# julius-sk/spgemm-prunning

Measured on AMD Instinct MI355X. Metric: SpGEMM+SSpMM GTEPS (edges/s) & HBM-BW% on Reddit h=256 k=16; vs CPU SpMM, higher is better.
Workload: dtype f32

## Files before the change

include/maxk_hip.h:

```cpp
#ifndef MAXK_HIP_H_
#define MAXK_HIP_H_

#include <stddef.h>
#include <stdint.h>

#ifdef __cplusplus
extern "C" {
#endif

#define MAXK_OK 0
#define MAXK_ERR_INVALID (-1)
#define MAXK_ERR_HIP (-2)
#define MAXK_ERR_NODEVICE (-3)
#define MAXK_ERR_LIBRARY (-4)

int maxk_version(void);

const char *maxk_last_error(void);

int maxk_device_count(void);

const char *maxk_source_digest(void);

const char *maxk_build_config(void);
// ... 3 lines not shown
int maxk_spgemm_forward(const int32_t *row_ptr, const int32_t *col_idx, const float *edge_val,
                        const float *cbsr_val, const uint8_t *cbsr_idx, const float *row_div,
                        float *out, int64_t num_rows, int64_t num_cols, int64_t num_e,
                        int32_t dim_origin, int32_t dim_k, int32_t chunk_edges,
                        void *workspace, size_t workspace_bytes, void *stream);
int maxk_spgemm_forward_sel(const int32_t *row_ptr, const int32_t *col_idx, const float *edge_val,
                            const float *cbsr_val, const uint8_t *cbsr_idx, const float *row_div,
                            float *out, int64_t num_rows, int64_t num_cols, int64_t num_e,
                            int32_t dim_origin, int32_t dim_k, int32_t chunk_edges,
                            void *workspace, size_t workspace_bytes, void *stream,
                            uint8_t *edge_sel);
int maxk_spgemm_forward_accumulate(const int32_t *row_ptr, const int32_t *col_idx,
                                   const float *edge_val, const float *cbsr_val,
                                   const uint8_t *cbsr_idx, const float *row_div, float *out,
                                   int64_t num_rows, int64_t num_cols, int64_t num_e,
                                   int32_t dim_origin, int32_t dim_k, int32_t chunk_edges,
                                   void *workspace, size_t workspace_bytes, void *stream);
int maxk_spgemm_forward_accumulate_sel(const int32_t *row_ptr, const int32_t *col_idx,
                                       const float *edge_val, const float *cbsr_val,
                                       const uint8_t *cbsr_idx, const float *row_div, float *out,
                                       int64_t num_rows, int64_t num_cols, int64_t num_e,
                                       int32_t dim_origin, int32_t dim_k, int32_t chunk_edges,
                                       void *workspace, size_t workspace_bytes, void *stream,
                                       uint8_t *edge_sel);
int maxk_records_ok(int64_t num_rows, int64_t num_cols, int64_t num_e, int32_t dim_origin,
                    int32_t dim_k);
int maxk_cbsr_records(const float *cbsr_val, const uint8_t *cbsr_idx, uint8_t *rec,
                      int64_t num_rows, int32_t dim_origin, int32_t dim_k, void *stream);
int maxk_spgemm_forward_records(const int32_t *row_ptr, const int32_t *col_idx,
                                const float *edge_val, const uint8_t *rec, const float *row_div,
                                float *out, int64_t num_rows, int64_t num_cols, int64_t num_e,
                                int32_t dim_origin, int32_t dim_k, int32_t chunk_edges,
                                void *workspace, size_t workspace_bytes, void *stream,
                                int32_t accumulate);

size_t maxk_edge_weight_grad_workspace_size(int64_t num_rows, int64_t num_cols, int64_t num_e,
                                            int32_t dim_origin, int32_t dim_k,
                                            int32_t chunk_edges);
int maxk_edge_weight_grad(const int32_t *row_ptr, const int32_t *col_idx, const float *cbsr_val,
                          const uint8_t *cbsr_idx, const float *grad_out, const float *row_div,
                          float *grad_edge, int64_t num_rows, int64_t num_cols, int64_t num_e,
                          int32_t dim_origin, int32_t dim_k, int32_t chunk_edges,
                          void *workspace, size_t workspace_bytes, void *stream);

#define MAXK_MAX_HEADS 8

size_t maxk_spgemm_forward_heads_workspace_size(int64_t num_rows, int64_t num_cols,
                                                int64_t num_e, int32_t dim_origin, int32_t dim_k,
                                                int32_t num_heads, int32_t chunk_edges);
int maxk_spgemm_forward_heads(const int32_t *row_ptr, const int32_t *col_idx,
                              const float *edge_val, const float *cbsr_val,
                              const uint8_t *cbsr_idx, const float *row_div, float *out,
                              int64_t num_rows, int64_t num_cols, int64_t num_e,
                              int32_t dim_origin, int32_t dim_k, int32_t num_heads,
                              int32_t chunk_edges, void *workspace, size_t workspace_bytes,
                              void *stream);

size_t maxk_edge_weight_grad_heads_workspace_size(int64_t num_rows, int64_t num_cols,
                                                  int64_t num_e, int32_t dim_origin,
                                                  int32_t dim_k, int32_t num_heads,
                                                  int32_t chunk_edges);
int maxk_edge_weight_grad_heads(const int32_t *row_ptr, const int32_t *col_idx,
                                const float *cbsr_val, const uint8_t *cbsr_idx,
                                const float *grad_out, const float *row_div, float *grad_edge,
                                int64_t num_rows, int64_t num_cols, int64_t num_e,
                                int32_t dim_origin, int32_t dim_k, int32_t num_heads,
                                int32_t chunk_edges, void *workspace, size_t workspace_bytes,
                                void *stream);

size_t maxk_edge_softmax_workspace_size(int64_t num_rows, int64_t num_cols, int64_t num_e,
                                        int32_t chunk_edges);
int maxk_edge_softmax(const int32_t *row_ptr, const float *logits, float *w, int64_t num_rows,
                      int64_t num_cols, int64_t num_e, int32_t chunk_edges, void *workspace,
                      size_t workspace_bytes, void *stream);
size_t maxk_edge_softmax_backward_workspace_size(int64_t num_rows, int64_t num_cols,
                                                 int64_t num_e, int32_t chunk_edges);
int maxk_edge_softmax_backward(const int32_t *row_ptr, const float *w, const float *grad_w,
                               float *grad_logits, int64_t num_rows, int64_t num_cols,
                               int64_t num_e, int32_t chunk_edges, void *workspace,
                               size_t workspace_bytes, void *stream);
size_t maxk_gat_edge_softmax_workspace_size(int64_t num_rows, int64_t num_cols, int64_t num_e,
                                            int32_t chunk_edges);
int maxk_gat_edge_softmax(const int32_t *row_ptr, const int32_t *col_idx, const float *s_dst,
                          const float *s_src, float negative_slope, float *w, int64_t num_rows,
                          int64_t num_cols, int64_t num_e, int32_t chunk_edges, void *workspace,
                          size_t workspace_bytes, void *stream);
size_t maxk_gat_edge_softmax_backward_workspace_size(int64_t num_rows, int64_t num_cols,
                                                     int64_t num_e, int32_t chunk_edges);
int maxk_gat_edge_softmax_backward(const int32_t *row_ptr, const int32_t *col_idx,
                                   const int32_t *col_ptr, const int32_t *csc_eid,
                                   const float *s_dst, const float *s_src, float negative_slope,
                                   const float *w, const float *grad_w, float *grad_s_dst,
                                   float *grad_s_src, int64_t num_rows, int64_t num_cols,
                                   int64_t num_e, int32_t chunk_edges, void *workspace,
                                   size_t workspace_bytes, void *stream);

size_t maxk_gat_edge_softmax_heads_workspace_size(int32_t num_heads, int64_t num_rows,
                                                  int64_t num_cols, int64_t num_e,
                                                  int32_t chunk_edges);
int maxk_gat_edge_softmax_heads(const int32_t *row_ptr, const int32_t *col_idx,
                                const float *s_dst, const float *s_src, float negative_slope,
                                float *w, int32_t num_heads, int64_t num_rows, int64_t num_cols,
                                int64_t num_e, int32_t chunk_edges, void *workspace,
                                size_t workspace_bytes, void *stream);
size_t maxk_gat_edge_softmax_heads_backward_workspace_size(int32_t num_heads, int64_t num_rows,
                                                           int64_t num_cols, int64_t num_e,
                                                           int32_t chunk_edges);
int maxk_gat_edge_softmax_heads_backward(const int32_t *row_ptr, const int32_t *col_idx,
                                         const int32_t *col_ptr, const int32_t *csc_eid,
                                         const float *s_dst, const float *s_src,
                                         float negative_slope, const float *w,
                                         const float *grad_w, float *grad_s_dst,
                                         float *grad_s_src, int32_t num_heads, int64_t num_rows,
                                         int64_t num_cols, int64_t num_e, int32_t chunk_edges,
                                         void *workspace, size_t workspace_bytes, void *stream);

size_t maxk_gat_attention_heads_workspace_size(int64_t num_rows, int64_t num_cols, int64_t num_e,
                                               int32_t dim_origin, int32_t dim_k,
                                               int32_t num_heads, int32_t chunk_edges);
int maxk_gat_attention_heads(const int32_t *row_ptr, const int32_t *col_idx, const float *s_dst,
                             const float *s_src, float negative_slope, const float *cbsr_val,
                             const uint8_t *cbsr_idx, float *out, float *row_max, float *row_sum,
                             int64_t num_rows, int64_t num_cols, int64_t num_e,
                             int32_t dim_origin, int32_t dim_k, int32_t num_heads,
                             int32_t chunk_edges, void *workspace, size_t workspace_bytes,
                             void *stream);
size_t maxk_gat_edge_alpha_heads_workspace_size(int32_t num_heads, int64_t num_rows,
                                                int64_t num_cols, int64_t num_e);
int maxk_gat_edge_alpha_heads(const int32_t *row_ptr, const int32_t *col_idx, const float *s_dst,
                              const float *s_src, float negative_slope, const float *row_max,
                              const float *row_sum, float *w, int32_t num_heads,
                              int64_t num_rows, int64_t num_cols, int64_t num_e, void *workspace,
                              size_t workspace_bytes, void *stream);

size_t maxk_gat_attention_heads_backward_workspace_size(int64_t num_rows, int64_t num_cols,
                                                        int64_t num_e, int32_t dim_origin,
                                                        int32_t dim_k, int32_t num_heads,
                                                        int32_t chunk_edges);
int maxk_gat_attention_heads_backward(
    const int32_t *row_ptr, const int32_t *col_idx, const int32_t *col_ptr,
    const int32_t *csc_eid, const float *s_dst, const float *s_src, float negative_slope,
    const float *cbsr_val, const uint8_t *cbsr_idx, const float *out, const float *row_max,
    const float *row_sum, const float *grad_out, float *grad_s_dst, float *grad_s_src,
    float *grad_cbsr, int64_t num_rows, int64_t num_cols, int64_t num_e, int32_t dim_origin,
    int32_t dim_k, int32_t num_heads, int32_t chunk_edges, void *workspace,
    size_t workspace_bytes, void *stream);

int maxk_edge_dropout_heads(const float *w, float *out, int32_t num_heads, int64_t num_e, float p,
                            uint64_t seed, void *stream);
size_t maxk_gat_attention_heads_dropout_workspace_size(int64_t num_rows, int64_t num_cols,
                                                       int64_t num_e, int32_t dim_origin,
                                                       int32_t dim_k, int32_t num_heads,
                                                       int32_t chunk_edges);
int maxk_gat_attention_heads_dropout(
    const int32_t *row_ptr, const int32_t *col_idx, const float *s_dst, const float *s_src,
    float negative_slope, const float *cbsr_val, const uint8_t *cbsr_idx, float *out,
    float *row_max, float *row_sum, int64_t num_rows, int64_t num_cols, int64_t num_e,
    int32_t dim_origin, int32_t dim_k, int32_t num_heads, int32_t chunk_edges, float p,
    uint64_t seed, void *workspace, size_t workspace_bytes, void *stream);
size_t maxk_gat_attention_heads_dropout_backward_workspace_size(
    int64_t num_rows, int64_t num_cols, int64_t num_e, int32_t dim_origin, int32_t dim_k,
    int32_t num_heads, int32_t chunk_edges);
int maxk_gat_attention_heads_dropout_backward(
    const int32_t *row_ptr, const int32_t *col_idx, const int32_t *col_ptr,
    const int32_t *csc_eid, const float *s_dst, const float *s_src, float negative_slope,
    const float *cbsr_val, const uint8_t *cbsr_idx, const float *out, const float *row_max,
    const float *row_sum, const float *grad_out, float *grad_s_dst, float *grad_s_src,
    float *grad_cbsr, int64_t num_rows, int64_t num_cols, int64_t num_e, int32_t dim_origin,
    int32_t dim_k, int32_t num_heads, int32_t chunk_edges, float p, uint64_t seed,
    void *workspace, size_t workspace_bytes, void *stream);

size_t maxk_dot_attention_heads_workspace_size(int64_t num_rows, int64_t num_cols, int64_t num_e,
                                               int32_t dim_origin, int32_t dim_k,
                                               int32_t num_heads, int32_t chunk_edges);
int maxk_dot_attention_heads(const int32_t *row_ptr, const int32_t *col_idx, const float *q,
                             float scale, const float *cbsr_val, const uint8_t *cbsr_idx,
                             float *out, float *row_max, float *row_sum, int64_t num_rows,
                             int64_t num_cols, int64_t num_e, int32_t dim_origin, int32_t dim_k,
                             int32_t num_heads, int32_t chunk_edges, void *workspace,
                             size_t workspace_bytes, void *stream);
size_t maxk_dot_edge_alpha_heads_workspace_size(int64_t num_rows, int64_t num_cols, int64_t num_e,
                                                int32_t dim_origin, int32_t dim_k,
                                                int32_t num_heads, int32_t chunk_edges);
int maxk_dot_edge_alpha_heads(const int32_t *row_ptr, const int32_t *col_idx, const float *q,
                              float scale, const float *cbsr_val, const uint8_t *cbsr_idx,
                              const float *row_max, const float *row_sum, float *w,
                              int64_t num_rows, int64_t num_cols, int64_t num_e,
                              int32_t dim_origin, int32_t dim_k, int32_t num_heads,
                              int32_t chunk_edges, void *workspace, size_t workspace_bytes,
                              void *stream);

size_t maxk_dot_attention_heads_backward_workspace_size(int64_t num_rows, int64_t num_cols,
                                                        int64_t num_e, int32_t dim_origin,
                                                        int32_t dim_k, int32_t num_heads,
                                                        int32_t chunk_edges);
int maxk_dot_attention_heads_backward(
    const int32_t *row_ptr, const int32_t *col_idx, const int32_t *col_ptr, const int32_t *csc_eid,
    const float *q, float scale, const float *cbsr_val, const uint8_t *cbsr_idx, const float *out,
    const float *row_max, const float *row_sum, const float *grad_out, float *grad_q,
    float *grad_cbsr, int64_t num_rows, int64_t num_cols, int64_t num_e, int32_t dim_origin,
    int32_t dim_k, int32_t num_heads, int32_t chunk_edges, void *workspace,
    size_t workspace_bytes, void *stream);

size_t maxk_sspmm_backward_workspace_size(int64_t num_rows, int64_t num_cols, int64_t num_e,
                                          int32_t dim_origin, int32_t dim_k, int32_t chunk_edges);
int maxk_sspmm_backward(const int32_t *row_ptr, const int32_t *col_idx, const float *edge_val,
                        const float *grad_out, const float *row_div, const uint8_t *cbsr_idx,
                        float *grad_cbsr, int64_t num_rows, int64_t num_cols, int64_t num_e,
                        int32_t dim_origin, int32_t dim_k, int32_t chunk_edges,
                        void *workspace, size_t workspace_bytes, void *stream);

size_t maxk_sspmm_backward_csc_workspace_size(int64_t num_rows, int64_t num_cols, int64_t num_e,
                                              int32_t dim_origin, int32_t dim_k,
                                              int32_t chunk_edges);
int maxk_sspmm_backward_csc(const int32_t *row_ptr, const int32_t *col_idx, const float *edge_val,
                            const float *grad_out, const float *row_div, const uint8_t *cbsr_idx,
                            const int32_t *col_ptr, const int32_t *csc_eid, float *grad_cbsr,
                            int64_t num_rows, int64_t num_cols, int64_t num_e, int32_t dim_origin,
                            int32_t dim_k, int32_t chunk_edges, void *workspace,
                            size_t workspace_bytes, void *stream);

int maxk_sspmm_backward_csc_sel(const int32_t *row_ptr, const int32_t *col_idx,
                                const float *edge_val, const float *grad_out, const float *row_div,
                                const uint8_t *edge_sel, const int32_t *col_ptr,
                                const int32_t *csc_eid, float *grad_cbsr, int64_t num_rows,
                                int64_t num_cols, int64_t num_e, int32_t dim_origin, int32_t dim_k,
                                int32_t chunk_edges, void *workspace, size_t workspace_bytes,
                                void *stream);
int maxk_edge_selectors(const int32_t *col_idx, const uint8_t *cbsr_idx, int64_t num_e,
                        int32_t dim_k, uint8_t *edge_sel, void *stream);
int64_t maxk_edge_selectors_blocks(int64_t n_words);

size_t maxk_sspmm_backward_heads_workspace_size(int64_t num_rows, int64_t num_cols,
                                                int64_t num_e, int32_t dim_origin, int32_t dim_k,
                                                int32_t num_heads, int32_t chunk_edges);
int maxk_sspmm_backward_heads(const int32_t *row_ptr, const int32_t *col_idx,
                              const float *edge_val, const float *grad_out, const float *row_div,
                              const uint8_t *cbsr_idx, const int32_t *col_ptr,
                              const int32_t *csc_eid, float *grad_cbsr, int64_t num_rows,
                              int64_t num_cols, int64_t num_e, int32_t dim_origin, int32_t dim_k,
                              int32_t num_heads, int32_t chunk_edges, void *workspace,
                              size_t workspace_bytes, void *stream);

size_t maxk_transpose_plan_workspace_size(int64_t num_cols, int64_t num_e);
int maxk_transpose_plan(const int32_t *col_idx, int64_t num_cols, int64_t num_e,
                        int32_t *col_ptr, int32_t *csc_eid, void *workspace,
                        size_t workspace_bytes, void *stream);

int maxk_bucket_shift(int32_t dim_k);
int64_t maxk_bucket_count(int64_t num_cols, int32_t bucket_shift);

int32_t maxk_bsort_window(int32_t dim_k);
size_t maxk_bsort_plan_workspace_size(int64_t num_cols, int64_t num_e);
int maxk_bsort_plan(const int32_t *row_ptr, const int32_t *col_idx, int64_t num_rows,
                    int64_t num_cols, int64_t num_e, int32_t dim_k, int32_t bucket_shift,
                    int32_t *bucket_ptr, int32_t *bucket_pos, uint16_t *bucket_dst,
                    uint16_t *win_src, int32_t *edge_row, void *workspace,
                    size_t workspace_bytes, void *stream);
size_t maxk_sspmm_backward_bsort_workspace_size(int64_t num_rows, int64_t num_cols,
                                                int64_t num_e, int32_t dim_origin,
                                                int32_t dim_k);
int maxk_sspmm_backward_bsort(const int32_t *row_ptr, const int32_t *col_idx,
                              const float *edge_val, const float *grad_out, const float *row_div,
                              const uint8_t *cbsr_idx, const uint8_t *edge_sel,
                              const int32_t *bucket_ptr, const int32_t *bucket_pos,
                              const uint16_t *bucket_dst, const uint16_t *win_src,
                              const int32_t *edge_row, int32_t bucket_shift, float *grad_cbsr,
                              int64_t num_rows,
                              int64_t num_cols, int64_t num_e, int32_t dim_origin, int32_t dim_k,
                              void *workspace, size_t workspace_bytes, void *stream);

size_t maxk_sspmm_backward_pull_workspace_size(int64_t num_rows, int64_t num_cols,
                                               int32_t dim_origin, int32_t dim_k, int32_t slices);
int maxk_sspmm_backward_pull(const float *grad_out, const float *row_div,
                             const uint8_t *cbsr_idx, const int32_t *tile_ptr,
                             const uint32_t *ent, int32_t bucket_shift, int32_t slices,
                             float *grad_cbsr, int64_t num_rows, int64_t num_cols, int64_t num_e,
                             int32_t dim_origin, int32_t dim_k, void *workspace,
                             size_t workspace_bytes, void *stream);

#define MAXK_PULL_NO_REDUCE 2
#define MAXK_PULL_REDUCE_ONLY 4
size_t maxk_sspmm_backward_pull_tiles_workspace_size(int64_t num_rows, int64_t num_cols,
                                                     int32_t dim_origin, int32_t dim_k,
                                                     int32_t n_tiles);
int maxk_sspmm_backward_pull_tiles(const float *grad_out, const float *row_div,
                                   const uint8_t *cbsr_idx, const int32_t *tile_list,
                                   const int32_t *tile_ent, int32_t n_tiles,
                                   const int32_t *bucket_ptr, const int32_t *bucket_tiles,
                                   const uint32_t *ent, int32_t bucket_shift, int32_t slices,
                                   int32_t accumulate, float *grad_cbsr, int64_t num_rows,
                                   int64_t num_cols, int64_t num_e, int32_t dim_origin,
                                   int32_t dim_k, void *workspace, size_t workspace_bytes,
                                   void *stream);

int maxk_pull_shift(int32_t dim_k);
int maxk_pull_slices(int64_t num_rows, int64_t num_cols, int32_t dim_origin, int32_t dim_k);
size_t maxk_pull_plan_workspace_size(int64_t num_rows, int64_t num_cols, int64_t num_e,
                                     int32_t bucket_shift, int32_t slices);
int maxk_pull_plan(const int32_t *row_ptr, const int32_t *col_idx, const float *edge_val,
                   int64_t num_rows, int64_t num_cols, int64_t num_e, int32_t bucket_shift,
                   int32_t slices, int32_t *tile_ptr, uint32_t *ent, void *workspace,
                   size_t workspace_bytes, void *stream);

int maxk_dense_route(int32_t dim_origin, int32_t dim_k);
int maxk_dense_plan(const int32_t *row_ptr, const float *edge_val, const int32_t *csc_eid,
                    int64_t num_rows, int64_t num_e, int32_t *t_src, float *t_w, void *stream);
size_t maxk_sspmm_backward_dense_workspace_size(int64_t num_rows, int64_t num_cols,
                                                int64_t num_e, int32_t dim_origin, int32_t dim_k,
                                                int32_t chunk_edges);
int maxk_sspmm_backward_dense(const int32_t *col_ptr, const int32_t *t_src, const float *t_w,
                              const float *grad_out, const float *row_div,
                              const uint8_t *cbsr_idx, float *grad_cbsr, int64_t num_rows,
                              int64_t num_cols, int64_t num_e, int32_t dim_origin, int32_t dim_k,
                              int32_t chunk_edges, void *workspace, size_t workspace_bytes,
                              void *stream);

#define MAXK_BWD_PULL 0
#define MAXK_BWD_CSC 1
#define MAXK_BWD_HYBRID 3
#define MAXK_BWD_ATOMIC 4
#define MAXK_BWD_BSORT 5
#define MAXK_BWD_DENSE 6
#define MAXK_BSORT_KMAX 8
#define MAXK_HYBRID_LOCALITY 1.5
#define MAXK_HYBRID_DENSITY 0.5f
#define MAXK_HYBRID_PRESCALED 1
int maxk_backward_mode_auto(int64_t num_rows, int64_t num_cols, int64_t num_e, int32_t dim_origin,
                            int32_t dim_k, double pull_locality);
int maxk_pull_locality(const int32_t *row_ptr, const int32_t *col_idx, int64_t num_rows,
                       int64_t num_e, int32_t bucket_shift, double *locality, void *workspace,
                       size_t workspace_bytes, void *stream);
size_t maxk_hybrid_plan_workspace_size(int64_t num_rows, int64_t num_cols, int64_t num_e,
                                       int32_t bucket_shift, int32_t slices);
int maxk_hybrid_plan(const int32_t *row_ptr, const int32_t *col_idx, const float *edge_val,
                     const int32_t *tile_ptr, const uint32_t *ent, int64_t num_rows,
                     int64_t num_cols, int64_t num_e, int32_t bucket_shift, int32_t slices,
                     float density, int32_t *tile_list, int32_t *tile_ent, int32_t *bucket_ptr,
                     int32_t *bucket_tiles, uint32_t *ent_pull, int32_t *off_row_ptr,
                     int32_t *off_col, float *off_val, int64_t *counts, void *workspace,
                     size_t workspace_bytes, void *stream);
int maxk_pull_entries_scale(const uint32_t *ent, const int32_t *tile_ids, const int32_t *tile_ent,
                            int64_t n_runs, int64_t num_rows, int64_t num_cols,
                            int32_t bucket_shift, int32_t slices, const float *row_div,
                            uint32_t *ent_out, void *stream);
size_t maxk_sspmm_backward_hybrid_workspace_size(int64_t num_rows, int64_t num_cols,
                                                 int64_t n_off_e, int32_t dim_origin,
                                                 int32_t dim_k, int64_t n_tiles);
int maxk_sspmm_backward_hybrid(
    const float *grad_out, const float *row_div, const uint8_t *cbsr_idx,
    const int32_t *tile_list, const int32_t *tile_ent, int32_t n_tiles, const int32_t *bucket_ptr,
    const int32_t *bucket_tiles, const uint32_t *ent_pull, int64_t n_pull_e, int32_t bucket_shift,
    int32_t slices, const int32_t *off_row_ptr, const int32_t *off_col, const float *off_val,
    int64_t n_off_e, const int32_t *off_col_ptr, const int32_t *off_csc_eid, int32_t flags,
    float *grad_cbsr, int64_t num_rows, int64_t num_cols, int32_t dim_origin, int32_t dim_k,
    void *workspace, size_t workspace_bytes, void *stream, void *side_stream, void *ev_fork,
    void *ev_join);

int maxk_topk_cbsr(const float *x, int64_t ld_x, float *cbsr_val, uint8_t *cbsr_idx,
                   int32_t *idx32, int64_t num_rows, int32_t dim_origin, int32_t dim_k,
                   void *stream);
int maxk_topk_cbsr_u8(const uint8_t *x, int64_t ld_x, uint8_t *cbsr_val, uint8_t *cbsr_idx,
                      int32_t *idx32, int64_t num_rows, int32_t dim_origin, int32_t dim_k,
                      void *stream);
int maxk_topk_u8_reference(const uint8_t *x, uint8_t *val, uint8_t *idx, int64_t num_rows,
                           int32_t dim_origin, int32_t dim_k, void *stream);
int maxk_topk_error_rows(int64_t *rows, int32_t reset, void *stream);

int maxk_cbsr_scatter_dense(const float *cbsr_val, const uint8_t *cbsr_idx, float *dense,
                            int64_t num_rows, int32_t dim_origin, int32_t dim_k, void *stream);

int maxk_topk_cbsr_dense(const float *x, int64_t ld_x, float *cbsr_val, uint8_t *cbsr_idx,
                         float *dense, int64_t num_rows, int32_t dim_origin, int32_t dim_k,
                         void *stream);

int maxk_topk_backward(const float *grad_val, const float *grad_dense, const uint8_t *cbsr_idx,
                       float *grad_x, int64_t num_rows, int32_t dim_origin, int32_t dim_k,
                       void *stream);

int maxk_warp4_count(const int32_t *row_ptr, int64_t num_rows, int32_t warp_max_nz,
                     int64_t *num_entries, void *stream);
size_t maxk_warp4_build_workspace_size(int64_t num_rows);
int maxk_warp4_build(const int32_t *row_ptr, int64_t num_rows, int32_t warp_max_nz,
                     int32_t *warp4, int64_t num_entries, void *workspace,
                     size_t workspace_bytes, void *stream);
int maxk_warp4_to_row_ptr(const int32_t *warp4, int64_t num_entries, int64_t num_rows,
                          int32_t *row_ptr, void *stream);

typedef struct maxk_dense_spmm_plan maxk_dense_spmm_plan;
int maxk_dense_spmm_plan_create(maxk_dense_spmm_plan **plan, const int32_t *row_ptr,
                                const int32_t *col_idx, const float *edge_val, const float *x,
                                float *y, int64_t num_rows, int64_t num_cols, int64_t num_e,
                                int32_t dim, int32_t alg, void *stream);
int maxk_dense_spmm_run(maxk_dense_spmm_plan *plan, void *stream);
int maxk_dense_spmm_bind(maxk_dense_spmm_plan *plan, const float *x, float *y);
int maxk_dense_spmm_plan_destroy(maxk_dense_spmm_plan *plan);

#ifdef __cplusplus
}
#endif

#endif
```

spgemm-prunning_amd/csrc/sspmm_pull.hip:

```cpp
#include <algorithm>

#include "sspmm_bwd.h"

namespace maxk {
namespace {

__global__ __launch_bounds__(kBlock) void gprime_kernel(const float *__restrict__ G,
                                                        const float *__restrict__ row_div,
                                                        float *__restrict__ Gp, int64_t n4,
                                                        int D4) {
    const int64_t i = blockIdx.x * (int64_t)kBlock + threadIdx.x;
    if (i >= n4) return;
    const float dv = row_div[i / D4];
    float4 v = reinterpret_cast<const float4 *>(G)[i];
    v.x /= dv;
    v.y /= dv;
    v.z /= dv;
    v.w /= dv;
    reinterpret_cast<float4 *>(Gp)[i] = v;
}

template <int LR, int U, bool SEL_LDS, int VPL>
__global__ __launch_bounds__(1024) void pull_tile_kernel(
    const float *__restrict__ Gp, const uint8_t *__restrict__ cbsr_idx,
    const int32_t *__restrict__ tile_ptr, const uint2 *__restrict__ ent,
    float *__restrict__ tile_out, int64_t num_cols, int n_buckets, int rows_per_slice, int D,
    int k, int shift) {
    extern __shared__ double acc[];
    constexpr int EPI = kWave / LR;
    constexpr int STEP = EPI * U;
    const int tid = threadIdx.x;
    const int lane = lane_id(), w = tid / kWave;
    const int g = lane / LR, q = lane % LR;
    const bool qok = q < k / VPL;
    const int ks = k + 1;
    const int t = blockIdx.x;
    const int j = t % n_buckets;
    const float *__restrict__ Gs = Gp + (size_t)(t / n_buckets) * rows_per_slice * D;
    const int s0 = tile_ptr[t], s1 = tile_ptr[t + 1];
    const int64_t c0 = (int64_t)j << shift;
    const uint8_t *__restrict__ selg = cbsr_idx + c0 * k;
    uint8_t *sel_lds = reinterpret_cast<uint8_t *>(acc + (ks << shift));
    for (int i = tid; i < (ks << shift); i += 1024) acc[i] = 0.0;
    if (SEL_LDS) {
        const int rows = num_cols - c0 < (1 << shift) ? (int)(num_cols - c0) : (1 << shift);
        const int nb = rows * k;
        for (int i = tid; i < nb / 16; i += 1024)
            reinterpret_cast<uint4 *>(sel_lds)[i] = reinterpret_cast<const uint4 *>(selg)[i];
        for (int i = (nb & ~15) + tid; i < nb; i += 1024) sel_lds[i] = selg[i];
    }
    __syncthreads();
    int base = s0 + w * STEP;
    uint2 en[U];
    constexpr bool kShfl = MAXK_PULL_SHFL && LR <= 8;
    constexpr int NL = (STEP + kWave - 1) / kWave;
    uint2 my[NL];
    auto load_ids = [&](int b) {
        if constexpr (kShfl) {
#pragma unroll
            for (int m = 0; m < NL; ++m) {
                const int e = b + m * kWave + lane;
                my[m] = ent[e < s1 ? e : s1 - 1];
                if (e >= s1 || m * kWave + lane >= STEP) my[m].x = 0xffff0000u;
            }
        } else {
#pragma unroll
            for (int u = 0; u < U; ++u) {
                const int e = b + u * EPI + g;
                en[u] = ent[e < s1 ? e : s1 - 1];
                if (e >= s1) en[u].x = 0xffff0000u;
            }
        }
    };
    if (base < s1) load_ids(base);
    for (; base < s1; base += 16 * STEP) {
        if constexpr (kShfl) {
#pragma unroll
            for (int u = 0; u < U; ++u) {
                const int m = (u * EPI) / kWave;
                const int src = (u * EPI + g - m * kWave) * 4;
                en[u].x = (uint32_t)__builtin_amdgcn_ds_bpermute(src, (int)my[m].x);
                en[u].y = (uint32_t)__builtin_amdgcn_ds_bpermute(src, (int)my[m].y);
            }
        }
        uint32_t sv[U];
        int dc[U];
        float wc[U];
#pragma unroll
        for (int u = 0; u < U; ++u) {
            const uint32_t key = en[u].x;
            dc[u] = (key >> 16) == 0xffffu ? -1 : (int)(key >> 16);
            const int bo = (dc[u] < 0 ? 0 : dc[u]) * k + (qok ? q : 0) * VPL;
            const uint8_t *sb8 = SEL_LDS ? sel_lds : selg;
            sv[u] = VPL == 4 ? *reinterpret_cast<const uint32_t *>(sb8 + bo) : (uint32_t)sb8[bo];
        }
        float v[U][VPL];
#pragma unroll
        for (int u = 0; u < U; ++u) {
            const float *gr = Gs + (en[u].x & 0xffffu) * (uint32_t)D;
#pragma unroll
            for (int i = 0; i < VPL; ++i) {
                const uint32_t c = (sv[u] >> (8 * i)) & 255u;
                const bool in = c < (uint32_t)D;
                const float x = gr[in ? c : 0u];
                v[u][i] = in ? x : 0.0f;
            }
            wc[u] = __uint_as_float(en[u].y);
        }
        if (base + 16 * STEP < s1) load_ids(base + 16 * STEP);
#pragma unroll
        for (int u = 0; u < U; ++u) {
            if (dc[u] >= 0 && qok) {
                double *a = &acc[dc[u] * ks + VPL * q];
#pragma unroll
                for (int i = 0; i < VPL; ++i) atomicAdd(a + i, (double)(wc[u] * v[u][i]));
            }
        }
    }
    __syncthreads();
    float *o = tile_out + (size_t)t * ((size_t)k << shift);
    if (MAXK_PULL_F4_FLUSH && k % 4 == 0) {
        for (int i4 = tid; i4 < (k << shift) / 4; i4 += 1024) {
            const double *a = &acc[i4 * 4 + (i4 * 4) / k];
            reinterpret_cast<float4 *>(o)[i4] =
                make_float4((float)a[0], (float)a[1], (float)a[2], (float)a[3]);
        }
    } else {
        for (int i = tid; i < (k << shift); i += 1024) o[i] = (float)acc[i + i / k];
    }
}

__global__ __launch_bounds__(kBlock) void pull_sel_kernel(const uint8_t *__restrict__ sel,
                                                          uint8_t *__restrict__ sel_q,
                                                          uint8_t *__restrict__ lmap,
                                                          int64_t num_cols, int k, int kp,
                                                          int vpl) {
    __shared__ uint32_t bm[kBlock / 4 * 8];
    __shared__ uint8_t s_out[kBlock], l_out[kBlock];
    const int nd = kBlock / k;
    const int tid = threadIdx.x;
    const int d = tid / k, l = tid % k;
    const int64_t c0 = (int64_t)blockIdx.x * nd;
    const int64_t c = c0 + d;
    const bool act = d < nd && c < num_cols;
    for (int i = tid; i < nd * 8; i += kBlock) bm[i] = 0u;
    __syncthreads();
    const uint32_t s = act ? sel[c * k + l] : 0u;
    if (act) atomicOr(&bm[d * 8 + (s >> 5)], 1u << (s & 31));
    __syncthreads();
    if (act) {
        int distinct = 0, rank = 0;
        for (int wd = 0; wd < 8; ++wd) {
            const uint32_t b = bm[d * 8 + wd];
            distinct += __popc(b);
            if (wd < (int)(s >> 5)) rank += __popc(b);
        }
        rank += __popc(bm[d * 8 + (s >> 5)] & ((1u << (s & 31)) - 1u));
        if (distinct < k) {
            rank = 0;
            for (int m = 0; m < k; ++m) {
                const uint32_t sm = sel[c * k + m];
                rank += (sm < s) || (sm == s && m < l);
            }
        }
        const int ql = kp / vpl, h = rank / kp, r = rank % kp;
        const int slot = h * kp + vpl * (r % ql) + r / ql;
        s_out[d * k + slot] = (uint8_t)s;
        l_out[d * k + slot] = (uint8_t)l;
    }
    __syncthreads();
    const int64_t nb = (num_cols - c0 < nd ? num_cols - c0 : nd) * (int64_t)k;
    if (tid < nb) {
        sel_q[c0 * k + tid] = s_out[tid];
        lmap[c0 * k + tid] = l_out[tid];
    }
}

__global__ __launch_bounds__(kBlock) void pull_sel4_kernel(const uint8_t *__restrict__ sel,
                                                           uint8_t *__restrict__ sel_q,
                                                           uint8_t *__restrict__ lmap,
                                                           int64_t num_cols, int k, int kp,
                                                           int vpl) {
    __shared__ uint32_t bm[kBlock * 8];
    __shared__ uint32_t s_out[kBlock], l_out[kBlock];
    const int tpd = k / 4;
    const int nd = kBlock / tpd;
    const int tid = threadIdx.x;
    const int d = tid / tpd, l0 = (tid % tpd) * 4;
    const int64_t c0 = (int64_t)blockIdx.x * nd;
    const int64_t c = c0 + d;
    const bool act = d < nd && c < num_cols;
    for (int i = tid; i < nd * 8; i += kBlock) bm[i] = 0u;
    __syncthreads();
    const uint32_t w4 = act ? *reinterpret_cast<const uint32_t *>(sel + c * k + l0) : 0u;
    if (act) {
#pragma unroll
        for (int j = 0; j < 4; ++j) {
            const uint32_t sj = (w4 >> (8 * j)) & 255u;
            atomicOr(&bm[d * 8 + (sj >> 5)], 1u << (sj & 31));
        }
    }
    __syncthreads();
    if (act) {
        uint32_t wds[8];
        int distinct = 0;
#pragma unroll
        for (int wd = 0; wd < 8; ++wd) {
            wds[wd] = bm[d * 8 + wd];
            distinct += __popc(wds[wd]);
        }
        uint8_t *so = reinterpret_cast<uint8_t *>(s_out), *lo = reinterpret_cast<uint8_t *>(l_out);
        const int ql = kp / vpl;
#pragma unroll
        for (int j = 0; j < 4; ++j) {
            const uint32_t sj = (w4 >> (8 * j)) & 255u;
            const int l = l0 + j;
            int rank = 0;
            if (distinct == k) {
                const int hi = (int)(sj >> 5);
#pragma unroll
                for (int wd = 0; wd < 8; ++wd) {
                    rank += wd < hi ? __popc(wds[wd]) : 0;
                    rank += wd == hi ? __popc(wds[wd] & ((1u << (sj & 31)) - 1u)) : 0;
                }
            } else {
                for (int m = 0; m < k; ++m) {
                    const uint32_t sm = sel[c * k + m];
                    rank += (sm < sj) || (sm == sj && m < l);
                }
            }
            const int h = rank / kp, r = rank % kp;
            const int slot = h * kp + vpl * (r % ql) + r / ql;
            so[d * k + slot] = (uint8_t)sj;
            lo[d * k + slot] = (uint8_t)l;
        }
    }
    __syncthreads();
    const int64_t nbytes = (num_cols - c0 < nd ? num_cols - c0 : nd) * (int64_t)k;
    if ((int64_t)tid * 4 < nbytes) {
        reinterpret_cast<uint32_t *>(sel_q + c0 * k)[tid] = s_out[tid];
        reinterpret_cast<uint32_t *>(lmap + c0 * k)[tid] = l_out[tid];
    }
}

template <int LR, int U, bool FULLD, int VPL>
__device__ __forceinline__ void pull_q_entries(double *acc, const uint8_t *sel_lds,
                                               __amdgpu_buffer_rsrc_t grs,
                                               __amdgpu_buffer_rsrc_t ers, int n_e, int D,
                                               int kp, int shift) {
    constexpr int EPI = kWave / LR;
    constexpr int STEP = EPI * U;
    constexpr int NL = (STEP + kWave - 1) / kWave;
    const int tid = threadIdx.x;
    const int lane = lane_id(), w = tid / kWave;
    constexpr int EPQ = LR < 16 ? 16 / LR : 1;
    const int lc = (lane % 16) % 4, lm = (lane % 16) / 4;
    constexpr bool TR = MAXK_PULL_TRANSPOSE && LR <= 16;
    const int g = !TR ? lane / LR
                  : LR >= 4 ? (lane / 16) * EPQ + lc / (LR / 4 > 0 ? LR / 4 : 1)
                            : (lane / 16) * EPQ + lc * (4 / LR) + lm / LR;
    const int q = !TR ? lane % LR
                  : LR >= 4 ? (lc % (LR / 4 > 0 ? LR / 4 : 1)) * 4 + lm
                            : lm % LR;
    const bool qok = q < kp / VPL;
    const int ks = pull_ks(kp, shift);
    const uint32_t Db = (uint32_t)D * 4u;
    const int stride = 16 * STEP;
    const int base = w * STEP;
    const int nsteps = base < n_e ? (n_e - base + stride - 1) / stride : 0;
    const int idle = (w * kWave + lane) & ((1 << shift) - 1);

    typedef unsigned int u32x2 __attribute__((ext_vector_type(2)));
    u32x2 myA[NL], myB[NL];
    float vA[U][VPL], vB[U][VPL];
    int dA[U], dB[U];
    float wA[U], wB[U];
    auto load_ent = [&](u32x2(&my)[NL], int n) {
#pragma unroll
        for (int m = 0; m < NL; ++m)
            my[m] = __builtin_amdgcn_raw_buffer_load_b64(
                ers, (int)((uint32_t)(base + n * stride + m * kWave + lane) * 8u), 0, 0);
    };
    auto issue = [&](u32x2(&my)[NL], float(&v)[U][VPL], int(&dc)[U], float(&wc)[U], int n) {
        uint32_t ex[U], ey[U];
#pragma unroll
        for (int u = 0; u < U; ++u) {
            const int m = (u * EPI) / kWave;
            const int src = (u * EPI + g - m * kWave) * 4;
            ex[u] = (uint32_t)__builtin_amdgcn_ds_bpermute(src, (int)my[m][0]);
            ey[u] = (uint32_t)__builtin_amdgcn_ds_bpermute(src, (int)my[m][1]);
        }
        load_ent(my, n + 2);
        uint64_t sv[U];
        bool ok[U];
        const int eb = base + n * stride + g;
#pragma unroll
        for (int u = 0; u < U; ++u) {
            ok[u] = eb + u * EPI < n_e && qok;
            const int d = ok[u] ? (int)(ex[u] >> 16) : idle;
            dc[u] = d * ks + VPL * q * ok[u];
            const uint8_t *sp = sel_lds + d * kp + (ok[u] ? q * VPL : 0);
            if constexpr (VPL == 8)
                sv[u] = *reinterpret_cast<const uint64_t *>(sp);
            else if constexpr (VPL == 4)
                sv[u] = *reinterpret_cast<const uint32_t *>(sp);
            else
                sv[u] = *reinterpret_cast<const uint16_t *>(sp);
            wc[u] = ok[u] ? __uint_as_float(ey[u]) : 0.0f;
        }
#pragma unroll
        for (int u = 0; u < U; ++u) {
            const uint32_t ro = ok[u] ? (ex[u] & 0xffffu) * Db : 0x80000000u;
#pragma unroll
            for (int i = 0; i < VPL; ++i) {
                const uint32_t c = VPL == 8 ? (uint32_t)(sv[u] >> (8 * i)) & 255u
                                            : ((uint32_t)sv[u] >> (8 * i)) & 255u;
                uint32_t off = ro + c * 4u;
                if (!FULLD) off = c < (uint32_t)D ? off : 0x80000000u;
                v[u][i] = __builtin_bit_cast(
                    float, __builtin_amdgcn_raw_buffer_load_b32(grs, (int)off, 0, 0));
            }
        }
    };
    auto consume = [&](float(&v)[U][VPL], int(&dc)[U], float(&wc)[U]) {
#pragma unroll
        for (int u = 0; u < U; ++u) {
            double *a = &acc[dc[u]];
#pragma unroll
            for (int i = 0; i < VPL; ++i) atomicAdd(a + i, (double)(wc[u] * v[u][i]));
        }
    };
    if (nsteps > 0) {
        load_ent(myA, 0);
        load_ent(myB, 1);
        __builtin_amdgcn_sched_barrier(0);
        issue(myA, vA, dA, wA, 0);
        for (int n = 0; n < nsteps; n += 2) {
            issue(myB, vB, dB, wB, n + 1);
            __builtin_amdgcn_sched_barrier(0);
            consume(vA, dA, wA);
            __builtin_amdgcn_sched_barrier(0);
            issue(myA, vA, dA, wA, n + 2);
            __builtin_amdgcn_sched_barrier(0);
            consume(vB, dB, wB);
            __builtin_amdgcn_sched_barrier(0);
        }
    }
}

struct PullTile {
    int64_t r0, nrows, c0;
    int s0, s1;
};
__device__ __forceinline__ PullTile pull_tile_of(int t, int i, const int32_t *__restrict__ tile_ptr,
                                                 int n_buckets, int rows_per_slice,
                                                 int64_t num_rows, int shift) {
    PullTile p;
    p.r0 = (int64_t)(t / n_buckets) * rows_per_slice;
    p.nrows = num_rows - p.r0 < rows_per_slice ? num_rows - p.r0 : rows_per_slice;
    p.c0 = (int64_t)(t % n_buckets) << shift;
    p.s0 = tile_ptr[i];
    p.s1 = tile_ptr[i + 1];
    return p;
}

constexpr int kSelRegs = 2;
struct PullSel {
    uint4 v[kSelRegs];
};
__device__ __forceinline__ PullSel pull_sel_load(const uint8_t *__restrict__ sel_q, int64_t c0,
                                                 int64_t num_cols, int k, int kp, int h,
                                                 int shift) {
    PullSel r;
    const int tid = threadIdx.x;
    const int rows = num_cols - c0 < (1 << shift) ? (int)(num_cols - c0) : (1 << shift);
    const uint8_t *__restrict__ selg = sel_q + c0 * k + h * kp;
#pragma unroll
    for (int m = 0; m < kSelRegs; ++m) {
        const int i = tid + m * 1024;
        uint4 x = make_uint4(0u, 0u, 0u, 0u);
        if (kp % 16 == 0) {
            const int ppr = kp / 16;
            if (i < rows * ppr)
                x = *reinterpret_cast<const uint4 *>(selg + (int64_t)(i / ppr) * k + (i % ppr) * 16);
        } else {
            uint32_t wd[4];
            const int wpr = kp / 4;
#pragma unroll
            for (int b = 0; b < 4; ++b) {
                const int wi = i * 4 + b;
                wd[b] = wi < rows * wpr
                            ? *reinterpret_cast<const uint32_t *>(selg + (int64_t)(wi / wpr) * k +
                                                                  (wi % wpr) * 4)
                            : 0u;
            }
            x = make_uint4(wd[0], wd[1], wd[2], wd[3]);
        }
        r.v[m] = x;
    }
    return r;
}
__device__ __forceinline__ void pull_sel_store(uint8_t *sel_lds, const PullSel &r, int kp,
                                               int shift) {
    const int n16 = (kp << shift) / 16;
#pragma unroll
    for (int m = 0; m < kSelRegs; ++m) {
        const int i = threadIdx.x + m * 1024;
        if (i < n16) reinterpret_cast<uint4 *>(sel_lds)[i] = r.v[m];
    }
}

__device__ __forceinline__ void pull_flush(const double *acc, float *__restrict__ tile_out, int t,
                                           int h, int k, int kp, int shift) {
    const int ks = pull_ks(kp, shift);
    float *o = tile_out + (size_t)t * ((size_t)k << shift) + h * kp;
    const int w4 = kp / 4;
    for (int i4 = threadIdx.x; i4 < (kp << shift) / 4; i4 += 1024) {
        const int c = i4 / w4, s4 = i4 % w4;
        const double *a = &acc[c * ks + 4 * s4];
        *reinterpret_cast<float4 *>(o + (size_t)c * k + 4 * s4) =
            make_float4((float)a[0], (float)a[1], (float)a[2], (float)a[3]);
    }
}

template <int LR, int U, bool FULLD, int VPL>
__global__ __launch_bounds__(1024) void pull_q_kernel(
    const float *__restrict__ Gp, const uint8_t *__restrict__ sel_q,
    const int32_t *__restrict__ tile_ptr, const uint2 *__restrict__ ent,
    float *__restrict__ tile_out, int64_t num_cols, int n_buckets, int n_tiles,
    int rows_per_slice, int64_t num_rows, int D, int k, int kp, int shift,
    const int32_t *__restrict__ tile_list) {
    extern __shared__ double acc[];
    const int tid = threadIdx.x;
    const int ks = pull_ks(kp, shift);
    const int H = k / kp;
    const int tp = MAXK_PULL_XCD ? xcd_contiguous_block(blockIdx.x, gridDim.x) : blockIdx.x;
    if (tp >= n_tiles * H) return;
    const int ti = tp / H, h = tp % H;
    const int t = tile_list ? tile_list[ti] : ti;
    const PullTile p = pull_tile_of(t, ti, tile_ptr, n_buckets, rows_per_slice, num_rows, shift);
    uint8_t *sel_lds = reinterpret_cast<uint8_t *>(acc + (ks << shift));
    for (int i = tid; i < (ks << shift); i += 1024) acc[i] = 0.0;
    pull_sel_store(sel_lds, pull_sel_load(sel_q, p.c0, num_cols, k, kp, h, shift), kp, shift);
    __syncthreads();
    const auto grs =
        wave_buffer(Gp + p.r0 * D, (uint32_t)(p.nrows > 0 ? p.nrows : 0) * (uint32_t)D * 4u);
    const auto ers = wave_buffer(ent + p.s0, (uint32_t)(p.s1 - p.s0) * 8u);
    pull_q_entries<LR, U, FULLD, VPL>(acc, sel_lds, grs, ers, p.s1 - p.s0, D, kp, shift);
    __syncthreads();
    pull_flush(acc, tile_out, ti, h, k, kp, shift);
}

__global__ __launch_bounds__(kBlock) void pull_reduce_kernel(const float *__restrict__ tile_out,
                                                             const uint8_t *__restrict__ lmap,
                                                             float *__restrict__ grad_cbsr,
                                                             int64_t num_cols, int n_buckets,
                                                             int slices, int k, int shift,
                                                             const int32_t *__restrict__ bucket_ptr,
                                                             const int32_t *__restrict__ bucket_tiles,
                                                             int accumulate) {
    const int j = blockIdx.x;
    const int64_t c0 = (int64_t)j << shift;
    const int rows = num_cols - c0 < (1 << shift) ? (int)(num_cols - c0) : (1 << shift);
    const int i = blockIdx.y * kBlock + threadIdx.x;
    const int nf = rows * k;
    if (i * 4 >= nf) return;
    const size_t n4 = ((size_t)k << shift) / 4;
    const float4 *to = reinterpret_cast<const float4 *>(tile_out);
    if (i * 4 + 4 > nf) {
        const int f0 = i * 4;
        for (int f = f0; f < nf; ++f) {
            float a = tile_out[(size_t)j * n4 * 4 + f];
            for (int s = 1; s < slices; ++s) a += tile_out[((size_t)s * n_buckets + j) * n4 * 4 + f];
            grad_cbsr[c0 * k + f] = a;
        }
        return;
    }
    float4 a;
    if (bucket_ptr) {
        a = make_float4(0.f, 0.f, 0.f, 0.f);
        for (int q = bucket_ptr[j]; q < bucket_ptr[j + 1]; ++q) {
            const float4 b = to[(size_t)bucket_tiles[q] * n4 + i];
            a.x += b.x;
            a.y += b.y;
            a.z += b.z;
            a.w += b.w;
        }
    } else {
        a = to[(size_t)j * n4 + i];
        for (int s = 1; s < slices; ++s) {
            const float4 b = to[((size_t)s * n_buckets + j) * n4 + i];
            a.x += b.x;
            a.y += b.y;
            a.z += b.z;
            a.w += b.w;
        }
    }
    if (lmap) {
        const size_t f0 = (size_t)c0 * k + (size_t)i * 4;
        const uint32_t m = *reinterpret_cast<const uint32_t *>(lmap + f0);
        float *row = grad_cbsr + (f0 / k) * k;
        if (accumulate) {
            a.x += row[m & 255u];
            a.y += row[(m >> 8) & 255u];
            a.z += row[(m >> 16) & 255u];
            a.w += row[m >> 24];
        }
        row[m & 255u] = a.x;
        row[(m >> 8) & 255u] = a.y;
        row[(m >> 16) & 255u] = a.z;
        row[m >> 24] = a.w;
        return;
    }
    reinterpret_cast<float4 *>(grad_cbsr + c0 * k)[i] = a;
}

int pull_parts(int k, int shift) {
    for (int H = 1; H <= k / 4; H *= 2) {
        if (k % (4 * H)) break;
        if (pull_fits(k / H, k / H, shift)) return H;
    }
    return 0;
}

struct PullLayout {
    size_t tile_off, sel_off, lmap_off, total;
};

PullLayout pull_layout(int64_t num_rows, int64_t num_cols, int D, int k, int64_t tiles,
                       int shift) {
    PullLayout L{};
    L.tile_off = al256((size_t)num_rows * D * sizeof(float));
    L.sel_off = L.tile_off + (size_t)tiles * ((size_t)k << shift) * sizeof(float);
    const size_t nsel = k % 4 == 0 ? al256((size_t)num_cols * k) : 0;
    L.lmap_off = L.sel_off + nsel;
    L.total = L.lmap_off + nsel;
    return L;
}

int pull_impl(const float *grad_out, const float *row_div, const uint8_t *cbsr_idx,
              const int32_t *tile_ptr, const uint32_t *ent, int32_t bucket_shift, int32_t slices,
              bool listed, const int32_t *tile_list, int32_t n_list, const int32_t *bucket_ptr,
              const int32_t *bucket_tiles, int32_t accumulate, float *grad_cbsr, int64_t num_rows,
              int64_t num_cols, int64_t num_e, int32_t dim_origin, int32_t dim_k, void *workspace,
              size_t workspace_bytes, void *stream) {
    if (int rc = check_common(num_rows, num_cols, num_e, dim_origin, dim_k, 0)) return rc;
    MAXK_REQUIRE(dim_k % 4 == 0 || dim_k <= 64,
                 "pull backward needs dim_k %% 4 == 0 or dim_k <= 64, got %d", dim_k);
    MAXK_REQUIRE(dim_origin % 4 == 0, "pull backward needs dim_origin %% 4 == 0, got %d",
                 dim_origin);
    const bool v4 = dim_k % 4 == 0;
    const int parts = MAXK_PULL_Q && v4 && bucket_shift >= 4 && bucket_shift <= 15
                          ? pull_parts(dim_k, bucket_shift)
                          : 0;
    const int max_shift = std::max(maxk_bucket_shift(dim_k), maxk_pull_shift(dim_k));
    MAXK_REQUIRE(bucket_shift >= 4 && bucket_shift <= 15 && bucket_shift <= max_shift &&
                     (parts > 0 || bucket_shift <= maxk_bucket_shift(dim_k)),
                 "bucket_shift %d out of range [4, min(15, %d)] for dim_k %d", bucket_shift,
                 max_shift, dim_k);
    const int64_t nb = maxk_bucket_count(num_cols, bucket_shift);
    MAXK_REQUIRE(slices >= 1 && slices * nb < (1LL << 31), "slices %d out of range", slices);
    const int64_t rps = (num_rows + slices - 1) / slices;
    MAXK_REQUIRE(rps <= 65536, "%d slices leave %lld rows per slice (max 65536)", slices,
                 (long long)rps);
    hipStream_t s = as_stream(stream);
    if (num_cols == 0) return MAXK_OK;
    MAXK_REQUIRE(grad_cbsr && tile_ptr, "grad_cbsr/tile_ptr must not be NULL");
    MAXK_REQUIRE(num_e == 0 || (grad_out && cbsr_idx && ent),
                 "grad/selector/plan pointers must not be NULL");
    MAXK_REQUIRE(!listed || (parts > 0 && bucket_ptr && n_list >= 0 &&
                             (n_list == 0 || (tile_list && bucket_tiles))),
                 "listed tiles need dim_k %% 4 == 0 and tile_list/bucket_ptr/bucket_tiles");
    const int64_t tiles = listed ? (int64_t)n_list : (int64_t)slices * nb;
    const PullLayout L = pull_layout(num_rows, num_cols, dim_origin, dim_k, tiles, bucket_shift);
    MAXK_REQUIRE(workspace && workspace_bytes >= L.total,
                 "workspace too small: need %zu bytes, got %zu", L.total, workspace_bytes);
    char *ws = reinterpret_cast<char *>(workspace);
    const bool front = !(accumulate & MAXK_PULL_REDUCE_ONLY);
    const bool back = !(accumulate & MAXK_PULL_NO_REDUCE);
    MAXK_REQUIRE(listed || (front && back), "reduce-only / no-reduce need listed tiles");
    MAXK_REQUIRE(front || back, "no-reduce and reduce-only together run nothing");
    const int k = dim_k;
    const float *Gp = grad_out;
    if (front && row_div && num_rows > 0 && num_e > 0) {
        const int64_t n4 = num_rows * dim_origin / 4;
        hipLaunchKernelGGL(gprime_kernel, dim3((unsigned)ceil_div(n4, kBlock)), dim3(kBlock), 0,
                           s, grad_out, row_div, reinterpret_cast<float *>(workspace), n4,
                           dim_origin / 4);
        MAXK_LAUNCHED("gprime_kernel");
        Gp = reinterpret_cast<const float *>(workspace);
    }
    float *tile_out = reinterpret_cast<float *>(ws + L.tile_off);
    const size_t acc_b = ((size_t)(k + 1) << bucket_shift) * sizeof(double);
    const size_t sel_b = ((size_t)k << bucket_shift);
    const bool sel_lds = acc_b + sel_b <= kPullLdsBytes;
    const size_t lds = acc_b + (sel_lds ? sel_b : 0);
    const uint2 *ent2 = reinterpret_cast<const uint2 *>(ent);
    const uint8_t *lmap = nullptr;
    if (parts > 0) {
        const int kp = k / parts;
        const size_t lds_q = pull_lds_bytes(pull_ks(kp, bucket_shift), kp, bucket_shift);
        uint8_t *sel_q = reinterpret_cast<uint8_t *>(ws + L.sel_off);
        uint8_t *lm = reinterpret_cast<uint8_t *>(ws + L.lmap_off);
        const int nd = kBlock / k;
        const int vpl = kp != 8 ? 4 : MAXK_PULL_VPL8 ? MAXK_PULL_VPL8 : parts == 1 ? 8 : 4;
        lmap = lm;
        if (!front) goto reduce;
        if (MAXK_PULL_SEL4 && (reinterpret_cast<uintptr_t>(cbsr_idx) & 3) == 0) {
            const int nd4 = kBlock / (k / 4);
            hipLaunchKernelGGL(pull_sel4_kernel, dim3((unsigned)ceil_div(num_cols, nd4)),
                               dim3(kBlock), 0, s, cbsr_idx, sel_q, lm, num_cols, k, kp, vpl);
            MAXK_LAUNCHED("pull_sel4_kernel");
        } else {
            hipLaunchKernelGGL(pull_sel_kernel, dim3((unsigned)ceil_div(num_cols, nd)),
                               dim3(kBlock), 0, s, cbsr_idx, sel_q, lm, num_cols, k, kp, vpl);
            MAXK_LAUNCHED("pull_sel_kernel");
        }
        const int64_t work = tiles * parts;
        const bool fulld = dim_origin == kMaxDim;
        const unsigned grid = (unsigned)(MAXK_PULL_XCD ? xcd_grid(work) : work);
        if (work == 0) goto reduce;
        const int lr = vpl == 4 ? lanes_per_edge(kp / 4) : kp / vpl;
        const bool ok = with_lanes(lr, [&](auto lr_c) {
            with_const<2, 4, 8>(vpl, [&](auto vpl_c) {
                with_const<0, 1>(fulld, [&](auto fd_c) {
                    constexpr int LR = decltype(lr_c)::value, VPL = decltype(vpl_c)::value;
                    if constexpr (VPL == 4 || LR * VPL == 8)
                        hipLaunchKernelGGL(
                            (pull_q_kernel<LR, MAXK_PULL_QU, decltype(fd_c)::value, VPL>),
                            dim3(grid), dim3(1024), lds_q, s, Gp, sel_q, tile_ptr, ent2, tile_out,
                            num_cols, (int)nb, (int)tiles, (int)rps, num_rows, dim_origin, k, kp,
                            bucket_shift, tile_list);
                });
            });
        });
        if (!ok) return bad_lanes(lr);
        MAXK_LAUNCHED("pull_q_kernel");
    } else {
        const int lr = lanes_per_edge(v4 ? k / 4 : k);
        const bool ok = with_lanes(lr, [&](auto lr_c) {
            with_const<0, 1>(sel_lds, [&](auto sl_c) {
                with_const<1, 4>(v4 ? 4 : 1, [&](auto vpl_c) {
                    hipLaunchKernelGGL(
                        (pull_tile_kernel<decltype(lr_c)::value, MAXK_PULL_U,
                                          decltype(sl_c)::value, decltype(vpl_c)::value>),
                        dim3((unsigned)tiles), dim3(1024), lds, s, Gp, cbsr_idx, tile_ptr, ent2,
                        tile_out, num_cols, (int)nb, (int)rps, dim_origin, k, bucket_shift);
                });
            });
        });
        if (!ok) return bad_lanes(lr);
        MAXK_LAUNCHED("pull_tile_kernel");
    }
reduce:
    if (!back) return MAXK_OK;
    hipLaunchKernelGGL(pull_reduce_kernel,
                       dim3((unsigned)nb, (unsigned)ceil_div(ceil_div((int64_t)k << bucket_shift, 4), kBlock)),
                       dim3(kBlock), 0, s, tile_out, lmap, grad_cbsr, num_cols, (int)nb, slices,
                       k, bucket_shift, listed ? bucket_ptr : nullptr,
                       listed ? bucket_tiles : nullptr, accumulate & 1);
    MAXK_LAUNCHED("pull_reduce_kernel");
    return MAXK_OK;
}
}
}

using namespace maxk;

extern "C" size_t maxk_sspmm_backward_pull_workspace_size(int64_t num_rows, int64_t num_cols,
                                                          int32_t dim_origin, int32_t dim_k,
                                                          int32_t slices) {
    if (num_rows < 0 || num_cols < 0 || dim_origin <= 0 || dim_k <= 0 || slices <= 0) return 0;
    const int shift = std::max(maxk_bucket_shift(dim_k), maxk_pull_shift(dim_k));
    return pull_layout(num_rows, num_cols, dim_origin, dim_k,
                       (int64_t)slices * maxk_bucket_count(num_cols, shift), shift).total;
}

extern "C" int maxk_sspmm_backward_pull(const float *grad_out, const float *row_div,
                                        const uint8_t *cbsr_idx, const int32_t *tile_ptr,
                                        const uint32_t *ent, int32_t bucket_shift,
                                        int32_t slices, float *grad_cbsr, int64_t num_rows,
                                        int64_t num_cols, int64_t num_e, int32_t dim_origin,
                                        int32_t dim_k, void *workspace, size_t workspace_bytes,
                                        void *stream) {
    clear_error();
    return pull_impl(grad_out, row_div, cbsr_idx, tile_ptr, ent, bucket_shift, slices, false,
                     nullptr, 0, nullptr, nullptr, 0, grad_cbsr, num_rows, num_cols, num_e, dim_origin, dim_k,
                     workspace, workspace_bytes, stream);
}

extern "C" size_t maxk_sspmm_backward_pull_tiles_workspace_size(int64_t num_rows,
                                                                int64_t num_cols,
                                                                int32_t dim_origin,
                                                                int32_t dim_k, int32_t n_tiles) {
    if (num_rows < 0 || num_cols < 0 || dim_origin <= 0 || dim_k <= 0 || n_tiles < 0) return 0;
    return pull_layout(num_rows, num_cols, dim_origin, dim_k, n_tiles,
                       std::max(maxk_bucket_shift(dim_k), maxk_pull_shift(dim_k))).total;
}

extern "C" int maxk_sspmm_backward_pull_tiles(
    const float *grad_out, const float *row_div, const uint8_t *cbsr_idx,
    const int32_t *tile_list, const int32_t *tile_ent, int32_t n_tiles,
    const int32_t *bucket_ptr, const int32_t *bucket_tiles, const uint32_t *ent,
    int32_t bucket_shift, int32_t slices, int32_t accumulate, float *grad_cbsr,
    int64_t num_rows, int64_t num_cols, int64_t num_e, int32_t dim_origin, int32_t dim_k,
    void *workspace, size_t workspace_bytes, void *stream) {
    clear_error();
    MAXK_REQUIRE(tile_ent, "tile_ent must not be NULL");
    return pull_impl(grad_out, row_div, cbsr_idx, tile_ent, ent, bucket_shift, slices, true,
                     tile_list, n_tiles, bucket_ptr, bucket_tiles, accumulate, grad_cbsr, num_rows, num_cols,
                     num_e, dim_origin, dim_k, workspace, workspace_bytes, stream);
}
```

spgemm-prunning_amd/csrc/transpose.hip:

```cpp
#include <hipcub/hipcub.hpp>

#include <algorithm>

#include "common.h"

namespace maxk {
namespace {

__global__ void iota_kernel(int32_t *__restrict__ a, int64_t n) {
    const int64_t i = (int64_t)blockIdx.x * blockDim.x + threadIdx.x;
    if (i < n) a[i] = (int32_t)i;
}

__global__ void col_ptr_kernel(const int32_t *__restrict__ sorted_cols, int64_t num_e,
                               int num_cols, int32_t *__restrict__ col_ptr) {
    const int64_t t = (int64_t)blockIdx.x * blockDim.x + threadIdx.x;
    if (t > num_e) return;
    int cur = t < num_e ? sorted_cols[t] : num_cols;
    int prev = t == 0 ? -1 : sorted_cols[t - 1];
    cur = cur > num_cols ? num_cols : cur;
    prev = prev > num_cols ? num_cols : prev;
    for (int c = prev + 1; c <= cur; ++c) col_ptr[c] = (int32_t)t;
}

// ... 117 lines not shown
    size_t tmp_bytes = workspace_bytes - 2 * a;
    hipLaunchKernelGGL(iota_kernel, dim3((unsigned)ceil_div(num_e, kBlock)), dim3(kBlock), 0, s,
                       ids, num_e);
    MAXK_LAUNCHED("iota_kernel");
    const int kb = key_bits(num_cols);
    if (bucket_shift < kb) {
        MAXK_HIP(hipcub::DeviceRadixSort::SortPairs(tmp, tmp_bytes, col_idx, keys_out, ids,
                                                    bucket_eid, (int)num_e, bucket_shift, kb, s));
    } else {
        MAXK_HIP(hipMemcpyAsync(keys_out, col_idx, (size_t)num_e * 4, hipMemcpyDeviceToDevice, s));
        MAXK_HIP(hipMemcpyAsync(bucket_eid, ids, (size_t)num_e * 4, hipMemcpyDeviceToDevice, s));
    }
    hipLaunchKernelGGL(bucket_ptr_kernel, dim3((unsigned)ceil_div(num_e + 1, kBlock)),
                       dim3(kBlock), 0, s, keys_out, num_e, (int)bucket_shift, (int)nb, bucket_ptr,
                       bucket_dst);
    MAXK_LAUNCHED("bucket_ptr_kernel");
    return MAXK_OK;
}

namespace maxk {
namespace {

__global__ void bsort_key_kernel(const int32_t *__restrict__ col_idx, int64_t num_e, int W,
                                 int nb, int shift, int32_t *__restrict__ keys,
                                 int32_t *__restrict__ ids) {
    const int64_t e = (int64_t)blockIdx.x * blockDim.x + threadIdx.x;
    if (e >= num_e) return;
    int b = col_idx[e] >> shift;
    b = b < 0 ? 0 : (b >= nb ? nb - 1 : b);
    keys[e] = (int32_t)((e / W) * nb + b);
    ids[e] = (int32_t)e;
}

__global__ void bsort_pos_kernel(const int32_t *__restrict__ perm, int64_t num_e, int W,
                                 uint16_t *__restrict__ win_src, int32_t *__restrict__ pos) {
    const int64_t p = (int64_t)blockIdx.x * blockDim.x + threadIdx.x;
    if (p >= num_e) return;
    const int e = perm[p];
    win_src[p] = (uint16_t)(e - p / W * W);
    pos[e] = (int32_t)p;
}

__global__ void bsort_map_kernel(const int32_t *__restrict__ pos, int64_t num_e,
                                 int32_t *__restrict__ bucket_pos) {
    const int64_t i = (int64_t)blockIdx.x * blockDim.x + threadIdx.x;
    if (i < num_e) bucket_pos[i] = pos[bucket_pos[i]];
}

__global__ void bsort_rows_kernel(const int32_t *__restrict__ row_ptr, int num_rows,
                                  int64_t num_e, int32_t *__restrict__ edge_row) {
    const int64_t e = (int64_t)blockIdx.x * blockDim.x + threadIdx.x;
    if (e >= num_e) return;
    int lo = 0, hi = num_rows - 1;
    while (lo < hi) {
        const int mid = (int)(((int64_t)lo + hi + 1) >> 1);
        if (row_ptr[mid] <= e) lo = mid; else hi = mid - 1;
    }
    edge_row[e] = lo;
}

size_t bsort_sort_bytes(int64_t num_e) {
    size_t bytes = 0;
    (void)hipcub::DeviceRadixSort::SortPairs(nullptr, bytes, (const int32_t *)nullptr,
                                             (int32_t *)nullptr, (const int32_t *)nullptr,
                                             (int32_t *)nullptr, (int)num_e, 0, 31);
    return bytes;
}

}
}

extern "C" size_t maxk_bsort_plan_workspace_size(int64_t num_cols, int64_t num_e) {
    if (num_cols < 0 || num_e <= 0) return 0;
    const size_t a = al256((size_t)num_e * 4);
    const size_t bucket = bucket_plan_workspace_size(num_cols, num_e);
    const size_t own = 4 * a + al256(bsort_sort_bytes(num_e));
    return own > bucket ? own : bucket;
}

extern "C" int maxk_bsort_plan(const int32_t *row_ptr, const int32_t *col_idx, int64_t num_rows,
                               int64_t num_cols, int64_t num_e, int32_t dim_k,
                               int32_t bucket_shift, int32_t *bucket_ptr, int32_t *bucket_pos,
                               uint16_t *bucket_dst, uint16_t *win_src, int32_t *edge_row,
                               void *workspace, size_t workspace_bytes, void *stream) {
    clear_error();
    const int W = maxk_bsort_window(dim_k);
    MAXK_REQUIRE(W > 0, "window-sorted plan needs dim_k %% 4 == 0 in [4, 256], got %d", dim_k);
    MAXK_REQUIRE(num_rows >= 0 && num_rows < (1LL << 31), "num_rows out of range");
    MAXK_REQUIRE(num_cols >= 0 && num_cols < (1LL << 31), "num_cols out of range");
    MAXK_REQUIRE(num_e >= 0 && num_e < (1LL << 31), "num_e out of range");
    MAXK_REQUIRE(bucket_shift >= 0 && bucket_shift <= 16, "bucket_shift must be in [0,16]");
    const int64_t nb = maxk_bucket_count(num_cols, bucket_shift);
    const int64_t nwin = ceil_div(num_e, W);
    MAXK_REQUIRE(nwin * (nb > 0 ? nb : 1) < (1LL << 31),
                 "%lld windows x %lld buckets exceed the 31-bit sort key", (long long)nwin,
                 (long long)nb);
    const size_t need = maxk_bsort_plan_workspace_size(num_cols, num_e);
    if (num_e > 0) {
        MAXK_REQUIRE(row_ptr && win_src && edge_row, "row_ptr/win_src/edge_row must not be NULL");
        MAXK_REQUIRE(num_rows > 0, "edges present but num_rows == 0");
        MAXK_REQUIRE(workspace && workspace_bytes >= need, "workspace too small: need %zu", need);
    }
    if (int rc = bucket_plan(col_idx, num_cols, num_e, bucket_shift, bucket_ptr, bucket_pos,
                                  bucket_dst, workspace, workspace_bytes, stream))
        return rc;
    if (num_e == 0) return MAXK_OK;
    hipStream_t s = as_stream(stream);
    char *ws = reinterpret_cast<char *>(workspace);
    const size_t a = al256((size_t)num_e * 4);
    int32_t *keys = reinterpret_cast<int32_t *>(ws);
    int32_t *ids = reinterpret_cast<int32_t *>(ws + a);
    int32_t *keys_out = reinterpret_cast<int32_t *>(ws + 2 * a);
    int32_t *perm = reinterpret_cast<int32_t *>(ws + 3 * a);
    void *tmp = ws + 4 * a;
    size_t tmp_bytes = workspace_bytes - 4 * a;
    const dim3 g((unsigned)ceil_div(num_e, kBlock));
    const int nbi = (int)(nb > 0 ? nb : 1);
    hipLaunchKernelGGL(bsort_key_kernel, g, dim3(kBlock), 0, s, col_idx, num_e, W, nbi,
                       (int)bucket_shift, keys, ids);
    MAXK_LAUNCHED("bsort_key_kernel");
    MAXK_HIP(hipcub::DeviceRadixSort::SortPairs(tmp, tmp_bytes, keys, keys_out, ids, perm,
                                                (int)num_e, 0, key_bits(nwin * nbi), s));
    int32_t *pos = keys;
    hipLaunchKernelGGL(bsort_pos_kernel, g, dim3(kBlock), 0, s, perm, num_e, W, win_src, pos);
    MAXK_LAUNCHED("bsort_pos_kernel");
    hipLaunchKernelGGL(bsort_map_kernel, g, dim3(kBlock), 0, s, pos, num_e, bucket_pos);
    MAXK_LAUNCHED("bsort_map_kernel");
    hipLaunchKernelGGL(bsort_rows_kernel, g, dim3(kBlock), 0, s, row_ptr, (int)num_rows, num_e,
                       edge_row);
    MAXK_LAUNCHED("bsort_rows_kernel");
    return MAXK_OK;
}

namespace maxk {
namespace {

constexpr int64_t kPullSliceBytes = 7LL << 19;

__global__ void pull_key_kernel(const int32_t *__restrict__ row_ptr,
                                const int32_t *__restrict__ col_idx, int num_rows,
                                int rows_per_slice, int n_buckets, int shift,
                                int32_t *__restrict__ keys, int32_t *__restrict__ row_of) {
    const int r = (int)(((int64_t)blockIdx.x * blockDim.x + threadIdx.x) / kWave);
    if (r >= num_rows) return;
    const int lane = lane_id();
    const int b = row_ptr[r], e = row_ptr[r + 1];
    const int base = (r / rows_per_slice) * n_buckets;
    for (int i = b + lane; i < e; i += kWave) {
        keys[i] = base + (col_idx[i] >> shift);
        row_of[i] = r;
    }
}

__global__ void pull_gather_kernel(const int32_t *__restrict__ eid,
                                   const int32_t *__restrict__ row_of,
                                   const int32_t *__restrict__ col_idx,
                                   const float *__restrict__ edge_val, int64_t num_e, int shift,
                                   int rows_per_slice, uint2 *__restrict__ ent) {
    const int64_t i = (int64_t)blockIdx.x * blockDim.x + threadIdx.x;
    if (i >= num_e) return;
    const int e = eid[i];
    const int r = row_of[e];
    const uint32_t in_slice = (uint32_t)(r % rows_per_slice);
    const uint32_t dst = (uint32_t)(col_idx[e] & ((1 << shift) - 1));
    ent[i] = make_uint2(in_slice | (dst << 16), __float_as_uint(edge_val[e]));
}

__global__ void tile_ptr_kernel(const int32_t *__restrict__ sorted_keys, int64_t num_e,
                                int n_tiles, int32_t *__restrict__ tile_ptr) {
    const int64_t t = (int64_t)blockIdx.x * blockDim.x + threadIdx.x;
    if (t > num_e) return;
    int cur = t < num_e ? sorted_keys[t] : n_tiles;
    int prev = t == 0 ? -1 : sorted_keys[t - 1];
    cur = cur > n_tiles ? n_tiles : cur;
    prev = prev > n_tiles ? n_tiles : prev;
    for (int x = prev + 1; x <= cur; ++x) tile_ptr[x] = (int32_t)t;
}

size_t pull_sort_temp_bytes(int64_t num_e, int64_t n_tiles) {
    size_t bytes = 0;
    (void)hipcub::DeviceRadixSort::SortPairs(nullptr, bytes, (const int32_t *)nullptr,
                                             (int32_t *)nullptr, (const int32_t *)nullptr,
                                             (int32_t *)nullptr, (int)num_e, 0,
                                             key_bits(n_tiles));
    return bytes;
}

}
}

extern "C" int maxk_pull_shift(int32_t dim_k) {
    if (dim_k <= 0) return -1;
    int s = maxk_bucket_shift(dim_k);
    const int kp_min = dim_k >= 32 ? MAXK_PULL_MIN_KP_WIDE : MAXK_PULL_MIN_KP;
    for (int H = 2; MAXK_PULL_Q && H <= MAXK_PULL_H && dim_k % (4 * H) == 0 &&
                    dim_k / H >= kp_min;
         H *= 2) {
        const int kp = dim_k / H;
        int sh = 0;
        while (sh < 15 && maxk::pull_fits(kp, kp, sh + 1)) ++sh;
        s = std::max(s, sh);
    }
    const int p = s - MAXK_PULL_SHIFT_DELTA;
    return p < 4 ? 4 : (p > 15 ? 15 : p);
}

static int pull_parts_of(int32_t dim_k) {
    int H = 1;
    const int kp_min = dim_k >= 32 ? MAXK_PULL_MIN_KP_WIDE : MAXK_PULL_MIN_KP;
    while (MAXK_PULL_Q && 2 * H <= MAXK_PULL_H && dim_k % (8 * H) == 0 && dim_k / (2 * H) >= kp_min)
        H *= 2;
    return H;
}


extern "C" int maxk_pull_slices(int64_t num_rows, int64_t num_cols, int32_t dim_origin,
                                int32_t dim_k) {
    if (num_rows <= 0 || dim_origin <= 0) return 1;
    if (num_cols <= 0) num_cols = num_rows;
    const int parts = dim_k % 4 == 0 ? pull_parts_of(dim_k) : 1;
    const int64_t part_bytes = dim_k <= 8    ? maxk::kPullSliceBytes * 3 / 2
                               : dim_k <= 16 ? maxk::kPullSliceBytes * 33 / 28
                                             : maxk::kPullSliceBytes;
    const int64_t per = part_bytes * (parts < 3 ? parts : 3);
    int64_t s = (num_rows * dim_origin * 4 + per - 1) / per;
    const int64_t lo = (num_rows + 65535) / 65536;
    s = s < lo ? lo : s;
    if (dim_k % 4 == 0 && MAXK_PULL_Q) {
        const int shift = maxk_pull_shift(dim_k);
        const int64_t wg = maxk_bucket_count(num_cols, shift) * parts;
        const int64_t cus = device_cus();
        auto rounds = [&](int64_t n) { return (n * wg + cus - 1) / cus; };
        if (shift > 0 && wg > 0 && rounds(s) <= 5) {
            int64_t best = s;
            for (int64_t c = s - 1; c >= (s + 1) / 2 && c >= lo; --c)
                if (rounds(c) < rounds(best)) best = c;
            s = best;
        }
    }
    return (int)(s < 1 ? 1 : (s > 256 ? 256 : s));
}

extern "C" size_t maxk_pull_plan_workspace_size(int64_t num_rows, int64_t num_cols,
                                                int64_t num_e, int32_t bucket_shift,
                                                int32_t slices) {
    if (num_rows < 0 || num_cols < 0 || num_e <= 0 || slices <= 0) return 0;
    const int64_t nt = slices * maxk_bucket_count(num_cols, bucket_shift);
    return 5 * al256((size_t)num_e * 4) + al256(pull_sort_temp_bytes(num_e, nt));
}

extern "C" int maxk_pull_plan(const int32_t *row_ptr, const int32_t *col_idx,
                              const float *edge_val, int64_t num_rows, int64_t num_cols,
                              int64_t num_e, int32_t bucket_shift, int32_t slices,
                              int32_t *tile_ptr, uint32_t *ent, void *workspace,
                              size_t workspace_bytes, void *stream) {
    clear_error();
    MAXK_REQUIRE(num_rows >= 0 && num_rows < (1LL << 31), "num_rows out of range");
    MAXK_REQUIRE(num_cols >= 0 && num_cols < (1LL << 31), "num_cols out of range");
    MAXK_REQUIRE(num_e >= 0 && num_e < (1LL << 31), "num_e out of range");
    MAXK_REQUIRE(bucket_shift >= 4 && bucket_shift <= 15, "bucket_shift must be in [4,15]");
    const int64_t nb = maxk_bucket_count(num_cols, bucket_shift);
    MAXK_REQUIRE(slices >= 1 && slices * nb < (1LL << 31), "slices %d out of range", slices);
    const int64_t rps64 = (num_rows + slices - 1) / slices;
    MAXK_REQUIRE(rps64 <= 65536, "%d slices leave %lld rows per slice (max 65536)", slices,
                 (long long)rps64);
    MAXK_REQUIRE(tile_ptr != nullptr, "tile_ptr must not be NULL");
    hipStream_t s = as_stream(stream);
    const int64_t nt = slices * nb;
    if (num_e == 0 || num_rows == 0) {
        MAXK_HIP(hipMemsetAsync(tile_ptr, 0, (size_t)(nt + 1) * 4, s));
        return MAXK_OK;
    }
    MAXK_REQUIRE(row_ptr && col_idx && edge_val && ent, "CSR/plan pointers must not be NULL");
    const size_t need = maxk_pull_plan_workspace_size(num_rows, num_cols, num_e, bucket_shift, slices);
    MAXK_REQUIRE(workspace && workspace_bytes >= need, "workspace too small: need %zu", need);
    char *ws = reinterpret_cast<char *>(workspace);
    const size_t a = al256((size_t)num_e * 4);
    int32_t *keys = reinterpret_cast<int32_t *>(ws);
    int32_t *keys_out = reinterpret_cast<int32_t *>(ws + a);
    int32_t *ids = reinterpret_cast<int32_t *>(ws + 2 * a);
    int32_t *eid = reinterpret_cast<int32_t *>(ws + 3 * a);
    int32_t *row_of = reinterpret_cast<int32_t *>(ws + 4 * a);
    void *tmp = ws + 5 * a;
    size_t tmp_bytes = workspace_bytes - 5 * a;
    const int rps = (int)rps64;
    hipLaunchKernelGGL(pull_key_kernel, dim3((unsigned)ceil_div(num_rows * kWave, kBlock)),
                       dim3(kBlock), 0, s, row_ptr, col_idx, (int)num_rows, rps, (int)nb,
                       (int)bucket_shift, keys, row_of);
    MAXK_LAUNCHED("pull_key_kernel");
    hipLaunchKernelGGL(iota_kernel, dim3((unsigned)ceil_div(num_e, kBlock)), dim3(kBlock), 0, s,
                       ids, num_e);
    MAXK_LAUNCHED("iota_kernel");
    MAXK_HIP(hipcub::DeviceRadixSort::SortPairs(tmp, tmp_bytes, keys, keys_out, ids, eid,
                                                (int)num_e, 0, key_bits(nt), s));
    hipLaunchKernelGGL(pull_gather_kernel, dim3((unsigned)ceil_div(num_e, kBlock)), dim3(kBlock),
                       0, s, eid, row_of, col_idx, edge_val, num_e, (int)bucket_shift, rps,
                       reinterpret_cast<uint2 *>(ent));
    MAXK_LAUNCHED("pull_gather_kernel");
    hipLaunchKernelGGL(tile_ptr_kernel, dim3((unsigned)ceil_div(num_e + 1, kBlock)), dim3(kBlock),
                       0, s, keys_out, num_e, (int)nt, tile_ptr);
    MAXK_LAUNCHED("tile_ptr_kernel");
    return MAXK_OK;
}
```

spgemm-prunning_amd/maxk_cuda_kernels/__init__.py:

```python
from __future__ import annotations

import contextlib
import ctypes
import os
import warnings
from typing import List, Optional, Tuple

import torch

from . import _capi
from ._cache import TensorCache

_L = _capi.load()

__all__ = [
    "spmm_maxk_forward", "spmm_maxk_backward", "cuda_topk_maxk", "cuda_topk_maxk_float",
    "topk_u8_reference",
    "records_ok",
    "cbsr_records",
    "spgemm_forward_records",
    "prepare_cbsr_format_maxk", "cusparse_spmm", "load_warp4_metadata",
    "load_warp4_metadata_csc", "generate_sparse_selector", "benchmark_spmm_maxk",
    "validate_spmm_maxk", "validate_spmm_maxk_backward", "CudaTimer",
    "topk_cbsr", "cbsr_scatter_dense", "topk_cbsr_dense", "topk_backward", "topk_error_rows",
    "build_warp4_metadata", "warp4_to_indptr",
    "spgemm_forward", "sspmm_backward", "edge_weight_grad", "graph_only_mode", "DenseSpMMPlan",
    "edge_softmax", "edge_softmax_backward", "gat_edge_softmax", "gat_edge_softmax_backward",
    "spgemm_forward_heads", "edge_weight_grad_heads", "MAX_HEADS", "heads_forward_route",
    "sspmm_backward_heads", "heads_backward_route",
    "gat_edge_softmax_heads", "gat_edge_softmax_heads_backward", "heads_softmax_route",
    "gat_attention_heads", "gat_edge_alpha_heads", "heads_attention_route",
    "gat_attention_heads_backward", "heads_attention_backward_route", "edge_dropout_heads",
    "dot_attention_heads", "dot_edge_alpha_heads", "dot_attention_heads_backward",
    "dot_attention_backward_route",
    "version", "device_count",
    "transpose_plan", "bsort_plan", "pull_plan", "edge_selector_mode", "backward_plan", "BWD_MODES",
    "dense_plan", "hybrid_plan", "pull_locality", "edge_selectors_wanted",
]

FULL_DIM = 256


def _lib():
    return _L


def version() -> int:
    return _lib().maxk_version()


def device_count() -> int:
    return _lib().maxk_device_count()


def _validate_mode() -> str:
    v = os.environ.get("MAXK_VALIDATE", "")
    return "once" if v == "" else ("never" if v == "0" else "always")


def _validate_default() -> bool:
    return _validate_mode() == "always"


_CHECKED = TensorCache()


def _check_graph_once(row_ptr, col_idx, num_cols):
    def build():
        _validate_graph(row_ptr, col_idx, num_cols, col_idx.numel())
        return True
    _CHECKED.get((row_ptr, col_idx), (int(num_cols),), build)


def _validate_call(validate, row_ptr, col_idx, num_cols, sel, D):
    if validate is False:
        return
    if torch.cuda.is_current_stream_capturing():
        return
    if validate if validate is not None else _validate_default():
        _validate_graph(row_ptr, col_idx, num_cols, col_idx.numel())
        _validate_selector(sel, D)
    elif validate is None and _validate_mode() == "once":
        _check_graph_once(row_ptr, col_idx, num_cols)


def _ptr(t: Optional[torch.Tensor]):
    return t.data_ptr() if t is not None and t.numel() > 0 else None


def _need(t, name, dtype=None):
    if not isinstance(t, torch.Tensor):
        raise RuntimeError(f"{name} must be a tensor")
    if not t.is_cuda:
        raise RuntimeError(f"{name} must be CUDA tensor")
    if dtype is not None and t.dtype != dtype:
        raise RuntimeError(f"{name} must be {str(dtype).replace('torch.', '')}")
    if not t.is_contiguous():
        raise RuntimeError(f"{name} must be contiguous")


def _stream(dev):
    return torch._C._cuda_getCurrentRawStream(
        dev.index if dev.index is not None else torch.cuda.current_device())


_NO_SWITCH = contextlib.nullcontext()


def _on(dev):
    cur = torch._C._cuda_getDevice()
    return _NO_SWITCH if dev.index is None or dev.index == cur else torch.cuda.device(dev)


def _launch(dev, name, *args):
    with _on(dev):
        _capi.check(getattr(_L, name)(*args), name)


def _sized(dev, name, *args) -> int:
    with _on(dev):
        return int(getattr(_L, name)(*args))


def _workspace(dev, size_name, *size_args) -> torch.Tensor:
    return torch.empty(max(_sized(dev, size_name, *size_args), 1), dtype=torch.uint8, device=dev)


def _launch_ws(dev, name, size_name, size_args, args, tail=()):
    with _on(dev):
        n = max(getattr(_L, size_name)(*size_args), 1)
        ws = torch.empty(n, dtype=torch.uint8, device=dev)
        _capi.check(getattr(_L, name)(*args, ws.data_ptr(), n, _stream(dev), *tail), name)


def _validate_graph(row_ptr, col_idx, num_cols, num_e):
    if row_ptr.numel() == 0:
        raise RuntimeError("row_ptr must have num_rows+1 entries")
    if int(row_ptr[0]) != 0 or int(row_ptr[-1]) != num_e:
        raise RuntimeError(f"row_ptr must start at 0 and end at num_e={num_e}")
    if row_ptr.numel() > 1 and bool((row_ptr[1:] < row_ptr[:-1]).any()):
        raise RuntimeError("row_ptr must be non-decreasing")
    if num_e and (int(col_idx.min()) < 0 or int(col_idx.max()) >= num_cols):
        raise RuntimeError(f"col_idx out of range [0, {num_cols})")


def _validate_selector(sel, D):
    if sel.numel() and int(sel.max()) >= D:
        raise RuntimeError(f"sparse_selector entries must be < dim_origin={D}")


def warp4_to_indptr(warp4_metadata: torch.Tensor, num_v: int,
                    num_warps: Optional[int] = None) -> torch.Tensor:
    _need(warp4_metadata, "warp4_metadata", torch.int32)
    W = warp4_metadata.numel() // 4 if num_warps is None else min(int(num_warps),
                                                                   warp4_metadata.numel() // 4)
    row_ptr = torch.empty(num_v + 1, dtype=torch.int32, device=warp4_metadata.device)
    _launch(warp4_metadata.device, "maxk_warp4_to_row_ptr", _ptr(warp4_metadata), W, num_v,
            _ptr(row_ptr), _stream(warp4_metadata.device))
    return row_ptr


def build_warp4_metadata(indptr: torch.Tensor, warp_max_nz: int = 64) -> torch.Tensor:
    _need(indptr, "indptr", torch.int32)
    dev = indptr.device
    V = indptr.numel() - 1
    n = ctypes.c_int64(0)
    _launch(dev, "maxk_warp4_count", _ptr(indptr), V, warp_max_nz, ctypes.byref(n), _stream(dev))
    out = torch.empty(4 * n.value, dtype=torch.int32, device=dev)
    _launch_ws(dev, "maxk_warp4_build", "maxk_warp4_build_workspace_size", (V,),
               (_ptr(indptr), V, warp_max_nz, _ptr(out), n.value))
    return out


def _read_warp4_file(path: str, device="cuda") -> torch.Tensor:
    if not os.path.exists(path):
        raise RuntimeError(f"Cannot open warp4 file: {path}")
    import numpy as np
    data = np.fromfile(path, dtype=np.int32)
    return torch.from_numpy(data).to(device)


def load_warp4_metadata(graph_name: str, num_warps: int = 12, warp_max_nz: int = 64) -> torch.Tensor:
    path = f"kernels/w{num_warps}_nz{warp_max_nz}_warp_4/{graph_name}.warp4"
    return _read_warp4_file(path)


def load_warp4_metadata_csc(graph_name: str, num_warps: int = 12,
                            warp_max_nz: int = 64) -> torch.Tensor:
    path = f"kernels/w{num_warps}_nz{warp_max_nz}_warp_4_csc/{graph_name}.warp4_csc"
    return _read_warp4_file(path)


def _forward_common(indptr, indices, values, num_cols, k, sel, D, row_div, chunk, out, accumulate,
                    validate, dev):
    if values.numel() != indices.numel():
        raise RuntimeError("values and indices must have the same length")
    num_rows = indptr.numel() - 1
    if row_div is not None:
        _need(row_div, "row_div", torch.float32)
        if row_div.numel() != num_rows:
            raise RuntimeError("row_div must have num_rows entries")
    _validate_call(validate, indptr, indices, num_cols, sel, D)
    if out is None:
        if accumulate:
            raise RuntimeError("accumulate=True needs out=")
        out = torch.empty(num_rows, D, dtype=torch.float32, device=dev)
    else:
        _need(out, "out", torch.float32)
        if tuple(out.shape) != (num_rows, D):
            raise RuntimeError("out must be [num_rows, dim_origin]")
    return out, (num_rows, num_cols, indices.numel(), D, k, chunk)


def spgemm_forward(indptr: torch.Tensor, indices: torch.Tensor, values: torch.Tensor,
                   cbsr_val: torch.Tensor, cbsr_idx: torch.Tensor, dim_origin: int,
                   row_div: Optional[torch.Tensor] = None, chunk: int = 0,
                   out: Optional[torch.Tensor] = None, validate: Optional[bool] = None,
                   accumulate: bool = False, edge_sel_out: Optional[torch.Tensor] = None
                   ) -> torch.Tensor:
    for t, n, dt in ((indptr, "indptr", torch.int32), (indices, "indices", torch.int32),
                     (values, "values", torch.float32), (cbsr_val, "input_data", torch.float32),
                     (cbsr_idx, "sparse_selector", torch.uint8)):
        _need(t, n, dt)
    num_cols, k = (cbsr_val.shape[0], cbsr_val.shape[1]) if cbsr_val.dim() == 2 else (0, 0)
    if cbsr_idx.shape != cbsr_val.shape:
        raise RuntimeError("input_data and sparse_selector must have the same [V, k] shape")
    out, shape = _forward_common(indptr, indices, values, num_cols, k, cbsr_idx, int(dim_origin),
                                 row_div, chunk, out, accumulate, validate, cbsr_val.device)
    tail = ()
    if edge_sel_out is not None:
        _need(edge_sel_out, "edge_sel_out", torch.uint8)
        if tuple(edge_sel_out.shape) != (shape[2], k):
            raise RuntimeError("edge_sel_out must be [num_e, k]")
        tail = (_ptr(edge_sel_out),)
    _launch_ws(cbsr_val.device, "maxk_spgemm_forward" + ("_accumulate" if accumulate else "")
               + ("_sel" if tail else ""), "maxk_spgemm_forward_workspace_size", shape,
               (_ptr(indptr), _ptr(indices), _ptr(values), _ptr(cbsr_val), _ptr(cbsr_idx),
                _ptr(row_div), _ptr(out), *shape), tail)
    return out


def edge_weight_grad(indptr: torch.Tensor, indices: torch.Tensor, cbsr_val: torch.Tensor,
                     cbsr_idx: torch.Tensor, grad_output: torch.Tensor,
                     row_div: Optional[torch.Tensor] = None, chunk: int = 0,
                     out: Optional[torch.Tensor] = None,
                     validate: Optional[bool] = None) -> torch.Tensor:
    for t, n, dt in ((indptr, "indptr", torch.int32), (indices, "indices", torch.int32),
                     (cbsr_val, "input_data", torch.float32),
                     (cbsr_idx, "sparse_selector", torch.uint8),
                     (grad_output, "grad_output", torch.float32)):
        _need(t, n, dt)
    if cbsr_val.dim() != 2 or cbsr_idx.shape != cbsr_val.shape:
        raise RuntimeError("input_data and sparse_selector must have the same [V, k] shape")
    num_cols, k = cbsr_val.shape
    num_rows = indptr.numel() - 1
    if grad_output.dim() != 2 or grad_output.shape[0] != num_rows:
        raise RuntimeError("grad_output must be [num_rows, dim_origin]")
    D = grad_output.shape[1]
    if row_div is not None:
        _need(row_div, "row_div", torch.float32)
        if row_div.numel() != num_rows:
            raise RuntimeError("row_div must have num_rows entries")
    _validate_call(validate, indptr, indices, num_cols, cbsr_idx, D)
    E = indices.numel()
    dev = grad_output.device
    if out is None:
        out = torch.empty(E, dtype=torch.float32, device=dev)
    else:
        _need(out, "out", torch.float32)
        if tuple(out.shape) != (E,):
            raise RuntimeError("out must be [num_e]")
    shape = (num_rows, num_cols, E, D, k, chunk)
    _launch_ws(dev, "maxk_edge_weight_grad", "maxk_edge_weight_grad_workspace_size", shape,
               (_ptr(indptr), _ptr(indices), _ptr(cbsr_val), _ptr(cbsr_idx), _ptr(grad_output),
                _ptr(row_div), _ptr(out), *shape))
    return out


MAX_HEADS = 8


def _heads_operands(indptr, indices, cbsr_val, cbsr_idx, row_div, validate, D):
    for t, n, dt in ((indptr, "indptr", torch.int32), (indices, "indices", torch.int32),
                     (cbsr_val, "input_data", torch.float32),
                     (cbsr_idx, "sparse_selector", torch.uint8)):
        _need(t, n, dt)
    if cbsr_val.dim() != 2 or cbsr_idx.shape != cbsr_val.shape:
        raise RuntimeError("input_data and sparse_selector must have the same [V, k] shape")
    num_cols, k = cbsr_val.shape
    num_rows = indptr.numel() - 1
    if row_div is not None:
        _need(row_div, "row_div", torch.float32)
        if row_div.numel() != num_rows:
            raise RuntimeError("row_div must have num_rows entries")
    _validate_call(validate, indptr, indices, num_cols, cbsr_idx, D)
    return num_rows, num_cols, k


def _heads_out(out, shape, dev, what):
    if out is None:
        return torch.empty(*shape, dtype=torch.float32, device=dev)
    _need(out, "out", torch.float32)
    if tuple(out.shape) != tuple(shape):
        raise RuntimeError(f"out must be {what}")
    return out


def spgemm_forward_heads(indptr: torch.Tensor, indices: torch.Tensor, values: torch.Tensor,
                         cbsr_val: torch.Tensor, cbsr_idx: torch.Tensor, dim_origin: int,
                         row_div: Optional[torch.Tensor] = None, chunk: int = 0,
                         out: Optional[torch.Tensor] = None,
                         validate: Optional[bool] = None) -> torch.Tensor:
    D = int(dim_origin)
    _need(values, "values", torch.float32)
    num_rows, num_cols, k = _heads_operands(indptr, indices, cbsr_val, cbsr_idx, row_div,
                                            validate, D)
    E = indices.numel()
    if values.dim() != 2 or values.shape[1] != E or not 1 <= values.shape[0] <= MAX_HEADS:
        raise RuntimeError(f"values must be [H, num_e] with 1 <= H <= {MAX_HEADS}")
    H = values.shape[0]
    dev = cbsr_val.device
    out = _heads_out(out, (H, num_rows, D), dev, "[H, num_rows, dim_origin]")
    shape = (num_rows, num_cols, E, D, k, H, chunk)
    _launch_ws(dev, "maxk_spgemm_forward_heads", "maxk_spgemm_forward_heads_workspace_size", shape,
               (_ptr(indptr), _ptr(indices), _ptr(values), _ptr(cbsr_val), _ptr(cbsr_idx),
                _ptr(row_div), _ptr(out), *shape))
    return out


HEADS_SPARSE_DEGREE = 128


def heads_forward_route(num_rows: int, num_e: int) -> str:
    forced = os.environ.get("MAXK_HEADS_FWD", "")
    if forced in ("heads", "calls"):
        return forced
    return "heads" if num_e < HEADS_SPARSE_DEGREE * num_rows else "calls"


def edge_weight_grad_heads(indptr: torch.Tensor, indices: torch.Tensor, cbsr_val: torch.Tensor,
# ... 270 lines not shown
    _need(row_sum, "row_sum", torch.float32)
    if tuple(row_max.shape) != (H, num_rows) or tuple(row_sum.shape) != (H, num_rows):
        raise RuntimeError("row_max and row_sum must be [H, num_rows]")
    _validate_rows(validate, indptr, indices, num_cols, E)
    dev = s_src.device
    out = _heads_out(out, (H, E), dev, "[H, num_e]")
    shape = (H, num_rows, num_cols, E)
    _launch_ws(dev, "maxk_gat_edge_alpha_heads", "maxk_gat_edge_alpha_heads_workspace_size", shape,
               (_ptr(indptr), _ptr(indices), _ptr(s_dst), _ptr(s_src), float(negative_slope),
                _ptr(row_max), _ptr(row_sum), _ptr(out), *shape))
    return out


def _dot_operands(indptr, indices, q, cbsr_val, cbsr_idx, D, scale, validate):
    _need(q, "q", torch.float32)
    if q.dim() != 3 or not 1 <= q.shape[0] <= MAX_HEADS or q.shape[2] != D:
        raise RuntimeError(f"q must be [H, num_rows, dim_origin] with 1 <= H <= {MAX_HEADS}")
    num_rows, num_cols, k = _heads_operands(indptr, indices, cbsr_val, cbsr_idx, None, validate, D)
    if q.shape[1] != num_rows:
        raise RuntimeError("q must be [H, num_rows, dim_origin]")
    scale = float(scale)
    if not (0.0 < scale < float("inf")):
        raise RuntimeError(f"scale must be finite and > 0, got {scale}")
    return q.shape[0], num_rows, num_cols, k, scale


def dot_attention_heads(indptr: torch.Tensor, indices: torch.Tensor, q: torch.Tensor,
                        cbsr_val: torch.Tensor, cbsr_idx: torch.Tensor, dim_origin: int,
                        scale: float, chunk: int = 0, validate: Optional[bool] = None,
                        out: Optional[torch.Tensor] = None):
    D = int(dim_origin)
    H, num_rows, num_cols, k, scale = _dot_operands(indptr, indices, q, cbsr_val, cbsr_idx, D,
                                                    scale, validate)
    dev = cbsr_val.device
    out = _heads_out(out, (H, num_rows, D), dev, "[H, num_rows, dim_origin]")
    row_max = torch.empty(H, num_rows, dtype=torch.float32, device=dev)
    row_sum = torch.empty(H, num_rows, dtype=torch.float32, device=dev)
    shape = (num_rows, num_cols, indices.numel(), D, k, H, chunk)
    _launch_ws(dev, "maxk_dot_attention_heads", "maxk_dot_attention_heads_workspace_size", shape,
               (_ptr(indptr), _ptr(indices), _ptr(q), scale, _ptr(cbsr_val), _ptr(cbsr_idx),
                _ptr(out), _ptr(row_max), _ptr(row_sum), *shape))
    return out, row_max, row_sum


def dot_edge_alpha_heads(indptr: torch.Tensor, indices: torch.Tensor, q: torch.Tensor,
                         cbsr_val: torch.Tensor, cbsr_idx: torch.Tensor, dim_origin: int,
                         scale: float, row_max: torch.Tensor, row_sum: torch.Tensor,
                         chunk: int = 0, out: Optional[torch.Tensor] = None,
                         validate: Optional[bool] = None) -> torch.Tensor:
    D = int(dim_origin)
    H, num_rows, num_cols, k, scale = _dot_operands(indptr, indices, q, cbsr_val, cbsr_idx, D,
                                                    scale, validate)
    _need(row_max, "row_max", torch.float32)
    _need(row_sum, "row_sum", torch.float32)
    if tuple(row_max.shape) != (H, num_rows) or tuple(row_sum.shape) != (H, num_rows):
        raise RuntimeError("row_max and row_sum must be [H, num_rows]")
    dev = cbsr_val.device
    E = indices.numel()
    out = _heads_out(out, (H, E), dev, "[H, num_e]")
    shape = (num_rows, num_cols, E, D, k, H, chunk)
    _launch_ws(dev, "maxk_dot_edge_alpha_heads", "maxk_dot_edge_alpha_heads_workspace_size", shape,
               (_ptr(indptr), _ptr(indices), _ptr(q), scale, _ptr(cbsr_val), _ptr(cbsr_idx),
                _ptr(row_max), _ptr(row_sum), _ptr(out), *shape))
    return out


def dot_attention_heads_backward(indptr: torch.Tensor, indices: torch.Tensor, q: torch.Tensor,
                                 cbsr_val: torch.Tensor, cbsr_idx: torch.Tensor,
                                 out: torch.Tensor, row_max: torch.Tensor, row_sum: torch.Tensor,
                                 grad_output: torch.Tensor, scale: float, chunk: int = 0,
                                 validate: Optional[bool] = None, plan=None):
    _need(grad_output, "grad_output", torch.float32)
    _need(out, "out", torch.float32)
    _need(q, "q", torch.float32)
    if q.dim() != 3:
        raise RuntimeError(f"q must be [H, num_rows, dim_origin] with 1 <= H <= {MAX_HEADS}")
    D = q.shape[2]
    H, num_rows, num_cols, k, scale = _dot_operands(indptr, indices, q, cbsr_val, cbsr_idx, D,
                                                    scale, validate)
    if tuple(grad_output.shape) != (H, num_rows, D) or tuple(out.shape) != (H, num_rows, D):
        raise RuntimeError("out and grad_output must be [H, num_rows, dim_origin]")
    _need(row_max, "row_max", torch.float32)
    _need(row_sum, "row_sum", torch.float32)
    if tuple(row_max.shape) != (H, num_rows) or tuple(row_sum.shape) != (H, num_rows):
        raise RuntimeError("row_max and row_sum must be [H, num_rows]")
    dev = cbsr_val.device
    col_ptr, csc_eid = plan if plan is not None else transpose_plan(indices, num_cols)
    grad_q = torch.empty(H, num_rows, D, dtype=torch.float32, device=dev)
    grad_cbsr = torch.empty(num_cols, k, dtype=torch.float32, device=dev)
    shape = (num_rows, num_cols, indices.numel(), D, k, H, chunk)
    _launch_ws(dev, "maxk_dot_attention_heads_backward",
               "maxk_dot_attention_heads_backward_workspace_size", shape,
               (_ptr(indptr), _ptr(indices), _ptr(col_ptr), _ptr(csc_eid), _ptr(q), scale,
                _ptr(cbsr_val), _ptr(cbsr_idx), _ptr(out), _ptr(row_max), _ptr(row_sum),
                _ptr(grad_output), _ptr(grad_q), _ptr(grad_cbsr), *shape))
    return grad_q, grad_cbsr


def dot_attention_backward_route(num_heads: int, num_rows: int, num_e: int, k: int) -> str:
    forced = os.environ.get("MAXK_DOT_ATTN_BWD", "")
    if forced in ("fused", "rebuilt"):
        return forced
    return "fused"


def heads_attention_route(num_heads: int, num_rows: int, num_e: int) -> Tuple[str, str]:
    forced = os.environ.get("MAXK_HEADS_ATTN", "")
    if forced in ("fused", "stored"):
        return forced, forced
    dense = num_e >= HEADS_SPARSE_DEGREE * num_rows
    return ("fused" if dense and num_heads >= 2 else "stored"), "stored"


def gat_attention_heads_backward(indptr: torch.Tensor, indices: torch.Tensor,
                                 s_dst: torch.Tensor, s_src: torch.Tensor,
                                 cbsr_val: torch.Tensor, cbsr_idx: torch.Tensor,
                                 out: torch.Tensor, row_max: torch.Tensor, row_sum: torch.Tensor,
                                 grad_output: torch.Tensor, negative_slope: float = 0.2,
                                 chunk: int = 0, validate: Optional[bool] = None, plan=None,
                                 dropout: float = 0.0, seed: int = 0):
    _need(grad_output, "grad_output", torch.float32)
    _need(out, "out", torch.float32)
    if grad_output.dim() != 3 or not 1 <= grad_output.shape[0] <= MAX_HEADS:
        raise RuntimeError(f"grad_output must be [H, num_rows, dim_origin] with 1 <= H <= "
                           f"{MAX_HEADS}")
    D = grad_output.shape[2]
    H, num_rows, num_cols, E = _gat_heads_operands(indptr, indices, s_dst, s_src)
    _, cols2, k = _heads_operands(indptr, indices, cbsr_val, cbsr_idx, None, validate, D)
    if cols2 != num_cols:
        raise RuntimeError("s_src must be [H, num_cols] with num_cols = input_data.shape[0]")
    if tuple(grad_output.shape) != (H, num_rows, D) or tuple(out.shape) != (H, num_rows, D):
        raise RuntimeError("out and grad_output must be [H, num_rows, dim_origin]")
    _need(row_max, "row_max", torch.float32)
    _need(row_sum, "row_sum", torch.float32)
    if tuple(row_max.shape) != (H, num_rows) or tuple(row_sum.shape) != (H, num_rows):
        raise RuntimeError("row_max and row_sum must be [H, num_rows]")
    dev = cbsr_val.device
    col_ptr, csc_eid = plan if plan is not None else transpose_plan(indices, num_cols)
    g_dst = torch.empty(H, num_rows, dtype=torch.float32, device=dev)
    g_src = torch.empty(H, num_cols, dtype=torch.float32, device=dev)
    g_cbsr = torch.empty(num_cols, k, dtype=torch.float32, device=dev)
    shape = (num_rows, num_cols, E, D, k, H, chunk)
    args = (_ptr(indptr), _ptr(indices), _ptr(col_ptr), _ptr(csc_eid), _ptr(s_dst), _ptr(s_src),
            float(negative_slope), _ptr(cbsr_val), _ptr(cbsr_idx), _ptr(out), _ptr(row_max),
            _ptr(row_sum), _ptr(grad_output), _ptr(g_dst), _ptr(g_src), _ptr(g_cbsr), *shape)
    if dropout > 0:
        _launch_ws(dev, "maxk_gat_attention_heads_dropout_backward",
                   "maxk_gat_attention_heads_dropout_backward_workspace_size", shape,
                   args + _dropout_args(dropout, seed))
    else:
        _dropout_args(dropout, seed)
        _launch_ws(dev, "maxk_gat_attention_heads_backward",
                   "maxk_gat_attention_heads_backward_workspace_size", shape, args)
    return g_dst, g_src, g_cbsr


def heads_attention_backward_route(num_heads: int, num_rows: int, num_e: int) -> str:
    forced = os.environ.get("MAXK_HEADS_ATTN_BWD", "")
    if forced in ("fused", "rebuilt"):
        return forced
    return "fused"


def records_ok(num_rows: int, num_cols: int, num_e: int, dim_origin: int, k: int) -> bool:
    return bool(_lib().maxk_records_ok(int(num_rows), int(num_cols), int(num_e), int(dim_origin),
                                       int(k)))


def cbsr_records(cbsr_val: torch.Tensor, cbsr_idx: torch.Tensor, dim_origin: int,
                 out: Optional[torch.Tensor] = None) -> torch.Tensor:
    _need(cbsr_val, "cbsr_val", torch.float32)
    _need(cbsr_idx, "cbsr_idx", torch.uint8)
    if cbsr_val.dim() != 2 or cbsr_idx.shape != cbsr_val.shape:
        raise RuntimeError("cbsr_val / cbsr_idx must be the same [V, k] shape")
    V, k = cbsr_val.shape
    if out is None:
        out = torch.empty(V, 5 * k, dtype=torch.uint8, device=cbsr_val.device)
    elif out.dtype != torch.uint8 or tuple(out.shape) != (V, 5 * k) or not out.is_contiguous():
        raise RuntimeError("out must be a contiguous uint8 [V, 5k] tensor")
    _launch(cbsr_val.device, "maxk_cbsr_records", _ptr(cbsr_val), _ptr(cbsr_idx), _ptr(out), V,
            int(dim_origin), k, _stream(cbsr_val.device))
    return out


def spgemm_forward_records(indptr: torch.Tensor, indices: torch.Tensor, values: torch.Tensor,
                           rec: torch.Tensor, k: int, dim_origin: int,
                           row_div: Optional[torch.Tensor] = None, chunk: int = 0,
                           out: Optional[torch.Tensor] = None,
                           accumulate: bool = False,
                           validate: Optional[bool] = None) -> torch.Tensor:
    _need(indptr, "indptr", torch.int32)
    _need(indices, "indices", torch.int32)
    _need(values, "values", torch.float32)
    _need(rec, "rec", torch.uint8)
    k = int(k)
    if k <= 0 or rec.dim() != 2 or rec.shape[1] != 5 * k:
        raise RuntimeError("rec must be [num_cols, 5k]")
    out, shape = _forward_common(indptr, indices, values, rec.shape[0], k, rec[:, 4 * k:],
                                 int(dim_origin), row_div, chunk, out, accumulate, validate,
                                 rec.device)
    _launch_ws(rec.device, "maxk_spgemm_forward_records", "maxk_spgemm_forward_workspace_size",
               shape, (_ptr(indptr), _ptr(indices), _ptr(values), _ptr(rec), _ptr(row_div),
                       _ptr(out), *shape), (1 if accumulate else 0,))
    return out


_PLAN_CACHE = TensorCache()


def transpose_plan(indices: torch.Tensor, num_cols: int, cache: bool = True):
    _need(indices, "indices", torch.int32)

    def build():
        dev = indices.device
        E = indices.numel()
        col_ptr = torch.empty(num_cols + 1, dtype=torch.int32, device=dev)
        csc_eid = torch.empty(max(E, 1), dtype=torch.int32, device=dev)[:E]
        _launch_ws(dev, "maxk_transpose_plan", "maxk_transpose_plan_workspace_size",
                   (num_cols, E), (_ptr(indices), num_cols, E, _ptr(col_ptr), _ptr(csc_eid)))
        return col_ptr, csc_eid
    return _PLAN_CACHE.get((indices,), (int(num_cols),), build, cache)


_DENSE_CACHE = TensorCache()


def dense_plan(indptr: torch.Tensor, indices: torch.Tensor, values: torch.Tensor, num_cols: int,
               cache: bool = True):
    for t, n, dt in ((indptr, "indptr", torch.int32), (indices, "indices", torch.int32),
                     (values, "values", torch.float32)):
        _need(t, n, dt)

    def build():
        col_ptr, csc_eid = transpose_plan(indices, num_cols, cache=False)
        dev = indices.device
        E = indices.numel()
        t_src = torch.empty(max(E, 1), dtype=torch.int32, device=dev)[:E]
        t_w = torch.empty(max(E, 1), dtype=torch.float32, device=dev)[:E]
        _launch(dev, "maxk_dense_plan", _ptr(indptr), _ptr(values), _ptr(csc_eid),
                indptr.numel() - 1, E, _ptr(t_src), _ptr(t_w), _stream(dev))
        return col_ptr, t_src, t_w
    return _DENSE_CACHE.get((indptr, indices, values), (int(num_cols),), build, cache)


_BSORT_CACHE = TensorCache()


def bsort_plan(indptr: torch.Tensor, indices: torch.Tensor, num_cols: int, k: int,
               cache: bool = True):
    _need(indptr, "indptr", torch.int32)
    _need(indices, "indices", torch.int32)
    L = _lib()
    if int(L.maxk_bsort_window(int(k))) <= 0:
        raise RuntimeError(f"bsort_plan: k must be a multiple of 4 in [4, 256], got {k}")
    shift = int(L.maxk_bucket_shift(int(k)))

    def build():
        dev = indices.device
        E = indices.numel()
        nb = int(L.maxk_bucket_count(num_cols, shift))
        bptr = torch.empty(nb + 1, dtype=torch.int32, device=dev)
        bpos = torch.empty(max(E, 1), dtype=torch.int32, device=dev)[:E]
        bdst = torch.empty(max(E, 1), dtype=torch.uint16, device=dev)[:E]
        wsrc = torch.empty(max(E, 1), dtype=torch.uint16, device=dev)[:E]
        wrow = torch.empty(max(E, 1), dtype=torch.int32, device=dev)[:E]
        _launch_ws(dev, "maxk_bsort_plan", "maxk_bsort_plan_workspace_size", (num_cols, E),
                   (_ptr(indptr), _ptr(indices), indptr.numel() - 1, num_cols, E, int(k), shift,
                    _ptr(bptr), _ptr(bpos), _ptr(bdst), _ptr(wsrc), _ptr(wrow)))
        return bptr, bpos, bdst, wsrc, wrow, shift
    return _BSORT_CACHE.get((indptr, indices), (int(k), int(num_cols)), build, cache)


_PULL_CACHE = TensorCache()


def pull_plan(indptr: torch.Tensor, indices: torch.Tensor, values: torch.Tensor, num_cols: int,
              k: int, dim: int = 256, slices: Optional[int] = None, cache: bool = True,
              shift: Optional[int] = None):
    for t, n, dt in ((indptr, "indptr", torch.int32), (indices, "indices", torch.int32),
                     (values, "values", torch.float32)):
        _need(t, n, dt)
    L = _lib()
    num_rows = indptr.numel() - 1
    shift = int(L.maxk_pull_shift(int(k))) if shift is None else int(shift)
    if shift < 0:
        raise RuntimeError(f"pull_plan: invalid k {k}")
    S = int(slices) if slices else _sized(indices.device, "maxk_pull_slices", num_rows,
                                          int(num_cols), int(dim), int(k))

    def build():
        dev = indices.device
        E = indices.numel()
        nb = int(L.maxk_bucket_count(num_cols, shift))
        tptr = torch.empty(S * nb + 1, dtype=torch.int32, device=dev)
        ent = torch.empty(max(E, 1), 2, dtype=torch.int32, device=dev)[:E]
        _launch_ws(dev, "maxk_pull_plan", "maxk_pull_plan_workspace_size",
                   (num_rows, num_cols, E, shift, S),
                   (_ptr(indptr), _ptr(indices), _ptr(values), num_rows, num_cols, E, shift, S,
                    _ptr(tptr), _ptr(ent)))
        return tptr, ent, shift, S
    return _PULL_CACHE.get((indptr, indices, values), (shift, S, int(num_cols)), build, cache)


_HYBRID_CACHE = TensorCache()
MAXK_PULL_NO_REDUCE, MAXK_PULL_REDUCE_ONLY = 2, 4
MAXK_HYBRID_PRESCALED = 1
_MODE_OF_CODE = {0: "pull", 1: "csc", 3: "hybrid", 4: "atomic", 5: "bsort", 6: "dense"}
_SIDE: dict = {}


def _side_stream(dev: torch.device) -> "torch.cuda.Stream":
    i = dev.index if dev.index is not None else torch.cuda.current_device()
    if i not in _SIDE:
        _SIDE[i] = torch.cuda.Stream(device=i)
    return _SIDE[i]
HYBRID_DENSITY = 0.5
HYBRID_LOCALITY = 1.5


def hybrid_plan(indptr: torch.Tensor, indices: torch.Tensor, values: torch.Tensor,
                num_cols: int, k: int, dim: int = 256, density: Optional[float] = None,
                cache: bool = True):
    if density is None:
        density = float(os.environ.get("MAXK_HYBRID_DENSITY", HYBRID_DENSITY))
    if k % 4:
        raise RuntimeError(f"hybrid backward needs k % 4 == 0, got k={k}")

    def build():
        tptr, ent, shift, S = pull_plan(indptr, indices, values, num_cols, k, dim, cache=False)
        dev = indices.device
        num_rows = indptr.numel() - 1
        E = indices.numel()
        nb = int(_lib().maxk_bucket_count(num_cols, shift))
        nt = S * nb
        i32 = dict(dtype=torch.int32, device=dev)
        tile_list = torch.empty(max(nt, 1), **i32)
        tile_ent = torch.empty(nt + 1, **i32)
        bucket_ptr = torch.empty(nb + 1, **i32)
        bucket_tiles = torch.empty(max(nt, 1), **i32)
        ent_d = torch.empty(max(E, 1), 2, **i32)
        off_ip = torch.empty(num_rows + 1, **i32)
        off_ix = torch.empty(max(E, 1), **i32)
        off_val = torch.empty(max(E, 1), dtype=torch.float32, device=dev)
        counts = (ctypes.c_int64 * 3)()
        _launch_ws(dev, "maxk_hybrid_plan", "maxk_hybrid_plan_workspace_size",
                   (num_rows, num_cols, E, shift, S),
                   (_ptr(indptr), _ptr(indices), _ptr(values), _ptr(tptr), _ptr(ent), num_rows,
                    num_cols, E, shift, S, float(density), _ptr(tile_list), _ptr(tile_ent),
                    _ptr(bucket_ptr), _ptr(bucket_tiles), _ptr(ent_d), _ptr(off_ip), _ptr(off_ix),
                    _ptr(off_val), counts))
        n_t, n_p, n_o = (int(c) for c in counts)
        del tptr, ent
        tile_list, bucket_tiles = tile_list[:n_t].clone(), bucket_tiles[:n_t].clone()
        tile_ent = tile_ent[:n_t + 1].clone()
        ent_d = ent_d[:n_p].clone()
        off_ix, off_val = off_ix[:n_o].clone(), off_val[:n_o].clone()
        off = (off_ip, off_ix, off_val, transpose_plan(off_ix, num_cols, cache=False))
        return tile_list, tile_ent, bucket_ptr, bucket_tiles, ent_d, shift, S, off
    return _HYBRID_CACHE.get((indptr, indices, values),
                             (int(k), int(dim), float(density), int(num_cols)), build, cache)


BWD_MODES = ("auto", "pull", "csc", "atomic", "hybrid", "bsort", "dense")
BSORT_KMAX = 8
_BSORT_WARNED: set = set()


_LOCALITY = TensorCache()
_SCALED = TensorCache()


def _scaled_entries(ent: torch.Tensor, tiles: Optional[torch.Tensor], tile_ent: torch.Tensor,
                    num_rows: int, num_cols: int, shift: int, S: int,
                    row_div: torch.Tensor) -> Optional[torch.Tensor]:
    sc = _SCALED.lookup((ent, row_div), ())
    if sc is not None:
        return sc
    if ent.is_cuda and torch.cuda.is_current_stream_capturing():
        return None

    def build():
        sc = torch.empty_like(ent)
        _launch(ent.device, "maxk_pull_entries_scale", _ptr(ent), _ptr(tiles), _ptr(tile_ent),
                tile_ent.numel() - 1, num_rows, num_cols, shift, S, _ptr(row_div), _ptr(sc),
                _stream(ent.device))
        return sc
    return _SCALED.get((ent, row_div), (), build)


def _prescale() -> bool:
    return os.environ.get("MAXK_PULL_PRESCALE", "1") != "0"


def pull_locality(indptr: torch.Tensor, indices: torch.Tensor, shift: int) -> float:
    def build():
        _need(indptr, "indptr", torch.int32)
        _need(indices, "indices", torch.int32)
        dev = indices.device
        out = ctypes.c_double(0.0)
        ws = torch.empty(8, dtype=torch.uint8, device=dev)
        _launch(dev, "maxk_pull_locality", _ptr(indptr), _ptr(indices), indptr.numel() - 1,
                indices.numel(), int(shift), ctypes.byref(out), _ptr(ws), ws.numel(),
                _stream(dev))
        return float(out.value)
    return _LOCALITY.get((indptr, indices), (int(shift),), build)


def _bwd_mode(mode: Optional[str], k: int = 4, num_e: int = 0, num_cols: int = 0,
              num_rows: Optional[int] = None, dim: Optional[int] = None,
              graph: Optional[tuple] = None) -> str:
    mode = mode or os.environ.get("MAXK_BWD_MODE", "auto")
    if mode not in BWD_MODES:
        raise RuntimeError(f"backward mode must be one of {BWD_MODES}, got {mode!r}")
    if mode == "auto":
        L = _lib()
        rows = num_rows if num_rows else num_cols
        D = -1 if dim is None else int(dim)
        code = int(L.maxk_backward_mode_auto(rows, num_cols, num_e, D, int(k), -1.0))
        if (code in (1, 5) and graph is not None and k % 4 == 0 and num_e > 0
                and rows <= 256 * 65536):
            loc = pull_locality(graph[0], graph[1], int(L.maxk_pull_shift(int(k))))
            code = int(L.maxk_backward_mode_auto(rows, num_cols, num_e, D, int(k), loc))
        mode = _MODE_OF_CODE[code]
    for ok, message in _MODE_NEEDS.get(mode, ()):
        if not ok(k, dim):
            raise RuntimeError(message.format(k=k, dim=dim))
    return mode


def _k4_dim4(k, dim):
    return k % 4 == 0 and (dim is None or dim % 4 == 0)


_MODE_NEEDS = {
    "bsort": ((lambda k, dim: k % 4 == 0, "backward mode 'bsort' needs k % 4 == 0, got k={k}"),),
    "pull": ((lambda k, dim: k % 4 == 0 or k <= 64,
              "backward mode 'pull' needs k % 4 == 0 or k <= 64, got k={k}"),
             (lambda k, dim: dim is None or dim % 4 == 0,
              "backward mode 'pull' needs dim_origin % 4 == 0, got {dim}")),
    "dense": ((_k4_dim4, "backward mode 'dense' needs k % 4 == 0 and dim_origin % 4 == 0, "
                         "got k={k}, dim={dim}"),),
    "hybrid": ((_k4_dim4, "backward mode 'hybrid' needs k % 4 == 0 and dim_origin % 4 == 0, "
                          "got k={k}, dim={dim}"),),
}


def graph_only_mode(k: int, num_e: int, num_cols: int) -> Optional[str]:
    if os.environ.get("MAXK_BWD_MODE", "auto") != "auto":
        return None
    L = _lib()
    k = int(k)
    if (k > 0 and k % 4 == 0 and k <= BSORT_KMAX and num_e > 0 and
            int(L.maxk_bsort_window(k)) * (1 << int(L.maxk_bucket_shift(k))) >= 2 * num_cols):
        return "bsort"
    return "csc"


def backward_plan(indices: torch.Tensor, num_cols: int, k: int, mode: Optional[str] = None,
                  num_rows: Optional[int] = None, indptr: Optional[torch.Tensor] = None,
                  values: Optional[torch.Tensor] = None, dim: Optional[int] = None):
    mode = _bwd_mode(mode, k, indices.numel(), num_cols, num_rows, dim,
                     None if indptr is None else (indptr, indices))
    if mode in ("pull", "hybrid"):
        if indptr is None or values is None:
            raise RuntimeError(f"backward_plan: mode '{mode}' needs indptr= and values=")
        if mode == "hybrid":
            return hybrid_plan(indptr, indices, values, num_cols, k, dim or 256)
        return pull_plan(indptr, indices, values, num_cols, k, dim or 256)
    if mode == "dense":
        if indptr is None or values is None:
            raise RuntimeError("backward_plan: mode 'dense' needs indptr= and values=")
        return dense_plan(indptr, indices, values, num_cols)
    if mode == "bsort":
        if indptr is None:
            raise RuntimeError("backward_plan: mode 'bsort' needs indptr=")
        return bsort_plan(indptr, indices, num_cols, k)
    if mode == "csc":
        return transpose_plan(indices, num_cols)
    return None


def sspmm_backward(indptr: torch.Tensor, indices: torch.Tensor, values: torch.Tensor,
                   grad_output: torch.Tensor, cbsr_idx: torch.Tensor,
                   row_div: Optional[torch.Tensor] = None, chunk: int = 0,
                   out: Optional[torch.Tensor] = None, validate: Optional[bool] = None,
                   mode: Optional[str] = None, plan=None,
                   edge_sel: Optional[torch.Tensor] = None) -> torch.Tensor:
    for t, n, dt in ((indptr, "indptr", torch.int32), (indices, "indices", torch.int32),
                     (values, "values", torch.float32), (grad_output, "grad_output", torch.float32),
                     (cbsr_idx, "sparse_selector", torch.uint8)):
        _need(t, n, dt)
    num_rows = indptr.numel() - 1
    if grad_output.dim() != 2 or grad_output.shape[0] != num_rows:
        raise RuntimeError("grad_output must be [num_rows, dim_origin]")
    D = grad_output.shape[1]
    num_cols, k = cbsr_idx.shape
    if row_div is not None:
        _need(row_div, "row_div", torch.float32)
        if row_div.numel() != num_rows:
            raise RuntimeError("row_div must have num_rows entries")
    _validate_call(validate, indptr, indices, num_cols, cbsr_idx, D)
    dev = grad_output.device
    if out is None:
        out = torch.empty(num_cols, k, dtype=torch.float32, device=dev)
    else:
        _need(out, "out", torch.float32)
        if tuple(out.shape) != (num_cols, k):
            raise RuntimeError("out must be [num_cols, k]")
    E = indices.numel()
    asked = mode or os.environ.get("MAXK_BWD_MODE", "auto")
    mode = _bwd_mode(mode, k, E, num_cols, num_rows, D, (indptr, indices))
    if mode == "dense" and asked == "auto" and not (
            grad_output.data_ptr() % 16 == 0 and out.data_ptr() % 16 == 0
            and cbsr_idx.data_ptr() % 4 == 0):
        mode, plan = "pull", None
    if edge_sel is not None and mode in ("csc", "bsort"):
        _need(edge_sel, "edge_sel", torch.uint8)
        if tuple(edge_sel.shape) != (E, k):
            raise RuntimeError("edge_sel must be [num_e, k]")
    _BWD[mode](indptr, indices, values, grad_output, row_div, cbsr_idx, edge_sel, out,
               (num_rows, num_cols, E, D, k), chunk, plan)
    return out


def _bwd_dense(indptr, indices, values, G, row_div, sel, edge_sel, out, shape, chunk, plan):
    col_ptr, t_src, t_w = (plan if plan is not None
                           else dense_plan(indptr, indices, values, shape[1]))
    _launch_ws(G.device, "maxk_sspmm_backward_dense", "maxk_sspmm_backward_dense_workspace_size",
               (*shape, chunk),
               (_ptr(col_ptr), _ptr(t_src), _ptr(t_w), _ptr(G), _ptr(row_div), _ptr(sel),
                _ptr(out), *shape, chunk))


def _bwd_hybrid(indptr, indices, values, G, row_div, sel, edge_sel, out, shape, chunk, plan):
    num_rows, num_cols, _, D, k = shape
    tl, te, bp, bt, ent, shift, S, off = (plan if plan is not None else
                                         hybrid_plan(indptr, indices, values, num_cols, k, D))
    oip, oix, oval, (ocp, oeid) = off
    n_t, n_off = tl.numel(), oix.numel()
    flags = 0
    if row_div is not None and n_t > 0 and _prescale():
        sc = _scaled_entries(ent, tl, te, num_rows, num_cols, shift, S, row_div)
        if sc is not None:
            ent, flags = sc, MAXK_HYBRID_PRESCALED
    dev = G.device
    size = "maxk_sspmm_backward_hybrid_workspace_size", (num_rows, num_cols, n_off, D, k, n_t)
    if not (n_off > 0 and n_t > 0 and os.environ.get("MAXK_HYBRID_STREAMS", "1") != "0"):
        _launch_ws(dev, "maxk_sspmm_backward_hybrid", *size,
                   (_ptr(G), _ptr(row_div), _ptr(sel), _ptr(tl), _ptr(te), n_t, _ptr(bp), _ptr(bt),
                    _ptr(ent), ent.shape[0], shift, S, _ptr(oip), _ptr(oix), _ptr(oval), n_off,
                    _ptr(ocp), _ptr(oeid), flags, _ptr(out), num_rows, num_cols, D, k),
                   (None, None, None))
        return
    with _on(dev):
        ws = _workspace(dev, size[0], *size[1])
        a = _sized(dev, "maxk_sspmm_backward_csc_workspace_size", num_rows, num_cols, n_off, D,
                   k, 0)
        a = (a + 255) // 256 * 256
        ws_csc, ws_pull = ws[:a], ws[a:]
        tile_div = None if flags & MAXK_HYBRID_PRESCALED else row_div

        def tiles(acc, stream):
            _launch(dev, "maxk_sspmm_backward_pull_tiles", _ptr(G), _ptr(tile_div), _ptr(sel),
                    _ptr(tl), _ptr(te), n_t, _ptr(bp), _ptr(bt), _ptr(ent), shift, S, acc,
                    _ptr(out), num_rows, num_cols, ent.shape[0], D, k, _ptr(ws_pull),
                    ws_pull.numel(), stream)
        main = torch.cuda.current_stream(dev)
        side = _side_stream(dev)
        side.wait_stream(main)
        tiles(MAXK_PULL_NO_REDUCE, ctypes.c_void_p(side.cuda_stream))
        _launch(dev, "maxk_sspmm_backward_csc", _ptr(oip), _ptr(oix), _ptr(oval), _ptr(G),
                _ptr(row_div), _ptr(sel), _ptr(ocp), _ptr(oeid), _ptr(out), num_rows, num_cols,
                n_off, D, k, 0, _ptr(ws_csc), ws_csc.numel(), _stream(dev))
        main.wait_stream(side)
        tiles(MAXK_PULL_REDUCE_ONLY | 1, _stream(dev))


def _bwd_pull(indptr, indices, values, G, row_div, sel, edge_sel, out, shape, chunk, plan):
    num_rows, num_cols, E, D, k = shape
    tptr, ent, shift, S = (plan if plan is not None else
                           pull_plan(indptr, indices, values, num_cols, k, D))
    if row_div is not None and E > 0 and _prescale():
        sc = _scaled_entries(ent, None, tptr, num_rows, num_cols, shift, S, row_div)
        if sc is not None:
            ent, row_div = sc, None
    _launch_ws(G.device, "maxk_sspmm_backward_pull", "maxk_sspmm_backward_pull_workspace_size",
               (num_rows, num_cols, D, k, S),
               (_ptr(G), _ptr(row_div), _ptr(sel), _ptr(tptr), _ptr(ent), shift, S, _ptr(out),
                *shape))


def _bwd_bsort(indptr, indices, values, G, row_div, sel, edge_sel, out, shape, chunk, plan):
    k = shape[4]
    if k > BSORT_KMAX and (id(indptr), k) not in _BSORT_WARNED:
        _BSORT_WARNED.add((id(indptr), k))
        warnings.warn(f"backward mode 'bsort' at k={k} > {BSORT_KMAX} (MAXK_BSORT_KMAX): a "
                      f"window of {int(_lib().maxk_bsort_window(k))} edges holds few rows per "
                      "destination bucket; correct, but csc is faster", stacklevel=3)
    bptr, bpos, bdst, wsrc, wrow, shift = (plan if plan is not None
                                           else bsort_plan(indptr, indices, shape[1], k))
    _launch_ws(G.device, "maxk_sspmm_backward_bsort", "maxk_sspmm_backward_bsort_workspace_size",
               shape,
               (_ptr(indptr), _ptr(indices), _ptr(values), _ptr(G), _ptr(row_div), _ptr(sel),
                _ptr(edge_sel), _ptr(bptr), _ptr(bpos), _ptr(bdst), _ptr(wsrc), _ptr(wrow), shift,
                _ptr(out), *shape))


def _bwd_atomic(indptr, indices, values, G, row_div, sel, edge_sel, out, shape, chunk, plan):
    _launch_ws(G.device, "maxk_sspmm_backward", "maxk_sspmm_backward_workspace_size",
               (*shape, chunk),
               (_ptr(indptr), _ptr(indices), _ptr(values), _ptr(G), _ptr(row_div), _ptr(sel),
                _ptr(out), *shape, chunk))


def _bwd_csc(indptr, indices, values, G, row_div, sel, edge_sel, out, shape, chunk, plan):
    col_ptr, csc_eid = plan if plan is not None else transpose_plan(indices, shape[1])
    name = "maxk_sspmm_backward_csc"
    if edge_sel is not None:
        name, sel = name + "_sel", edge_sel
    _launch_ws(G.device, name, "maxk_sspmm_backward_csc_workspace_size", (*shape, chunk),
               (_ptr(indptr), _ptr(indices), _ptr(values), _ptr(G), _ptr(row_div), _ptr(sel),
                _ptr(col_ptr), _ptr(csc_eid), _ptr(out), *shape, chunk))


_BWD = {"dense": _bwd_dense, "hybrid": _bwd_hybrid, "pull": _bwd_pull, "bsort": _bwd_bsort,
        "atomic": _bwd_atomic, "csc": _bwd_csc}


def sspmm_backward_heads(indptr: torch.Tensor, indices: torch.Tensor, values: torch.Tensor,
                         grad_output: torch.Tensor, cbsr_idx: torch.Tensor,
                         row_div: Optional[torch.Tensor] = None, chunk: int = 0,
                         out: Optional[torch.Tensor] = None, validate: Optional[bool] = None,
                         plan=None) -> torch.Tensor:
    _need(values, "values", torch.float32)
    _need(grad_output, "grad_output", torch.float32)
    _need(indptr, "indptr", torch.int32)
    _need(indices, "indices", torch.int32)
    _need(cbsr_idx, "sparse_selector", torch.uint8)
    if grad_output.dim() != 3 or not 1 <= grad_output.shape[0] <= MAX_HEADS:
        raise RuntimeError(f"grad_output must be [H, num_rows, dim_origin] with 1 <= H <= "
                           f"{MAX_HEADS}")
    H, _, D = grad_output.shape
    if cbsr_idx.dim() != 2:
        raise RuntimeError("sparse_selector must be [V, k]")
    num_cols, k = cbsr_idx.shape
    num_rows = indptr.numel() - 1
    E = indices.numel()
    if grad_output.shape[1] != num_rows:
        raise RuntimeError("grad_output must be [H, num_rows, dim_origin]")
    if tuple(values.shape) != (H, E):
        raise RuntimeError("values must be [H, num_e], H that of grad_output")
    if row_div is not None:
        _need(row_div, "row_div", torch.float32)
        if row_div.numel() != num_rows:
            raise RuntimeError("row_div must have num_rows entries")
    _validate_call(validate, indptr, indices, num_cols, cbsr_idx, D)
    dev = grad_output.device
    out = _heads_out(out, (num_cols, k), dev, "[num_cols, k]")
    col_ptr, csc_eid = plan if plan is not None else transpose_plan(indices, num_cols)
    shape = (num_rows, num_cols, E, D, k, H, chunk)
    _launch_ws(dev, "maxk_sspmm_backward_heads", "maxk_sspmm_backward_heads_workspace_size", shape,
               (_ptr(indptr), _ptr(indices), _ptr(values), _ptr(grad_output), _ptr(row_div),
                _ptr(cbsr_idx), _ptr(col_ptr), _ptr(csc_eid), _ptr(out), *shape))
    return out


HEADS_MAX_COLS = 1 << 24


def heads_backward_route(k: int, num_e: int, num_cols: int, num_rows: int,
                         num_heads: Optional[int] = None) -> str:
    if num_cols >= HEADS_MAX_COLS:
        return "calls"
    forced = os.environ.get("MAXK_HEADS_BWD", "")
    if forced in ("heads", "calls"):
        return forced
    if graph_only_mode(k, num_e, num_cols) is None or num_heads == 1:
        return "calls"
    return "heads"


EDGE_SEL_KMAX = 16


def edge_selectors_wanted(k: int) -> bool:
    mode = os.environ.get("MAXK_EDGE_SEL", "auto")
    if k % 4 or mode == "0":
        return False
    return mode == "1" or k <= EDGE_SEL_KMAX


def edge_selector_mode(indptr: torch.Tensor, indices: torch.Tensor, k: int, num_cols: int,
                       dim: Optional[int] = None, mode: Optional[str] = None) -> Optional[str]:
    if indices.numel() == 0 or not edge_selectors_wanted(k):
        return None
    if mode is None:
        mode = _bwd_mode(None, k, indices.numel(), num_cols, indptr.numel() - 1, dim,
                         (indptr, indices))
    return mode if mode in ("csc", "bsort") else None


def use_edge_selectors(indptr: torch.Tensor, indices: torch.Tensor, k: int, num_cols: int,
                       dim: Optional[int] = None) -> bool:
    return edge_selector_mode(indptr, indices, k, num_cols, dim) is not None


def edge_selectors(indices: torch.Tensor, cbsr_idx: torch.Tensor,
                   out: Optional[torch.Tensor] = None) -> torch.Tensor:
    _need(indices, "indices", torch.int32)
    _need(cbsr_idx, "sparse_selector", torch.uint8)
    E, k = indices.numel(), cbsr_idx.shape[1]
    if out is None:
        out = torch.empty(E, k, dtype=torch.uint8, device=indices.device)
    _launch(indices.device, "maxk_edge_selectors", _ptr(indices), _ptr(cbsr_idx), E, k, _ptr(out),
            _stream(indices.device))
    return out


def spmm_maxk_forward(warp4_metadata: torch.Tensor, indices: torch.Tensor, values: torch.Tensor,
                      input_data: torch.Tensor, sparse_selector: torch.Tensor, num_warps: int,
                      dim_sparse: int, *, dim_origin: int = FULL_DIM,
                      indptr: Optional[torch.Tensor] = None,
                      row_div: Optional[torch.Tensor] = None) -> torch.Tensor:
    _need(input_data, "input_data", torch.float32)
    if input_data.dim() != 2 or input_data.shape[1] != dim_sparse:
        raise RuntimeError("input_data must be [V, dim_sparse]")
    if indptr is None:
        indptr = warp4_to_indptr(warp4_metadata, input_data.shape[0], num_warps)
    return spgemm_forward(indptr, indices, values, input_data, sparse_selector, dim_origin,
                          row_div=row_div)


def spmm_maxk_backward(warp4_metadata: torch.Tensor, indices: torch.Tensor, values: torch.Tensor,
                       grad_output: torch.Tensor, sparse_selector: torch.Tensor, num_warps: int,
                       dim_sparse: int, *, indptr: Optional[torch.Tensor] = None,
                       row_div: Optional[torch.Tensor] = None) -> torch.Tensor:
    _need(grad_output, "grad_output", torch.float32)
    _need(sparse_selector, "sparse_selector", torch.uint8)
    if sparse_selector.dim() != 2 or sparse_selector.shape[1] != dim_sparse:
        raise RuntimeError("sparse_selector must be [V, dim_sparse]")
    if indptr is None:
        indptr = warp4_to_indptr(warp4_metadata, grad_output.shape[0], num_warps)
    return sspmm_backward(indptr, indices, values, grad_output, sparse_selector, row_div=row_div)


def topk_cbsr(x: torch.Tensor, k: int, with_int32: bool = False):
    if x.dim() != 2:
        raise RuntimeError("Input must be 2D tensor")
    if not x.is_cuda:
        raise RuntimeError("Input must be on CUDA")
    if x.stride(1) != 1:
        x = x.contiguous()
    V, D = x.shape
    if not (0 < k <= D):
        raise RuntimeError("Invalid k value")
    dev = x.device
    val = torch.empty(V, k, dtype=x.dtype, device=dev)
    idx = torch.empty(V, k, dtype=torch.uint8, device=dev)
    idx32 = torch.empty(V, k, dtype=torch.int32, device=dev) if with_int32 else None
    if x.dtype == torch.float32:
        name = "maxk_topk_cbsr"
    elif x.dtype == torch.uint8:
        name = "maxk_topk_cbsr_u8"
    else:
        raise RuntimeError("Input must be float32 or uint8")
    check = _checks_topk_rows(dev)
    _launch(dev, name, _ptr(x), x.stride(0), _ptr(val), _ptr(idx), _ptr(idx32), V, D, k,
            _stream(dev))
    if check:
        _check_topk_rows(dev, name)
    return (val, idx, idx32) if with_int32 else (val, idx)


def topk_error_rows(device=None, reset: bool = True) -> int:
    dev = torch.device("cuda", torch.cuda.current_device()) if device is None else device
    n = ctypes.c_int64(0)
    _launch(dev, "maxk_topk_error_rows", ctypes.byref(n), 1 if reset else 0, _stream(dev))
    return int(n.value)


def _checks_topk_rows(dev) -> bool:
    if not _validate_default() or torch.cuda.is_current_stream_capturing():
        return False
    topk_error_rows(dev, reset=True)
    return True


def _check_topk_rows(dev, name):
    bad = topk_error_rows(dev)
    if bad:
        raise RuntimeError(f"{name}: {bad} rows took other than k winners (kernel bug)")


def topk_u8_reference(input: torch.Tensor, k: int) -> Tuple[torch.Tensor, torch.Tensor]:
    _need(input, "input", torch.uint8)
    if input.dim() != 2 or input.shape[1] != 256:
        raise RuntimeError("the reference's uint8 top-k takes [N, 256] rows")
    if not 0 < k <= 256:
        raise RuntimeError("Invalid k value")
    N = input.shape[0]
    val = torch.empty(N, k, dtype=torch.uint8, device=input.device)
    idx = torch.empty(N, k, dtype=torch.uint8, device=input.device)
    _launch(input.device, "maxk_topk_u8_reference", _ptr(input), _ptr(val), _ptr(idx), N, 256,
            int(k), _stream(input.device))
    return val, idx


def cuda_topk_maxk(input: torch.Tensor, k: int,
                   reference_compat: bool = False) -> Tuple[torch.Tensor, torch.Tensor]:
    if input.dtype != torch.uint8:
        raise RuntimeError("Input must be uint8 tensor")
    if reference_compat:
        return topk_u8_reference(input, k)
    return topk_cbsr(input, k)


def cuda_topk_maxk_float(input: torch.Tensor, k: int,
                         reference_compat: bool = False) -> Tuple[torch.Tensor, torch.Tensor]:
    if not reference_compat:
        val, _, idx32 = topk_cbsr(input, k, with_int32=True)
        return val, idx32
    if input.dtype == torch.float32:
        q = torch.clamp((input * 255.0).round(), 0, 255).to(torch.uint8)
        v8, i8 = topk_u8_reference(q.contiguous(), k)
        table = (torch.arange(256, dtype=torch.float32) / 255.0).to(input.device)
        return table[v8.long()], i8.to(torch.int32)
    if input.dtype == torch.uint8:
        v8, i8 = topk_u8_reference(input, k)
        return v8, i8.to(torch.int32)
    raise RuntimeError("Input must be float32 or uint8")


def prepare_cbsr_format_maxk(features: torch.Tensor, maxk: int):
    return cuda_topk_maxk_float(features, maxk)


def cbsr_scatter_dense(cbsr_val: torch.Tensor, cbsr_idx: torch.Tensor, dim_origin: int,
                       out: Optional[torch.Tensor] = None) -> torch.Tensor:
    _need(cbsr_val, "cbsr_val", torch.float32)
    _need(cbsr_idx, "cbsr_idx", torch.uint8)
    V, k = cbsr_val.shape
    dev = cbsr_val.device
    if out is None:
        out = torch.empty(V, dim_origin, dtype=torch.float32, device=dev)
    _launch(dev, "maxk_cbsr_scatter_dense", _ptr(cbsr_val), _ptr(cbsr_idx), _ptr(out), V,
            dim_origin, k, _stream(dev))
    return out


def topk_cbsr_dense(x: torch.Tensor, k: int):
    if not (isinstance(x, torch.Tensor) and x.is_cuda and x.dtype == torch.float32):
        raise RuntimeError("x must be a float32 CUDA tensor")
    if x.dim() != 2:
        raise RuntimeError("Input must be 2D tensor")
    if x.stride(1) != 1:
        x = x.contiguous()
    V, D = x.shape
    if not (0 < k <= D):
        raise RuntimeError("Invalid k value")
    dev = x.device
    val = torch.empty(V, k, dtype=torch.float32, device=dev)
    idx = torch.empty(V, k, dtype=torch.uint8, device=dev)
    dense = torch.empty(V, D, dtype=torch.float32, device=dev)
    check = _checks_topk_rows(dev)
    _launch(dev, "maxk_topk_cbsr_dense", _ptr(x), x.stride(0), _ptr(val), _ptr(idx), _ptr(dense),
            V, D, k, _stream(dev))
    if check:
        _check_topk_rows(dev, "maxk_topk_cbsr_dense")
    return dense, val, idx


def topk_backward(grad_val: Optional[torch.Tensor], grad_dense: Optional[torch.Tensor],
                  cbsr_idx: torch.Tensor, dim_origin: int,
                  out: Optional[torch.Tensor] = None) -> torch.Tensor:
    _need(cbsr_idx, "cbsr_idx", torch.uint8)
    V, k = cbsr_idx.shape
    dev = cbsr_idx.device
    if grad_val is not None:
        _need(grad_val, "grad_val", torch.float32)
        if tuple(grad_val.shape) != (V, k):
            raise RuntimeError("grad_val must be [V, k]")
    if grad_dense is not None:
        _need(grad_dense, "grad_dense", torch.float32)
        if tuple(grad_dense.shape) != (V, dim_origin):
# ... 124 lines not shown
```

spgemm-prunning_amd/maxk_cuda_kernels/_capi.py:

```python
from __future__ import annotations

import ctypes
import os

_HERE = os.path.dirname(os.path.abspath(__file__))
LIB_PATH = os.environ.get(
    "MAXK_HIP_LIB", os.path.join(os.path.dirname(_HERE), "lib", "libmaxk_hip.so"))

MAXK_OK = 0
ERRORS = {-1: "invalid argument", -2: "HIP error", -3: "no HIP device", -4: "rocSPARSE error"}

_p = ctypes.c_void_p
_i32 = ctypes.c_int32
_i64 = ctypes.c_int64
_sz = ctypes.c_size_t

SIGNATURES = {
    "maxk_version": (ctypes.c_int, []),
    "maxk_last_error": (ctypes.c_char_p, []),
    "maxk_device_count": (ctypes.c_int, []),
    "maxk_source_digest": (ctypes.c_char_p, []),
    "maxk_build_config": (ctypes.c_char_p, []),
    "maxk_spgemm_forward_workspace_size": (_sz, [_i64, _i64, _i64, _i32, _i32, _i32]),
    "maxk_spgemm_forward": (ctypes.c_int, [_p, _p, _p, _p, _p, _p, _p, _i64, _i64, _i64,
                                           _i32, _i32, _i32, _p, _sz, _p]),
    "maxk_spgemm_forward_sel": (ctypes.c_int, [_p, _p, _p, _p, _p, _p, _p, _i64, _i64, _i64,
                                           _i32, _i32, _i32, _p, _sz, _p, _p]),
    "maxk_spgemm_forward_accumulate": (ctypes.c_int, [_p, _p, _p, _p, _p, _p, _p, _i64, _i64, _i64,
                                           _i32, _i32, _i32, _p, _sz, _p]),
    "maxk_spgemm_forward_accumulate_sel": (ctypes.c_int, [_p, _p, _p, _p, _p, _p, _p, _i64, _i64,
                                                          _i64, _i32, _i32, _i32, _p, _sz, _p,
                                                          _p]),
    "maxk_records_ok": (ctypes.c_int, [_i64, _i64, _i64, _i32, _i32]),
    "maxk_cbsr_records": (ctypes.c_int, [_p, _p, _p, _i64, _i32, _i32, _p]),
    "maxk_spgemm_forward_records": (ctypes.c_int, [_p, _p, _p, _p, _p, _p, _i64, _i64, _i64, _i32,
                                                   _i32, _i32, _p, _sz, _p, _i32]),
    "maxk_edge_weight_grad_workspace_size": (_sz, [_i64, _i64, _i64, _i32, _i32, _i32]),
    "maxk_edge_weight_grad": (ctypes.c_int, [_p, _p, _p, _p, _p, _p, _p, _i64, _i64, _i64,
                                             _i32, _i32, _i32, _p, _sz, _p]),
    "maxk_spgemm_forward_heads_workspace_size": (_sz, [_i64, _i64, _i64, _i32, _i32, _i32, _i32]),
    "maxk_spgemm_forward_heads": (ctypes.c_int, [_p, _p, _p, _p, _p, _p, _p, _i64, _i64, _i64,
                                                 _i32, _i32, _i32, _i32, _p, _sz, _p]),
    "maxk_edge_weight_grad_heads_workspace_size": (_sz, [_i64, _i64, _i64, _i32, _i32, _i32,
                                                         _i32]),
    "maxk_edge_weight_grad_heads": (ctypes.c_int, [_p, _p, _p, _p, _p, _p, _p, _i64, _i64, _i64,
                                                   _i32, _i32, _i32, _i32, _p, _sz, _p]),
    "maxk_edge_softmax_workspace_size": (_sz, [_i64, _i64, _i64, _i32]),
    "maxk_edge_softmax": (ctypes.c_int, [_p, _p, _p, _i64, _i64, _i64, _i32, _p, _sz, _p]),
    "maxk_edge_softmax_backward_workspace_size": (_sz, [_i64, _i64, _i64, _i32]),
    "maxk_edge_softmax_backward": (ctypes.c_int, [_p, _p, _p, _p, _i64, _i64, _i64, _i32, _p, _sz,
                                                  _p]),
    "maxk_gat_edge_softmax_workspace_size": (_sz, [_i64, _i64, _i64, _i32]),
    "maxk_gat_edge_softmax": (ctypes.c_int, [_p, _p, _p, _p, ctypes.c_float, _p, _i64, _i64, _i64,
                                             _i32, _p, _sz, _p]),
    "maxk_gat_edge_softmax_backward_workspace_size": (_sz, [_i64, _i64, _i64, _i32]),
    "maxk_gat_edge_softmax_backward": (ctypes.c_int, [_p, _p, _p, _p, _p, _p, ctypes.c_float, _p,
                                                      _p, _p, _p, _i64, _i64, _i64, _i32, _p, _sz,
                                                      _p]),
    "maxk_gat_edge_softmax_heads_workspace_size": (_sz, [_i32, _i64, _i64, _i64, _i32]),
    "maxk_gat_edge_softmax_heads": (ctypes.c_int, [_p, _p, _p, _p, ctypes.c_float, _p, _i32, _i64,
                                                   _i64, _i64, _i32, _p, _sz, _p]),
    "maxk_gat_edge_softmax_heads_backward_workspace_size": (_sz, [_i32, _i64, _i64, _i64, _i32]),
    "maxk_gat_edge_softmax_heads_backward": (ctypes.c_int, [_p, _p, _p, _p, _p, _p,
                                                            ctypes.c_float, _p, _p, _p, _p, _i32,
                                                            _i64, _i64, _i64, _i32, _p, _sz, _p]),
    "maxk_gat_attention_heads_workspace_size": (_sz, [_i64, _i64, _i64, _i32, _i32, _i32, _i32]),
    "maxk_gat_attention_heads": (ctypes.c_int, [_p, _p, _p, _p, ctypes.c_float, _p, _p, _p, _p, _p,
                                                _i64, _i64, _i64, _i32, _i32, _i32, _i32, _p, _sz,
                                                _p]),
    "maxk_gat_edge_alpha_heads_workspace_size": (_sz, [_i32, _i64, _i64, _i64]),
    "maxk_gat_edge_alpha_heads": (ctypes.c_int, [_p, _p, _p, _p, ctypes.c_float, _p, _p, _p, _i32,
                                                 _i64, _i64, _i64, _p, _sz, _p]),
    "maxk_gat_attention_heads_backward_workspace_size": (_sz, [_i64, _i64, _i64, _i32, _i32, _i32,
                                                               _i32]),
    "maxk_gat_attention_heads_backward": (ctypes.c_int, [_p, _p, _p, _p, _p, _p, ctypes.c_float,
                                                         _p, _p, _p, _p, _p, _p, _p, _p, _p,
                                                         _i64, _i64, _i64, _i32, _i32, _i32, _i32,
                                                         _p, _sz, _p]),
    "maxk_edge_dropout_heads": (ctypes.c_int, [_p, _p, _i32, _i64, ctypes.c_float,
                                               ctypes.c_uint64, _p]),
    "maxk_gat_attention_heads_dropout_workspace_size": (_sz, [_i64, _i64, _i64, _i32, _i32, _i32,
                                                              _i32]),
    "maxk_gat_attention_heads_dropout": (ctypes.c_int, [_p, _p, _p, _p, ctypes.c_float, _p, _p, _p,
                                                        _p, _p, _i64, _i64, _i64, _i32, _i32, _i32,
                                                        _i32, ctypes.c_float, ctypes.c_uint64, _p,
                                                        _sz, _p]),
    "maxk_gat_attention_heads_dropout_backward_workspace_size": (_sz, [_i64, _i64, _i64, _i32,
                                                                       _i32, _i32, _i32]),
    "maxk_gat_attention_heads_dropout_backward": (ctypes.c_int, [_p, _p, _p, _p, _p, _p,
                                                                 ctypes.c_float, _p, _p, _p, _p,
                                                                 _p, _p, _p, _p, _p, _i64, _i64,
                                                                 _i64, _i32, _i32, _i32, _i32,
                                                                 ctypes.c_float, ctypes.c_uint64,
                                                                 _p, _sz, _p]),
    "maxk_dot_attention_heads_workspace_size": (_sz, [_i64, _i64, _i64, _i32, _i32, _i32, _i32]),
    "maxk_dot_attention_heads": (ctypes.c_int, [_p, _p, _p, ctypes.c_float, _p, _p, _p, _p, _p,
                                                _i64, _i64, _i64, _i32, _i32, _i32, _i32, _p, _sz,
                                                _p]),
    "maxk_dot_edge_alpha_heads_workspace_size": (_sz, [_i64, _i64, _i64, _i32, _i32, _i32, _i32]),
    "maxk_dot_edge_alpha_heads": (ctypes.c_int, [_p, _p, _p, ctypes.c_float, _p, _p, _p, _p, _p,
                                                 _i64, _i64, _i64, _i32, _i32, _i32, _i32, _p, _sz,
                                                 _p]),
    "maxk_dot_attention_heads_backward_workspace_size": (_sz, [_i64, _i64, _i64, _i32, _i32, _i32,
                                                               _i32]),
    "maxk_dot_attention_heads_backward": (ctypes.c_int, [_p, _p, _p, _p, _p, ctypes.c_float, _p,
                                                         _p, _p, _p, _p, _p, _p, _p, _i64, _i64,
                                                         _i64, _i32, _i32, _i32, _i32, _p, _sz,
                                                         _p]),
    "maxk_sspmm_backward_workspace_size": (_sz, [_i64, _i64, _i64, _i32, _i32, _i32]),
    "maxk_sspmm_backward": (ctypes.c_int, [_p, _p, _p, _p, _p, _p, _p, _i64, _i64, _i64,
                                           _i32, _i32, _i32, _p, _sz, _p]),
    "maxk_sspmm_backward_csc_workspace_size": (_sz, [_i64, _i64, _i64, _i32, _i32, _i32]),
    "maxk_sspmm_backward_csc": (ctypes.c_int, [_p, _p, _p, _p, _p, _p, _p, _p, _p, _i64, _i64,
                                               _i64, _i32, _i32, _i32, _p, _sz, _p]),
    "maxk_sspmm_backward_csc_sel": (ctypes.c_int, [_p, _p, _p, _p, _p, _p, _p, _p, _p, _i64, _i64,
                                               _i64, _i32, _i32, _i32, _p, _sz, _p]),
    "maxk_sspmm_backward_heads_workspace_size": (_sz, [_i64, _i64, _i64, _i32, _i32, _i32, _i32]),
    "maxk_sspmm_backward_heads": (ctypes.c_int, [_p, _p, _p, _p, _p, _p, _p, _p, _p, _i64, _i64,
                                                 _i64, _i32, _i32, _i32, _i32, _p, _sz, _p]),
    "maxk_edge_selectors": (ctypes.c_int, [_p, _p, _i64, _i32, _p, _p]),
    "maxk_edge_selectors_blocks": (_i64, [_i64]),
    "maxk_transpose_plan_workspace_size": (_sz, [_i64, _i64]),
    "maxk_transpose_plan": (ctypes.c_int, [_p, _i64, _i64, _p, _p, _p, _sz, _p]),
    "maxk_dense_route": (ctypes.c_int, [_i32, _i32]),
    "maxk_dense_plan": (ctypes.c_int, [_p, _p, _p, _i64, _i64, _p, _p, _p]),
    "maxk_sspmm_backward_dense_workspace_size": (_sz, [_i64, _i64, _i64, _i32, _i32, _i32]),
    "maxk_sspmm_backward_dense": (ctypes.c_int, [_p, _p, _p, _p, _p, _p, _p, _i64, _i64, _i64,
                                                 _i32, _i32, _i32, _p, _sz, _p]),
    "maxk_bucket_shift": (ctypes.c_int, [_i32]),
    "maxk_bucket_count": (_i64, [_i64, _i32]),
    "maxk_bsort_window": (_i32, [_i32]),
    "maxk_bsort_plan_workspace_size": (_sz, [_i64, _i64]),
    "maxk_bsort_plan": (ctypes.c_int, [_p, _p, _i64, _i64, _i64, _i32, _i32, _p, _p, _p, _p, _p,
                                       _p, _sz, _p]),
    "maxk_sspmm_backward_bsort_workspace_size": (_sz, [_i64, _i64, _i64, _i32, _i32]),
    "maxk_sspmm_backward_bsort": (ctypes.c_int, [_p, _p, _p, _p, _p, _p, _p, _p, _p, _p, _p, _p,
                                                 _i32,
                                                 _p, _i64, _i64, _i64, _i32, _i32, _p, _sz, _p]),
    "maxk_sspmm_backward_pull_workspace_size": (_sz, [_i64, _i64, _i32, _i32, _i32]),
    "maxk_sspmm_backward_pull": (ctypes.c_int, [_p, _p, _p, _p, _p, _i32, _i32, _p, _i64, _i64,
                                                _i64, _i32, _i32, _p, _sz, _p]),
    "maxk_sspmm_backward_pull_tiles_workspace_size": (_sz, [_i64, _i64, _i32, _i32, _i32]),
    "maxk_sspmm_backward_pull_tiles": (ctypes.c_int, [_p, _p, _p, _p, _p, _i32, _p, _p, _p, _i32,
                                                      _i32, _i32, _p, _i64, _i64, _i64, _i32,
                                                      _i32, _p, _sz, _p]),
    "maxk_pull_shift": (ctypes.c_int, [_i32]),
    "maxk_pull_slices": (ctypes.c_int, [_i64, _i64, _i32, _i32]),
    "maxk_pull_plan_workspace_size": (_sz, [_i64, _i64, _i64, _i32, _i32]),
    "maxk_pull_plan": (ctypes.c_int, [_p, _p, _p, _i64, _i64, _i64, _i32, _i32, _p, _p, _p, _sz,
                                      _p]),
    "maxk_backward_mode_auto": (ctypes.c_int, [_i64, _i64, _i64, _i32, _i32, ctypes.c_double]),
    "maxk_pull_locality": (ctypes.c_int, [_p, _p, _i64, _i64, _i32,
                                          ctypes.POINTER(ctypes.c_double), _p, _sz, _p]),
    "maxk_hybrid_plan_workspace_size": (_sz, [_i64, _i64, _i64, _i32, _i32]),
    "maxk_hybrid_plan": (ctypes.c_int, [_p, _p, _p, _p, _p, _i64, _i64, _i64, _i32, _i32,
                                        ctypes.c_float, _p, _p, _p, _p, _p, _p, _p, _p,
                                        ctypes.POINTER(_i64), _p, _sz, _p]),
    "maxk_pull_entries_scale": (ctypes.c_int, [_p, _p, _p, _i64, _i64, _i64, _i32, _i32, _p, _p,
                                               _p]),
    "maxk_sspmm_backward_hybrid_workspace_size": (_sz, [_i64, _i64, _i64, _i32, _i32, _i64]),
    "maxk_sspmm_backward_hybrid": (ctypes.c_int, [_p, _p, _p, _p, _p, _i32, _p, _p, _p, _i64,
                                                  _i32, _i32, _p, _p, _p, _i64, _p, _p, _i32, _p,
                                                  _i64, _i64, _i32, _i32, _p, _sz, _p, _p, _p,
                                                  _p]),
    "maxk_topk_cbsr": (ctypes.c_int, [_p, _i64, _p, _p, _p, _i64, _i32, _i32, _p]),
    "maxk_topk_cbsr_u8": (ctypes.c_int, [_p, _i64, _p, _p, _p, _i64, _i32, _i32, _p]),
    "maxk_topk_u8_reference": (ctypes.c_int, [_p, _p, _p, _i64, _i32, _i32, _p]),
    "maxk_topk_error_rows": (ctypes.c_int, [_p, _i32, _p]),
    "maxk_cbsr_scatter_dense": (ctypes.c_int, [_p, _p, _p, _i64, _i32, _i32, _p]),
    "maxk_topk_cbsr_dense": (ctypes.c_int, [_p, _i64, _p, _p, _p, _i64, _i32, _i32, _p]),
    "maxk_topk_backward": (ctypes.c_int, [_p, _p, _p, _p, _i64, _i32, _i32, _p]),
    "maxk_warp4_count": (ctypes.c_int, [_p, _i64, _i32, ctypes.POINTER(_i64), _p]),
    "maxk_warp4_build_workspace_size": (_sz, [_i64]),
    "maxk_warp4_build": (ctypes.c_int, [_p, _i64, _i32, _p, _i64, _p, _sz, _p]),
    "maxk_warp4_to_row_ptr": (ctypes.c_int, [_p, _i64, _i64, _p, _p]),
    "maxk_dense_spmm_plan_create": (ctypes.c_int, [ctypes.POINTER(_p), _p, _p, _p, _p, _p,
                                                   _i64, _i64, _i64, _i32, _i32, _p]),
    "maxk_dense_spmm_run": (ctypes.c_int, [_p, _p]),
    "maxk_dense_spmm_bind": (ctypes.c_int, [_p, _p, _p]),
    "maxk_dense_spmm_plan_destroy": (ctypes.c_int, [_p]),
}

_lib = None
_load_error = None


def load():
    global _lib, _load_error
    if _lib is not None:
        return _lib
    if _load_error is not None:
        raise ImportError(_load_error)
    if not os.path.exists(LIB_PATH):
        _load_error = (f"libmaxk_hip.so not found at {LIB_PATH}; build it with "
                       f"`make -C spgemm-prunning_amd` (hipcc, gfx950)")
        raise ImportError(_load_error)
    try:
        lib = ctypes.CDLL(LIB_PATH)
    except OSError as exc:
        _load_error = f"cannot load {LIB_PATH}: {exc}"
        raise ImportError(_load_error) from exc
    for name, (res, args) in SIGNATURES.items():
        fn = getattr(lib, name)
        fn.restype = res
        fn.argtypes = args
    _lib = lib
    return lib


def check(rc: int, what: str) -> None:
    if rc != MAXK_OK:
        msg = _lib.maxk_last_error().decode(errors="replace") if _lib is not None else ""
        raise RuntimeError(f"{what} failed ({ERRORS.get(rc, rc)}): {msg}")
```

Baseline: 61.75.

## Add streaming pull backward with variable-width column buckets sized to CU count

Adds a stream form of the pull backward kernel. Column buckets have variable widths so that bucket×part work items fill whole rounds of compute units. Each block walks its whole entry range in runs and writes grad_cbsr directly, which removes the separate tile-output buffer and reduce kernel. Entries use a packed row/column encoding that depends on the bucket shift, and there is a matching prescale kernel. The path is on by default when the bucket-count heuristic applies, at the cost of a new planner and possible load imbalance across buckets.

```diff
diff --git a/include/maxk_hip.h b/include/maxk_hip.h
--- a/include/maxk_hip.h
+++ b/include/maxk_hip.h
@@ -329,6 +329,30 @@
                    int64_t num_rows, int64_t num_cols, int64_t num_e, int32_t bucket_shift,
                    int32_t slices, int32_t *tile_ptr, uint32_t *ent, void *workspace,
                    size_t workspace_bytes, void *stream);
+
+int64_t maxk_pull_stream_buckets(int64_t num_rows, int64_t num_cols, int64_t num_e,
+                                 int32_t dim_origin, int32_t dim_k, int32_t cus);
+int maxk_pull_stream_slices(int64_t num_rows, int64_t num_cols, int32_t dim_origin,
+                            int32_t dim_k);
+size_t maxk_pull_stream_plan_workspace_size(int64_t num_cols, int64_t num_e, int32_t n_buckets,
+                                            int32_t slices);
+int maxk_pull_stream_plan(const int32_t *row_ptr, const int32_t *col_idx, const float *edge_val,
+                          int64_t num_rows, int64_t num_cols, int64_t num_e, int32_t dim_k,
+                          int32_t n_buckets, int32_t slices, int32_t *bucket_col,
+                          int32_t *grp_ptr, uint32_t *ent, void *workspace,
+                          size_t workspace_bytes, void *stream);
+int maxk_pull_stream_entries_scale(const uint32_t *ent, int64_t num_e, int64_t num_rows,
+                                   int32_t dim_k, const float *row_div, uint32_t *ent_out,
+                                   void *stream);
+size_t maxk_sspmm_backward_pull_stream_workspace_size(int64_t num_rows, int64_t num_cols,
+                                                      int32_t dim_origin, int32_t dim_k);
+int maxk_sspmm_backward_pull_stream(const float *grad_out, const float *row_div,
+                                    const uint8_t *cbsr_idx, const int32_t *bucket_col,
+                                    const int32_t *grp_ptr, const uint32_t *ent,
+                                    int32_t n_buckets, float *grad_cbsr, int64_t num_rows,
+                                    int64_t num_cols, int64_t num_e, int32_t dim_origin,
+                                    int32_t dim_k, void *workspace, size_t workspace_bytes,
+                                    void *stream);
 
 int maxk_dense_route(int32_t dim_origin, int32_t dim_k);
 int maxk_dense_plan(const int32_t *row_ptr, const float *edge_val, const int32_t *csc_eid,
diff --git a/spgemm-prunning_amd/csrc/sspmm_pull.hip b/spgemm-prunning_amd/csrc/sspmm_pull.hip
--- a/spgemm-prunning_amd/csrc/sspmm_pull.hip
+++ b/spgemm-prunning_amd/csrc/sspmm_pull.hip
@@ -243,7 +243,7 @@
     }
 }
 
-template <int LR, int U, bool FULLD, int VPL>
+template <int LR, int U, bool FULLD, int VPL, bool GROW = false>
 __device__ __forceinline__ void pull_q_entries(double *acc, const uint8_t *sel_lds,
                                                __amdgpu_buffer_rsrc_t grs,
                                                __amdgpu_buffer_rsrc_t ers, int n_e, int D,
@@ -297,7 +297,9 @@
 #pragma unroll
         for (int u = 0; u < U; ++u) {
             ok[u] = eb + u * EPI < n_e && qok;
-            const int d = ok[u] ? (int)(ex[u] >> 16) : idle;
+            const int d = !ok[u] ? idle
+                          : GROW ? (int)(ex[u] & ((1u << shift) - 1u))
+                                 : (int)(ex[u] >> 16);
             dc[u] = d * ks + VPL * q * ok[u];
             const uint8_t *sp = sel_lds + d * kp + (ok[u] ? q * VPL : 0);
             if constexpr (VPL == 8)
@@ -310,7 +312,8 @@
         }
 #pragma unroll
         for (int u = 0; u < U; ++u) {
-            const uint32_t ro = ok[u] ? (ex[u] & 0xffffu) * Db : 0x80000000u;
+            const uint32_t ro =
+                ok[u] ? (GROW ? ex[u] >> shift : ex[u] & 0xffffu) * Db : 0x80000000u;
 #pragma unroll
             for (int i = 0; i < VPL; ++i) {
                 const uint32_t c = VPL == 8 ? (uint32_t)(sv[u] >> (8 * i)) & 255u
@@ -368,12 +371,10 @@
 struct PullSel {
     uint4 v[kSelRegs];
 };
-__device__ __forceinline__ PullSel pull_sel_load(const uint8_t *__restrict__ sel_q, int64_t c0,
-                                                 int64_t num_cols, int k, int kp, int h,
-                                                 int shift) {
+__device__ __forceinline__ PullSel pull_sel_load_rows(const uint8_t *__restrict__ sel_q,
+                                                      int64_t c0, int rows, int k, int kp, int h) {
     PullSel r;
     const int tid = threadIdx.x;
-    const int rows = num_cols - c0 < (1 << shift) ? (int)(num_cols - c0) : (1 << shift);
     const uint8_t *__restrict__ selg = sel_q + c0 * k + h * kp;
 #pragma unroll
     for (int m = 0; m < kSelRegs; ++m) {
@@ -399,6 +400,12 @@
         r.v[m] = x;
     }
     return r;
+}
+__device__ __forceinline__ PullSel pull_sel_load(const uint8_t *__restrict__ sel_q, int64_t c0,
+                                                 int64_t num_cols, int k, int kp, int h,
+                                                 int shift) {
+    const int rows = num_cols - c0 < (1 << shift) ? (int)(num_cols - c0) : (1 << shift);
+    return pull_sel_load_rows(sel_q, c0, rows, k, kp, h);
 }
 __device__ __forceinline__ void pull_sel_store(uint8_t *sel_lds, const PullSel &r, int kp,
                                                int shift) {
@@ -449,6 +456,65 @@
     pull_q_entries<LR, U, FULLD, VPL>(acc, sel_lds, grs, ers, p.s1 - p.s0, D, kp, shift);
     __syncthreads();
     pull_flush(acc, tile_out, ti, h, k, kp, shift);
+}
+
+#ifndef MAXK_PULL_STREAM_RUN
+#define MAXK_PULL_STREAM_RUN 16384
+#endif
+template <int LR, int U, bool FULLD, int VPL, int STREAM>
+__global__ __launch_bounds__(1024) void pull_q_kernel(
+    const float *__restrict__ Gp, const uint8_t *__restrict__ sel_q,
+    const uint8_t *__restrict__ lmap, const int32_t *__restrict__ bucket_col,
+    const int32_t *__restrict__ grp_ptr, const uint2 *__restrict__ ent,
+    float *__restrict__ grad_cbsr, int64_t num_cols, int n_buckets, int64_t num_rows, int D,
+    int k, int kp, int shift) {
+    static_assert(STREAM == 1, "the stream form");
+    extern __shared__ double acc[];
+    const int tid = threadIdx.x;
+    const int ks = pull_ks(kp, shift);
+    const int H = k / kp;
+    int b, h;
+    if (kXcds % H == 0) {
+        const int x = blockIdx.x % kXcds, per = gridDim.x / kXcds;
+        h = x % H;
+        b = (x / H) * per + blockIdx.x / kXcds;
+        if (b >= n_buckets) return;
+    } else {
+        const int tp = xcd_contiguous_block(blockIdx.x, gridDim.x);
+        if (tp >= n_buckets * H) return;
+        b = tp / H, h = tp % H;
+    }
+    const int64_t c0 = bucket_col[b];
+    int64_t c1 = bucket_col[b + 1];
+    c1 = c1 > num_cols ? num_cols : c1;
+    int width = c1 > c0 && c0 >= 0 ? (int)(c1 - c0) : 0;
+    width = width > (1 << shift) ? (1 << shift) : width;
+    const int s0 = grp_ptr[b];
+    const int n_e = width > 0 && grp_ptr[b + 1] > s0 ? grp_ptr[b + 1] - s0 : 0;
+    uint8_t *sel_lds = reinterpret_cast<uint8_t *>(acc + (ks << shift));
+    for (int i = tid; i < (ks << shift); i += 1024) acc[i] = 0.0;
+    pull_sel_store(sel_lds, pull_sel_load_rows(sel_q, c0, width, k, kp, h), kp, shift);
+    __syncthreads();
+    const auto grs = wave_buffer(Gp, (uint32_t)num_rows * (uint32_t)D * 4u);
+    constexpr int RUN = MAXK_PULL_STREAM_RUN;
+    for (int e0 = 0; e0 < n_e; e0 += RUN) {
+        const int n = n_e - e0 < RUN ? n_e - e0 : RUN;
+        const auto ers = wave_buffer(ent + s0 + e0, (uint32_t)n * 8u);
+        pull_q_entries<LR, U, FULLD, VPL, true>(acc, sel_lds, grs, ers, n, D, kp, shift);
+        __syncthreads();
+    }
+    const int w4 = kp / 4;
+    for (int i4 = tid; i4 < width * w4; i4 += 1024) {
+        const int d = i4 / w4, s4 = i4 % w4;
+        const double *a = &acc[d * ks + 4 * s4];
+        const size_t r0 = (size_t)(c0 + d) * k;
+        const uint32_t m = *reinterpret_cast<const uint32_t *>(lmap + r0 + h * kp + 4 * s4);
+        float *row = grad_cbsr + r0;
+        row[m & 255u] = (float)a[0];
+        row[(m >> 8) & 255u] = (float)a[1];
+        row[(m >> 16) & 255u] = (float)a[2];
+        row[m >> 24] = (float)a[3];
+    }
 }
 
 __global__ __launch_bounds__(kBlock) void pull_reduce_kernel(const float *__restrict__ tile_out,
@@ -536,6 +602,26 @@
     L.lmap_off = L.sel_off + nsel;
     L.total = L.lmap_off + nsel;
     return L;
+}
+
+int pull_vpl(int kp, int parts) {
+    return kp != 8 ? 4 : MAXK_PULL_VPL8 ? MAXK_PULL_VPL8 : parts == 1 ? 8 : 4;
+}
+
+int launch_pull_sel(const uint8_t *cbsr_idx, uint8_t *sel_q, uint8_t *lm, int64_t num_cols, int k,
+                    int kp, int vpl, hipStream_t s) {
+    if (MAXK_PULL_SEL4 && (reinterpret_cast<uintptr_t>(cbsr_idx) & 3) == 0) {
+        const int nd4 = kBlock / (k / 4);
+        hipLaunchKernelGGL(pull_sel4_kernel, dim3((unsigned)ceil_div(num_cols, nd4)),
+                           dim3(kBlock), 0, s, cbsr_idx, sel_q, lm, num_cols, k, kp, vpl);
+        MAXK_LAUNCHED("pull_sel4_kernel");
+    } else {
+        const int nd = kBlock / k;
+        hipLaunchKernelGGL(pull_sel_kernel, dim3((unsigned)ceil_div(num_cols, nd)),
+                           dim3(kBlock), 0, s, cbsr_idx, sel_q, lm, num_cols, k, kp, vpl);
+        MAXK_LAUNCHED("pull_sel_kernel");
+    }
+    return MAXK_OK;
 }
 
 int pull_impl(const float *grad_out, const float *row_div, const uint8_t *cbsr_idx,
@@ -602,20 +688,10 @@
         const size_t lds_q = pull_lds_bytes(pull_ks(kp, bucket_shift), kp, bucket_shift);
         uint8_t *sel_q = reinterpret_cast<uint8_t *>(ws + L.sel_off);
         uint8_t *lm = reinterpret_cast<uint8_t *>(ws + L.lmap_off);
-        const int nd = kBlock / k;
-        const int vpl = kp != 8 ? 4 : MAXK_PULL_VPL8 ? MAXK_PULL_VPL8 : parts == 1 ? 8 : 4;
+        const int vpl = pull_vpl(kp, parts);
         lmap = lm;
         if (!front) goto reduce;
-        if (MAXK_PULL_SEL4 && (reinterpret_cast<uintptr_t>(cbsr_idx) & 3) == 0) {
-            const int nd4 = kBlock / (k / 4);
-            hipLaunchKernelGGL(pull_sel4_kernel, dim3((unsigned)ceil_div(num_cols, nd4)),
-                               dim3(kBlock), 0, s, cbsr_idx, sel_q, lm, num_cols, k, kp, vpl);
-            MAXK_LAUNCHED("pull_sel4_kernel");
-        } else {
-            hipLaunchKernelGGL(pull_sel_kernel, dim3((unsigned)ceil_div(num_cols, nd)),
-                               dim3(kBlock), 0, s, cbsr_idx, sel_q, lm, num_cols, k, kp, vpl);
-            MAXK_LAUNCHED("pull_sel_kernel");
-        }
+        if (int rc = launch_pull_sel(cbsr_idx, sel_q, lm, num_cols, k, kp, vpl, s)) return rc;
         const int64_t work = tiles * parts;
         const bool fulld = dim_origin == kMaxDim;
         const unsigned grid = (unsigned)(MAXK_PULL_XCD ? xcd_grid(work) : work);
@@ -662,10 +738,129 @@
     MAXK_LAUNCHED("pull_reduce_kernel");
     return MAXK_OK;
 }
+
+#ifndef MAXK_PULL_STREAM_NARROW
+#define MAXK_PULL_STREAM_NARROW 125
+#endif
+
+int64_t stream_buckets(int64_t num_rows, int64_t num_cols, int64_t num_e, int D, int k,
+                       int64_t cus) {
+    if (!MAXK_PULL_Q || MAXK_PULL_STREAM_NARROW <= 0) return 0;
+    if (num_rows <= 0 || num_cols <= 0 || D <= 0 || D > kMaxDim || D % 4 || k <= 0 || k > D || k % 4)
+        return 0;
+    if (num_rows >= (1LL << 31) || num_cols >= (1LL << 31) || num_cols * (int64_t)k >= (1LL << 31))
+        return 0;
+    const int shift = maxk_pull_shift(k);
+    const int H = shift >= 4 && shift <= 15 ? pull_parts(k, shift) : 0;
+    if (H <= 0) return 0;
+    if (num_rows * D * 4 >= (1LL << 31) || num_e >= (1LL << 28)) return 0;
+    int row_bits = 0;
+    while ((1LL << row_bits) < num_rows) ++row_bits;
+    if (row_bits + shift > 32) return 0;
+    if (cus <= 0) cus = device_cus();
+    const int64_t nb_min = (num_cols + (1LL << shift) - 1) >> shift;
+    const int64_t rounds = (nb_min * H + cus - 1) / cus;
+    const int64_t nb = rounds * cus / H;
+    if (nb < nb_min || nb * H >= (1LL << 24)) return 0;
+    return (nb - nb_min) * 1000 <= nb * MAXK_PULL_STREAM_NARROW ? nb : 0;
+}
+
+int pull_stream_impl(const float *grad_out, const float *row_div, const uint8_t *cbsr_idx,
+                     const int32_t *bucket_col, const int32_t *grp_ptr, const uint32_t *ent,
+                     int32_t n_buckets, float *grad_cbsr, int64_t num_rows, int64_t num_cols,
+                     int64_t num_e, int32_t dim_origin, int32_t dim_k, void *workspace,
+                     size_t workspace_bytes, void *stream) {
+    if (int rc = check_common(num_rows, num_cols, num_e, dim_origin, dim_k, 0)) return rc;
+    const int k = dim_k;
+    MAXK_REQUIRE(MAXK_PULL_Q && k % 4 == 0 && dim_origin % 4 == 0,
+                 "stream pull needs dim_k %% 4 == 0 and dim_origin %% 4 == 0, got %d, %d", k,
+                 dim_origin);
+    const int shift = maxk_pull_shift(k);
+    const int parts = shift >= 4 && shift <= 15 ? pull_parts(k, shift) : 0;
+    MAXK_REQUIRE(parts > 0, "no part count fits dim_k %d", k);
+    MAXK_REQUIRE(num_rows * dim_origin * 4 < (1LL << 31), "stream pull: G of 2 GiB or more");
+    MAXK_REQUIRE(num_e < (1LL << 28), "stream pull: 2^28 entries or more");
+    int row_bits = 0;
+    while ((1LL << row_bits) < num_rows) ++row_bits;
+    MAXK_REQUIRE(row_bits + shift <= 32, "stream pull: %d row bits + %d column bits exceed 32",
+                 row_bits, shift);
+    MAXK_REQUIRE(n_buckets >= 1 && (int64_t)n_buckets * parts < (1LL << 24) &&
+                     ((int64_t)n_buckets << shift) >= num_cols,
+                 "n_buckets %d out of range", n_buckets);
+    hipStream_t s = as_stream(stream);
+    if (num_cols == 0) return MAXK_OK;
+    MAXK_REQUIRE(grad_cbsr && bucket_col && grp_ptr && cbsr_idx,
+                 "grad_cbsr/bucket_col/grp_ptr/selector pointers must not be NULL");
+    MAXK_REQUIRE(num_e == 0 || (grad_out && ent), "grad/plan pointers must not be NULL");
+    const PullLayout L = pull_layout(num_rows, num_cols, dim_origin, k, 0, shift);
+    MAXK_REQUIRE(workspace && workspace_bytes >= L.total,
+                 "workspace too small: need %zu bytes, got %zu", L.total, workspace_bytes);
+    char *ws = reinterpret_cast<char *>(workspace);
+    const float *Gp = grad_out;
+    if (row_div && num_rows > 0 && num_e > 0) {
+        const int64_t n4 = num_rows * dim_origin / 4;
+        hipLaunchKernelGGL(gprime_kernel, dim3((unsigned)ceil_div(n4, kBlock)), dim3(kBlock), 0,
+                           s, grad_out, row_div, reinterpret_cast<float *>(workspace), n4,
+                           dim_origin / 4);
+        MAXK_LAUNCHED("gprime_kernel");
+        Gp = reinterpret_cast<const float *>(workspace);
+    }
+    const int kp = k / parts;
+    const int vpl = pull_vpl(kp, parts);
+    uint8_t *sel_q = reinterpret_cast<uint8_t *>(ws + L.sel_off);
+    uint8_t *lm = reinterpret_cast<uint8_t *>(ws + L.lmap_off);
+    if (int rc = launch_pull_sel(cbsr_idx, sel_q, lm, num_cols, k, kp, vpl, s)) return rc;
+    const size_t lds_q = pull_lds_bytes(pull_ks(kp, shift), kp, shift);
+    const unsigned grid = (unsigned)xcd_grid((int64_t)n_buckets * parts);
+    const bool fulld = dim_origin == kMaxDim;
+    const int lr = vpl == 4 ? lanes_per_edge(kp / 4) : kp / vpl;
+    const bool ok = with_lanes(lr, [&](auto lr_c) {
+        with_const<2, 4, 8>(vpl, [&](auto vpl_c) {
+            with_const<0, 1>(fulld, [&](auto fd_c) {
+                constexpr int LR = decltype(lr_c)::value, VPL = decltype(vpl_c)::value;
+                if constexpr (VPL == 4 || LR * VPL == 8)
+                    hipLaunchKernelGGL(
+                        (pull_q_kernel<LR, MAXK_PULL_QU, decltype(fd_c)::value, VPL, 1>),
+                        dim3(grid), dim3(1024), lds_q, s, Gp, sel_q, lm, bucket_col, grp_ptr,
+                        reinterpret_cast<const uint2 *>(ent), grad_cbsr, num_cols, (int)n_buckets,
+                        num_rows, dim_origin, k, kp, shift);
+            });
+        });
+    });
+    if (!ok) return bad_lanes(lr);
+    MAXK_LAUNCHED("pull_q_kernel");
+    return MAXK_OK;
+}
 }
 }
 
 using namespace maxk;
+
+extern "C" int64_t maxk_pull_stream_buckets(int64_t num_rows, int64_t num_cols, int64_t num_e,
+                                            int32_t dim_origin, int32_t dim_k, int32_t cus) {
+    return stream_buckets(num_rows, num_cols, num_e, dim_origin, dim_k, cus);
+}
+
+extern "C" size_t maxk_sspmm_backward_pull_stream_workspace_size(int64_t num_rows,
+                                                                 int64_t num_cols,
+                                                                 int32_t dim_origin,
+                                                                 int32_t dim_k) {
+    if (num_rows < 0 || num_cols < 0 || dim_origin <= 0 || dim_k <= 0) return 0;
+    return pull_layout(num_rows, num_cols, dim_origin, dim_k, 0, 0).total;
+}
+
+extern "C" int maxk_sspmm_backward_pull_stream(const float *grad_out, const float *row_div,
+                                               const uint8_t *cbsr_idx, const int32_t *bucket_col,
+                                               const int32_t *grp_ptr, const uint32_t *ent,
+                                               int32_t n_buckets, float *grad_cbsr,
+                                               int64_t num_rows, int64_t num_cols, int64_t num_e,
+                                               int32_t dim_origin, int32_t dim_k, void *workspace,
+                                               size_t workspace_bytes, void *stream) {
+    clear_error();
+    return pull_stream_impl(grad_out, row_div, cbsr_idx, bucket_col, grp_ptr, ent, n_buckets,
+                            grad_cbsr, num_rows, num_cols, num_e, dim_origin, dim_k, workspace,
+                            workspace_bytes, stream);
+}
 
 extern "C" size_t maxk_sspmm_backward_pull_workspace_size(int64_t num_rows, int64_t num_cols,
                                                           int32_t dim_origin, int32_t dim_k,
diff --git a/spgemm-prunning_amd/csrc/transpose.hip b/spgemm-prunning_amd/csrc/transpose.hip
--- a/spgemm-prunning_amd/csrc/transpose.hip
+++ b/spgemm-prunning_amd/csrc/transpose.hip
@@ -443,3 +443,220 @@
     MAXK_LAUNCHED("tile_ptr_kernel");
     return MAXK_OK;
 }
+
+namespace maxk {
+namespace {
+
+__global__ void stream_indeg_kernel(const int32_t *__restrict__ col_idx, int64_t num_e,
+                                    int num_cols, int32_t *__restrict__ indeg) {
+    const int64_t e = (int64_t)blockIdx.x * blockDim.x + threadIdx.x;
+    if (e >= num_e) return;
+    const int c = col_idx[e];
+    if (c >= 0 && c < num_cols) atomicAdd(&indeg[c], 1);
+}
+
+__global__ __launch_bounds__(1024) void stream_bounds_kernel(const int32_t *__restrict__ cpre,
+                                                             int num_cols, int nb, int cap,
+                                                             int32_t *__restrict__ bucket_col) {
+    const int64_t total = cpre[num_cols];
+    for (int i = threadIdx.x; i <= nb; i += blockDim.x) {
+        const int64_t want = total * i / nb;
+        int lo = 0, hi = num_cols;
+        while (lo < hi) {
+            const int mid = (int)(((int64_t)lo + hi) >> 1);
+            if (cpre[mid] >= want) hi = mid; else lo = mid + 1;
+        }
+        if (lo > 0 && want - cpre[lo - 1] < cpre[lo] - want) --lo;
+        bucket_col[i] = i == 0 ? 0 : i == nb ? num_cols : lo;
+    }
+    __syncthreads();
+    if (threadIdx.x != 0) return;
+    int64_t prev = 0;
+    for (int i = 1; i < nb; ++i) {
+        int64_t lo = (int64_t)num_cols - (int64_t)(nb - i) * cap;
+        lo = lo < prev ? prev : lo;
+        const int64_t hi = prev + cap < num_cols ? prev + cap : num_cols;
+        int64_t c = bucket_col[i];
+        c = c < lo ? lo : (c > hi ? hi : c);
+        bucket_col[i] = (int32_t)c;
+        prev = c;
+    }
+}
+
+__device__ __forceinline__ int stream_bucket_of(const int32_t *__restrict__ bucket_col, int nb,
+                                                int c) {
+    int lo = 0, hi = nb - 1;
+    while (lo < hi) {
+        const int mid = (lo + hi + 1) >> 1;
+        if (bucket_col[mid] <= c) lo = mid; else hi = mid - 1;
+    }
+    return lo;
+}
+
+__global__ void stream_key_kernel(const int32_t *__restrict__ row_ptr,
+                                  const int32_t *__restrict__ col_idx, int num_rows,
+                                  int num_cols, int rows_per_slice, int slices,
+                                  const int32_t *__restrict__ bucket_col, int nb,
+                                  int32_t *__restrict__ keys, int32_t *__restrict__ row_of) {
+    const int r = (int)(((int64_t)blockIdx.x * blockDim.x + threadIdx.x) / kWave);
+    if (r >= num_rows) return;
+    const int lane = lane_id();
+    const int b = row_ptr[r], e = row_ptr[r + 1];
+    const int sl = r / rows_per_slice;
+    for (int i = b + lane; i < e; i += kWave) {
+        int c = col_idx[i];
+        c = c < 0 ? 0 : (c >= num_cols ? num_cols - 1 : c);
+        keys[i] = stream_bucket_of(bucket_col, nb, c) * slices + sl;
+        row_of[i] = r;
+    }
+}
+
+__global__ void stream_gather_kernel(const int32_t *__restrict__ eid,
+                                     const int32_t *__restrict__ sorted_keys,
+                                     const int32_t *__restrict__ row_of,
+                                     const int32_t *__restrict__ col_idx,
+                                     const float *__restrict__ edge_val, int64_t num_e, int cbits,
+                                     int slices, const int32_t *__restrict__ bucket_col,
+                                     uint2 *__restrict__ ent) {
+    const int64_t i = (int64_t)blockIdx.x * blockDim.x + threadIdx.x;
+    if (i >= num_e) return;
+    const int e = eid[i];
+    const uint32_t dst = (uint32_t)(col_idx[e] - bucket_col[sorted_keys[i] / slices]);
+    ent[i] = make_uint2(((uint32_t)row_of[e] << cbits) | (dst & ((1u << cbits) - 1u)),
+                        __float_as_uint(edge_val[e]));
+}
+
+__global__ void stream_grp_ptr_kernel(const int32_t *__restrict__ sorted_keys, int64_t num_e,
+                                      int slices, int nb, int32_t *__restrict__ grp_ptr) {
+    const int64_t t = (int64_t)blockIdx.x * blockDim.x + threadIdx.x;
+    if (t > num_e) return;
+    int cur = t < num_e ? sorted_keys[t] / slices : nb;
+    int prev = t == 0 ? -1 : sorted_keys[t - 1] / slices;
+    cur = cur > nb ? nb : cur;
+    prev = prev > nb ? nb : prev;
+    for (int x = prev + 1; x <= cur; ++x) grp_ptr[x] = (int32_t)t;
+}
+
+__global__ void stream_scale_kernel(const uint2 *__restrict__ ent, int64_t num_e, int cbits,
+                                    int64_t num_rows, const float *__restrict__ row_div,
+                                    uint2 *__restrict__ ent_out) {
+    const int64_t i = (int64_t)blockIdx.x * blockDim.x + threadIdx.x;
+    if (i >= num_e) return;
+    const uint2 v = ent[i];
+    const int64_t r = v.x >> cbits;
+    const float w = r < num_rows ? __uint_as_float(v.y) / row_div[r] : 0.0f;
+    ent_out[i] = make_uint2(v.x, __float_as_uint(w));
+}
+
+size_t stream_scan_bytes(int64_t n) {
+    size_t bytes = 0;
+    (void)hipcub::DeviceScan::ExclusiveSum(nullptr, bytes, (const int32_t *)nullptr,
+                                           (int32_t *)nullptr, (int)n);
+    return bytes;
+}
+
+}
+}
+
+extern "C" int maxk_pull_stream_slices(int64_t, int64_t, int32_t, int32_t) { return 1; }
+
+extern "C" size_t maxk_pull_stream_plan_workspace_size(int64_t num_cols, int64_t num_e,
+                                                       int32_t n_buckets, int32_t slices) {
+    if (num_cols < 0 || num_e <= 0 || n_buckets <= 0 || slices <= 0) return 0;
+    const size_t sort = pull_sort_temp_bytes(num_e, (int64_t)n_buckets * slices);
+    const size_t scan = stream_scan_bytes(num_cols + 1);
+    return 5 * al256((size_t)num_e * 4) + 2 * al256((size_t)(num_cols + 1) * 4) +
+           al256(sort > scan ? sort : scan);
+}
+
+extern "C" int maxk_pull_stream_plan(const int32_t *row_ptr, const int32_t *col_idx,
+                                     const float *edge_val, int64_t num_rows, int64_t num_cols,
+                                     int64_t num_e, int32_t dim_k, int32_t n_buckets,
+                                     int32_t slices, int32_t *bucket_col, int32_t *grp_ptr,
+                                     uint32_t *ent, void *workspace, size_t workspace_bytes,
+                                     void *stream) {
+    clear_error();
+    MAXK_REQUIRE(num_rows >= 0 && num_rows < (1LL << 31), "num_rows out of range");
+    MAXK_REQUIRE(num_cols >= 1 && num_cols < (1LL << 31), "num_cols out of range");
+    MAXK_REQUIRE(num_e >= 0 && num_e < (1LL << 28), "num_e out of range");
+    const int cbits = maxk_pull_shift(dim_k);
+    MAXK_REQUIRE(dim_k > 0 && dim_k % 4 == 0 && cbits >= 4 && cbits <= 15,
+                 "stream plan needs dim_k %% 4 == 0, got %d", dim_k);
+    int row_bits = 0;
+    while ((1LL << row_bits) < num_rows) ++row_bits;
+    MAXK_REQUIRE(row_bits + cbits <= 32, "%d row bits + %d column bits exceed 32", row_bits, cbits);
+    MAXK_REQUIRE(n_buckets >= 1 && ((int64_t)n_buckets << cbits) >= num_cols,
+                 "%d buckets of 2^%d columns do not cover %lld columns", n_buckets, cbits,
+                 (long long)num_cols);
+    MAXK_REQUIRE(slices >= 1 && (int64_t)slices * n_buckets < (1LL << 31),
+                 "slices %d out of range", slices);
+    MAXK_REQUIRE(bucket_col && grp_ptr, "bucket_col/grp_ptr must not be NULL");
+    hipStream_t s = as_stream(stream);
+    const int nb = n_buckets;
+    if (num_e == 0 || num_rows == 0) {
+        const size_t need = al256((size_t)(num_cols + 1) * 4);
+        MAXK_REQUIRE(workspace && workspace_bytes >= need, "workspace too small: need %zu", need);
+        int32_t *cpre = reinterpret_cast<int32_t *>(workspace);
+        if (int rc = zero_words(cpre, num_cols + 1, s)) return rc;
+        hipLaunchKernelGGL(stream_bounds_kernel, dim3(1), dim3(1024), 0, s, cpre, (int)num_cols,
+                           nb, 1 << cbits, bucket_col);
+        MAXK_LAUNCHED("stream_bounds_kernel");
+        return zero_words(grp_ptr, nb + 1, s);
+    }
+    MAXK_REQUIRE(row_ptr && col_idx && edge_val && ent, "CSR/plan pointers must not be NULL");
+    const size_t need = maxk_pull_stream_plan_workspace_size(num_cols, num_e, n_buckets, slices);
+    MAXK_REQUIRE(workspace && workspace_bytes >= need, "workspace too small: need %zu", need);
+    char *ws = reinterpret_cast<char *>(workspace);
+    const size_t a = al256((size_t)num_e * 4), c = al256((size_t)(num_cols + 1) * 4);
+    int32_t *keys = reinterpret_cast<int32_t *>(ws);
+    int32_t *keys_out = reinterpret_cast<int32_t *>(ws + a);
+    int32_t *ids = reinterpret_cast<int32_t *>(ws + 2 * a);
+    int32_t *eid = reinterpret_cast<int32_t *>(ws + 3 * a);
+    int32_t *row_of = reinterpret_cast<int32_t *>(ws + 4 * a);
+    int32_t *indeg = reinterpret_cast<int32_t *>(ws + 5 * a);
+    int32_t *cpre = reinterpret_cast<int32_t *>(ws + 5 * a + c);
+    void *tmp = ws + 5 * a + 2 * c;
+    size_t tmp_bytes = workspace_bytes - (5 * a + 2 * c);
+    const dim3 ge((unsigned)ceil_div(num_e, kBlock));
+    if (int rc = zero_words(indeg, num_cols + 1, s)) return rc;
+    hipLaunchKernelGGL(stream_indeg_kernel, ge, dim3(kBlock), 0, s, col_idx, num_e,
+                       (int)num_cols, indeg);
+    MAXK_LAUNCHED("stream_indeg_kernel");
+    MAXK_HIP(hipcub::DeviceScan::ExclusiveSum(tmp, tmp_bytes, indeg, cpre, (int)(num_cols + 1), s));
+    hipLaunchKernelGGL(stream_bounds_kernel, dim3(1), dim3(1024), 0, s, cpre, (int)num_cols, nb,
+                       1 << cbits, bucket_col);
+    MAXK_LAUNCHED("stream_bounds_kernel");
+    const int rps = (int)((num_rows + slices - 1) / slices);
+    hipLaunchKernelGGL(stream_key_kernel, dim3((unsigned)ceil_div(num_rows * kWave, kBlock)),
+                       dim3(kBlock), 0, s, row_ptr, col_idx, (int)num_rows, (int)num_cols, rps,
+                       (int)slices, bucket_col, nb, keys, row_of);
+    MAXK_LAUNCHED("stream_key_kernel");
+    hipLaunchKernelGGL(iota_kernel, ge, dim3(kBlock), 0, s, ids, num_e);
+    MAXK_LAUNCHED("iota_kernel");
+    MAXK_HIP(hipcub::DeviceRadixSort::SortPairs(tmp, tmp_bytes, keys, keys_out, ids, eid,
+                                                (int)num_e, 0, key_bits((int64_t)nb * slices), s));
+    hipLaunchKernelGGL(stream_gather_kernel, ge, dim3(kBlock), 0, s, eid, keys_out, row_of,
+                       col_idx, edge_val, num_e, cbits, (int)slices, bucket_col,
+                       reinterpret_cast<uint2 *>(ent));
+    MAXK_LAUNCHED("stream_gather_kernel");
+    hipLaunchKernelGGL(stream_grp_ptr_kernel, dim3((unsigned)ceil_div(num_e + 1, kBlock)),
+                       dim3(kBlock), 0, s, keys_out, num_e, (int)slices, nb, grp_ptr);
+    MAXK_LAUNCHED("stream_grp_ptr_kernel");
+    return MAXK_OK;
+}
+
+extern "C" int maxk_pull_stream_entries_scale(const uint32_t *ent, int64_t num_e,
+                                              int64_t num_rows, int32_t dim_k,
+                                              const float *row_div, uint32_t *ent_out,
+                                              void *stream) {
+    clear_error();
+    const int cbits = maxk_pull_shift(dim_k);
+    MAXK_REQUIRE(num_e >= 0 && num_rows >= 0 && cbits >= 4, "sizes out of range");
+    if (num_e == 0) return MAXK_OK;
+    MAXK_REQUIRE(ent && row_div && ent_out, "pointers must not be NULL");
+    hipLaunchKernelGGL(stream_scale_kernel, dim3((unsigned)ceil_div(num_e, kBlock)), dim3(kBlock),
+                       0, as_stream(stream), reinterpret_cast<const uint2 *>(ent), num_e, cbits,
+                       num_rows, row_div, reinterpret_cast<uint2 *>(ent_out));
+    MAXK_LAUNCHED("stream_scale_kernel");
+    return MAXK_OK;
+}
diff --git a/spgemm-prunning_amd/maxk_cuda_kernels/__init__.py b/spgemm-prunning_amd/maxk_cuda_kernels/__init__.py
--- a/spgemm-prunning_amd/maxk_cuda_kernels/__init__.py
+++ b/spgemm-prunning_amd/maxk_cuda_kernels/__init__.py
@@ -4,7 +4,7 @@
 import ctypes
 import os
 import warnings
-from typing import List, Optional, Tuple
+from typing import List, NamedTuple, Optional, Tuple
 
 import torch
 
@@ -36,6 +36,7 @@
     "version", "device_count",
     "transpose_plan", "bsort_plan", "pull_plan", "edge_selector_mode", "backward_plan", "BWD_MODES",
     "dense_plan", "hybrid_plan", "pull_locality", "edge_selectors_wanted",
+    "pull_stream_plan", "pull_stream_buckets", "PullStreamPlan",
 ]
 
 FULL_DIM = 256
@@ -912,6 +913,78 @@
     return _PULL_CACHE.get((indptr, indices, values), (shift, S, int(num_cols)), build, cache)
 
 
+_STREAM_CACHE = TensorCache()
+
+
+class PullStreamPlan(NamedTuple):
+    bucket_col: torch.Tensor
+    grp_ptr: torch.Tensor
+    ent: torch.Tensor
+    shift: int
+    n_buckets: int
+    slices: int
+
+
+def _stream_on() -> bool:
+    return os.environ.get("MAXK_PULL_STREAM", "1") != "0"
+
+
+def pull_stream_buckets(dev, num_rows: int, num_cols: int, num_e: int, dim: int, k: int) -> int:
+    if not _stream_on():
+        return 0
+    return _sized(dev, "maxk_pull_stream_buckets", int(num_rows), int(num_cols), int(num_e),
+                  int(dim), int(k), 0)
+
+
+def pull_stream_plan(indptr: torch.Tensor, indices: torch.Tensor, values: torch.Tensor,
+                     num_cols: int, k: int, dim: int = 256, groups: Optional[int] = None,
+                     slices: Optional[int] = None, cache: bool = True) -> PullStreamPlan:
+    for t, n, dt in ((indptr, "indptr", torch.int32), (indices, "indices", torch.int32),
+                     (values, "values", torch.float32)):
+        _need(t, n, dt)
+    L = _lib()
+    dev = indices.device
+    num_rows, E = indptr.numel() - 1, indices.numel()
+    shift = int(L.maxk_pull_shift(int(k)))
+    if k % 4 or shift < 4:
+        raise RuntimeError(f"pull_stream_plan needs k % 4 == 0, got k={k}")
+    nb = int(groups) if groups else pull_stream_buckets(dev, num_rows, num_cols, E, dim, k)
+    if nb <= 0:
+        raise RuntimeError(f"pull_stream_plan: the stream path does not apply to {num_rows} x "
+                           f"{num_cols}, dim={dim}, k={k}; pass groups= or use pull_plan")
+    S = int(slices) if slices else int(L.maxk_pull_stream_slices(num_rows, int(num_cols),
+                                                                 int(dim), int(k)))
+
+    def build():
+        bcol = torch.empty(nb + 1, dtype=torch.int32, device=dev)
+        gptr = torch.empty(nb + 1, dtype=torch.int32, device=dev)
+        ent = torch.empty(max(E, 1), 2, dtype=torch.int32, device=dev)[:E]
+        _launch_ws(dev, "maxk_pull_stream_plan", "maxk_pull_stream_plan_workspace_size",
+                   (max(int(num_cols), 1), max(E, 1), nb, S),
+                   (_ptr(indptr), _ptr(indices), _ptr(values), num_rows, int(num_cols), E, int(k),
+                    nb, S, _ptr(bcol), _ptr(gptr), _ptr(ent)))
+        return PullStreamPlan(bcol, gptr, ent, shift, nb, S)
+    return _STREAM_CACHE.get((indptr, indices, values), (int(k), nb, S, int(num_cols)), build,
+                             cache)
+
+
+def _scaled_stream_entries(plan: PullStreamPlan, num_rows: int, k: int,
+                           row_div: torch.Tensor) -> Optional[torch.Tensor]:
+    ent = plan.ent
+    sc = _SCALED.lookup((ent, row_div), ())
+    if sc is not None:
+        return sc
+    if ent.is_cuda and torch.cuda.is_current_stream_capturing():
+        return None
+
+    def build():
+        sc = torch.empty_like(ent)
+        _launch(ent.device, "maxk_pull_stream_entries_scale", _ptr(ent), ent.shape[0], num_rows,
+                int(k), _ptr(row_div), _ptr(sc), _stream(ent.device))
+        return sc
+    return _SCALED.get((ent, row_div), (), build)
+
+
 _HYBRID_CACHE = TensorCache()
 MAXK_PULL_NO_REDUCE, MAXK_PULL_REDUCE_ONLY = 2, 4
 MAXK_HYBRID_PRESCALED = 1
@@ -1076,7 +1149,7 @@
             raise RuntimeError(f"backward_plan: mode '{mode}' needs indptr= and values=")
         if mode == "hybrid":
             return hybrid_plan(indptr, indices, values, num_cols, k, dim or 256)
-        return pull_plan(indptr, indices, values, num_cols, k, dim or 256)
+        return _pull_plan_for(indptr, indices, values, num_cols, k, dim or 256)
     if mode == "dense":
         if indptr is None or values is None:
             raise RuntimeError("backward_plan: mode 'dense' needs indptr= and values=")
@@ -1186,10 +1259,31 @@
         tiles(MAXK_PULL_REDUCE_ONLY | 1, _stream(dev))
 
 
+def _pull_plan_for(indptr, indices, values, num_cols, k, dim):
+    num_rows, E = indptr.numel() - 1, indices.numel()
+    if k % 4 == 0 and pull_stream_buckets(indices.device, num_rows, num_cols, E, dim, k) > 0:
+        return pull_stream_plan(indptr, indices, values, num_cols, k, dim)
+    return pull_plan(indptr, indices, values, num_cols, k, dim)
+
+
 def _bwd_pull(indptr, indices, values, G, row_div, sel, edge_sel, out, shape, chunk, plan):
     num_rows, num_cols, E, D, k = shape
-    tptr, ent, shift, S = (plan if plan is not None else
-                           pull_plan(indptr, indices, values, num_cols, k, D))
+    if plan is None:
+        plan = _pull_plan_for(indptr, indices, values, num_cols, k, D)
+    if isinstance(plan, PullStreamPlan):
+        ent = plan.ent
+        if plan.shift != int(_lib().maxk_pull_shift(int(k))) or ent.shape[0] != E:
+            raise RuntimeError(f"the stream plan was not built for this graph at k={k}")
+        if row_div is not None and E > 0 and _prescale():
+            sc = _scaled_stream_entries(plan, num_rows, k, row_div)
+            if sc is not None:
+                ent, row_div = sc, None
+        _launch_ws(G.device, "maxk_sspmm_backward_pull_stream",
+                   "maxk_sspmm_backward_pull_stream_workspace_size", (num_rows, num_cols, D, k),
+                   (_ptr(G), _ptr(row_div), _ptr(sel), _ptr(plan.bucket_col), _ptr(plan.grp_ptr),
+                    _ptr(ent), plan.n_buckets, _ptr(out), *shape))
+        return
+    tptr, ent, shift, S = plan
     if row_div is not None and E > 0 and _prescale():
         sc = _scaled_entries(ent, None, tptr, num_rows, num_cols, shift, S, row_div)
         if sc is not None:
diff --git a/spgemm-prunning_amd/maxk_cuda_kernels/_capi.py b/spgemm-prunning_amd/maxk_cuda_kernels/_capi.py
--- a/spgemm-prunning_amd/maxk_cuda_kernels/_capi.py
+++ b/spgemm-prunning_amd/maxk_cuda_kernels/_capi.py
@@ -149,6 +149,15 @@
     "maxk_pull_plan_workspace_size": (_sz, [_i64, _i64, _i64, _i32, _i32]),
     "maxk_pull_plan": (ctypes.c_int, [_p, _p, _p, _i64, _i64, _i64, _i32, _i32, _p, _p, _p, _sz,
                                       _p]),
+    "maxk_pull_stream_buckets": (_i64, [_i64, _i64, _i64, _i32, _i32, _i32]),
+    "maxk_pull_stream_slices": (ctypes.c_int, [_i64, _i64, _i32, _i32]),
+    "maxk_pull_stream_plan_workspace_size": (_sz, [_i64, _i64, _i32, _i32]),
+    "maxk_pull_stream_plan": (ctypes.c_int, [_p, _p, _p, _i64, _i64, _i64, _i32, _i32, _i32, _p,
+                                             _p, _p, _p, _sz, _p]),
+    "maxk_pull_stream_entries_scale": (ctypes.c_int, [_p, _i64, _i64, _i32, _p, _p, _p]),
+    "maxk_sspmm_backward_pull_stream_workspace_size": (_sz, [_i64, _i64, _i32, _i32]),
+    "maxk_sspmm_backward_pull_stream": (ctypes.c_int, [_p, _p, _p, _p, _p, _p, _i32, _p, _i64,
+                                                       _i64, _i64, _i32, _i32, _p, _sz, _p]),
     "maxk_backward_mode_auto": (ctypes.c_int, [_i64, _i64, _i64, _i32, _i32, ctypes.c_double]),
     "maxk_pull_locality": (ctypes.c_int, [_p, _p, _i64, _i64, _i32,
                                           ctypes.POINTER(ctypes.c_double), _p, _sz, _p]),
```

Result: faster. 67.40 (median of 6 runs) (+9.1%).
